# mozack/vdjer

Measured on AMD Instinct MI355X. Metric: M paired-reads/sec (k-mer build + contig score), IgH 50bp PE, higher is better.
Workload: dtype u8/u64 (2-bit packed bases, integer counts)

## Files before the change

profiles/summarize_pmc.py:

```python
#!/usr/bin/env python3
import collections
import csv
import glob
import json
import os
import sys


def short(name):
    return name.replace("void ", "").replace("(anonymous namespace)::", "").split("(")[0].split("<")[0]


def med(v):
    v = sorted(v)
    return v[len(v) // 2] if v else None


def stream_in(bench_line):
    if not bench_line:
        return {}
    b = bench_line
    pairs = b["config"]["pairs_per_gpu"]
    st = b.get("scorer_stats", {})
    sym, symw = st.get("kmer_build_sym", 0), st.get("kmer_build_sym_walk", 0)
    tuples = st.get("gated_instances", 0) / (2 if sym else 1)
    items = st.get("recount_items", 0)
    recs = 4 * pairs
    gate = 24 * recs
    return {"k_pool_pack": 101 * recs,
            "k_gated_hist": gate, "k_part_records_g": gate + 16 * tuples, "k_part_tuples_g": 16 * tuples, "k_seg_hist_g": 16 * tuples,
            "k_gated_reduce": 16 * tuples, "k_gated_local": 16 * tuples, "k_walk_items": 24 * recs,
            "k_part_items": 8 * items, "k_recount": 8 * items, "k_compact_partials": 0, "k_bucket_merge": 0}


COMPOSITES = {
    "k_surv_table": ("k_surv_table2", "k_succ_links2"),
    "k_chain_order": ("k_chain_init", "k_chain_jump", "k_chain_len", "k_scan_sums", "k_scan_apply", "k_chain_place", "k_chain_permute", "k_table_remap",
                      "k_partner", "k_chain_words", "k_partner_check"),
    "k_node_order": ("k_rank_keys", "k_rank_scatter", "k_node_emit2"),
    "k_shard_resolve": ("k_resolve_first", "k_resolve_add", "k_resolve_keep"),
}


def step_span(rows, steps):
    packs = [i for i, r in enumerate(rows) if short(r["Kernel_Name"]).startswith("k_pool_pack") or short(r["Kernel_Name"]).startswith("k_pool_unpack")]
    walks = [i for i, r in enumerate(rows) if short(r["Kernel_Name"]) == "k_walk_items"]
    if not packs or len(walks) < steps:
        return []
    chains = int(os.environ.get("PROF_CHAINS", "1"))
    per = max(1, round(len(packs) / max(1, len(walks)))) * chains
    first = packs[-per * steps] if len(packs) >= per * steps else packs[0]
    return rows[first:]


def main():
    out = sys.argv[1]
    steps_timed = int(os.environ.get("PROF_STEPS", "2"))
    bench_line = None
    try:
        bench_line = json.loads(open(os.path.join(out, "bench.json")).read().strip().splitlines()[-1])
    except Exception:
        pass
    STREAM_IN = stream_in(bench_line)
    res = collections.defaultdict(dict)
    step_tot = {}
    for grp in ("fetch", "write", "sq", "tcc", "inst", "ea"):
        per = collections.defaultdict(lambda: collections.defaultdict(list))
        for f in glob.glob(os.path.join(out, grp, "**", "*counter_collection.csv"), recursive=True):
            rows = list(csv.DictReader(open(f)))
            for r in rows:
                per[short(r["Kernel_Name"])][r["Counter_Name"]].append(float(r["Counter_Value"]))
            if grp in ("fetch", "write") and rows:
                key = "Dispatch_Id" if "Dispatch_Id" in rows[0] else None
                if key:
                    rows.sort(key=lambda r: int(r[key]))
                span = step_span(rows, steps_timed)
                agg = collections.defaultdict(lambda: [0.0, 0])
                for r in span:
                    a = agg[short(r["Kernel_Name"])]
                    a[0] += float(r["Counter_Value"]) * 1024
                    a[1] += 1
                step_tot[grp] = {k_: (v_[0] / steps_timed, v_[1] / steps_timed) for k_, v_ in agg.items()}
        for k, cs in per.items():
            for c, v in cs.items():
                res[k][c] = med(v)
                res[k].setdefault("launches_seen", len(v))
    stats = {}
    for f in glob.glob(os.path.join(out, "stats", "**", "*kernel_stats.csv"), recursive=True):
        for r in csv.DictReader(open(f)):
            stats[short(r["Name"])] = {"calls": int(r["Calls"]), "avg_ns": float(r["AverageNs"]), "total_ns": float(r["TotalDurationNs"])}
    for k, d in res.items():
        if "FETCH_SIZE" in d:
            fetch, write = d["FETCH_SIZE"] * 1024, d.get("WRITE_SIZE", 0.0) * 1024
            stream = STREAM_IN.get(k)
            d["fabric_bytes_max"] = int(2 * fetch + write)
            d["stream_in_bytes"] = None if stream is None else int(stream)
            d["hbm_bytes"] = int(fetch + min(fetch, stream / 2) + write) if stream is not None else int(2 * fetch + write)
            d["traffic_rule"] = "FETCH + min(FETCH, stream_in/2) + WRITE" if stream is not None else "2*FETCH + WRITE (no stated stream: bound)"
        if d.get("TCC_HIT_sum") is not None and d.get("TCC_MISS_sum") is not None and d["TCC_HIT_sum"] + d["TCC_MISS_sum"] > 0:
            d["l2_hit"] = round(d["TCC_HIT_sum"] / (d["TCC_HIT_sum"] + d["TCC_MISS_sum"]), 4)
        if d.get("SQ_WAVE_CYCLES"):
            for c in ("SQ_WAIT_ANY", "SQ_WAIT_INST_ANY", "SQ_ACTIVE_INST_ANY", "SQ_WAIT_INST_LDS"):
                if d.get(c) is not None:
                    d[c + "_frac"] = round(d[c] / d["SQ_WAVE_CYCLES"], 4)
        if d.get("SQ_LDS_IDX_ACTIVE"):
            d["lds_conflict_frac"] = round(d.get("SQ_LDS_BANK_CONFLICT", 0.0) / d["SQ_LDS_IDX_ACTIVE"], 4)
        d.update(stats.get(k, {}))
        if d.get("SQ_INSTS_VALU") and d.get("avg_ns"):
            d["valu_issue_frac_at_2.4GHz"] = round(d["SQ_INSTS_VALU"] * 4 / (1024 * 2.4 * d["avg_ns"]), 3)
    step = None
    if "fetch" in step_tot:
        fk, wk = step_tot["fetch"], step_tot.get("write", {})
        tot_f = tot_w = tot_cal = 0.0
        per_kernel = {}
        for k_ in set(fk) | set(wk):
            f_, n_ = fk.get(k_, (0.0, 0))
            w_ = wk.get(k_, (0.0, 0))[0]
            stream = STREAM_IN.get(k_)
            cal = f_ + (min(f_, stream * n_ / 2) if stream is not None else f_) + w_
            per_kernel[k_] = {"fetch_bytes_per_step": int(f_), "write_bytes_per_step": int(w_), "launches_per_step": n_, "fabric_bytes_per_step": int(cal)}
            tot_f += f_; tot_w += w_; tot_cal += cal
        step = {"bytes_per_step": int(tot_cal), "bytes_per_step_max": int(2 * tot_f + tot_w), "fetch_counted": int(tot_f), "write_counted": int(tot_w),
                "kernels_counted": len(per_kernel), "steps": steps_timed,
                "rule": "every dispatch of the last `steps` steps of the process (all kernels: the library's, rocPRIM's, fills), FETCH_SIZE / WRITE_SIZE passes; "
                        "per kernel FETCH + min(FETCH, stated coalesced input / 2) + WRITE, kernels without a stated stream at the bound 2*FETCH + WRITE",
                "per_kernel": per_kernel}
        for comp, members in COMPOSITES.items():
            got = [per_kernel[m] for m in members if m in per_kernel]
            if got:
                res[comp]["composite_of"] = [m for m in members if m in per_kernel]
                res[comp]["hbm_bytes_per_step"] = int(sum(g["fabric_bytes_per_step"] for g in got))
                res[comp]["launches_per_step"] = sum(g["launches_per_step"] for g in got)
                ns_ = sum(res[m].get("avg_ns", 0.0) * per_kernel[m]["launches_per_step"] for m in members if m in per_kernel and m in res)
                res[comp]["ns_per_step"] = ns_
                for c in ("l2_hit", "SQ_WAIT_ANY_frac", "lds_conflict_frac"):
                    ws = [(res[m].get(c), res[m].get("avg_ns", 0.0) * per_kernel[m]["launches_per_step"]) for m in members if m in res and m in per_kernel and res[m].get(c) is not None]
                    if ws and sum(w for _, w in ws) > 0:
                        res[comp][c] = round(sum(v * w for v, w in ws) / sum(w for _, w in ws), 4)
    json.dump({"kernels": res, "step": step}, sys.stdout, indent=1, sort_keys=True)


if __name__ == "__main__":
    main()
```

vdjer_amd/csrc/vdjx_kmer.hip:

```cpp
#include "vdjx_common.h"

#include <algorithm>
#include <numeric>
#include <type_traits>
#include <string.h>
#include <stdlib.h>

#define HIST_THREADS 512
#define HIST_BLOCKS 512u
#define LOCAL_SLOTS 2048u
#define K3_SUB_TUPLES g_sub_tuples
__device__ u32 g_sub_tuples = 262144u;
#define NONE32 0xFFFFFFFFu
#define INST_MASK 0x7FFFFFFFu

struct RecView {
	u64 bhi, blo, nm, lq;
};

__device__ inline RecView load_rec(const u64* __restrict__ bases, const u64* __restrict__ nmask,
                                   const u64* __restrict__ lowq, size_t r) {
	RecView v;
	const ulonglong2 b = ((const ulonglong2*) bases)[r];
	v.bhi = b.x; v.blo = b.y;
// ... 1132 lines not shown
#define REPLY_RQ0 248
template <bool SYM>
__global__ __launch_bounds__(64) void k_shard_reply(const uint2* __restrict__ queries, u32 nq, const u32* __restrict__ owner_off, u32 G,
                                                    const Partial* __restrict__ dense, const u32* __restrict__ dense_ref,
                                                    const u32* __restrict__ dstart, u32 NBo, const u64* __restrict__ low_inst,
                                                    const u64* __restrict__ bases, const u64* __restrict__ nmask,
                                                    vdjx_qrows quals, u64 rec_base, const u32* __restrict__ scan, u32 n_local, int k, int rl, int ob,
                                                    uint8_t* __restrict__ replies) {
	const u32 qi = blockIdx.x;
	if (qi >= nq) return;
	const u32 lane = threadIdx.x;
	u32 o = 0;
	while (o + 1 < G && owner_off[o + 1] <= qi) o++;
	const uint2 q = queries[qi];
	const u32 di = dstart[(size_t) o * NBo] + q.x;
	u64 finst, finst_r = 0;
	u32 p_cg;
	if (SYM) { const PartialS p = ((const PartialS*) dense)[di]; finst = ps_fg(p); finst_r = p.fgr; p_cg = ps_cg(p); }
	else { const Partial p = dense[di]; finst = p.fg; p_cg = p.cg; }
	const u32 need = q.y >> 30;
	const u32 om = (1u << ob) - 1u;
	auto local_rec = [&](u64 inst) -> u64 {
		if (!scan) return (inst >> ob) - rec_base;
		const u32 g = (u32) (inst >> ob);
		u32 lo = 0, hi = n_local;
		while (lo + 1 < hi) { const u32 mid = lo + ((hi - lo) >> 1); if (scan[mid] <= g) lo = mid; else hi = mid; }
		return lo;
	};
	const u64 frec = local_rec(finst);
	const u32 foff = (u32) finst & om;
	const u64 finst_local = (frec << ob) | foff;
	const u64 frec_r = SYM ? local_rec(finst_r) : 0;
	const u32 foff_r = (u32) finst_r & om;
	const u64 finst_r_local = (frec_r << ob) | foff_r;
	uint8_t* out = replies + (size_t) qi * REPLY_BYTES;
	if (lane == 0) {
		((u32*) out)[0] = q.y;
		((u32*) out)[1] = 0;
		((u64*) out)[1] = finst;
		if (SYM) ((u64*) out)[REPLY_R0 / 8] = finst_r;
	}
	if (!SYM && lane < (REPLY_BYTES - REPLY_R0) / 4) ((u32*) (out + REPLY_R0))[lane] = 0;
	if (lane < 8) {
		const int W = rl <= VDJX_SHORT_READ_LEN ? 2 : VDJX_LONG_W, M = rl <= VDJX_SHORT_READ_LEN ? 1 : VDJX_LONG_M;
		((u64*) out)[2 + lane] = (int) lane < W ? bases[frec * W + lane] : ((int) lane < W + M ? nmask[frec * M + (lane - W)] : 0ull);
	}
	if ((int) lane >= k) return;
	u32 acc = 0, acc_r = 0;
	const u32 ref = dense_ref[di];
	if ((need & NEED_Q) && ref != NONE32) {
		const u32 cg = p_cg & ~PART_FLAG;
		for (u32 i = 0; i < cg; i++) {
			const u64 inst = low_inst[ref + i];
			if (inst != (scan ? finst_local : finst)) acc += (u32) (uint8_t) (quals.row((inst >> ob) - rec_base)[((u32) inst & om) + lane] - 33);
			if (SYM) {
				const u64 m = vdjx_inst_mirror(inst, ob, rl, k);
				if (m != (scan ? finst_r_local : finst_r)) acc_r += (u32) (uint8_t) (quals.row((m >> ob) - rec_base)[((u32) m & om) + lane] - 33);
			}
		}
	}
	const uint8_t* fr = quals.row(frec);
	out[REPLY_Q0 + lane] = (uint8_t) (acc > 255u ? 255u : acc);
	out[REPLY_Q0 + REPLY_KQ + lane] = (uint8_t) (fr[foff + lane] - 33);
	out[REPLY_Q0 + 2 * REPLY_KQ + lane] = (uint8_t) (fr[lane] - 33);
	if (SYM) {
		const uint8_t* frr = quals.row(frec_r);
		out[REPLY_RQ0 + lane] = (uint8_t) (acc_r > 255u ? 255u : acc_r);
		out[REPLY_RQ0 + REPLY_KQ + lane] = (uint8_t) (frr[foff_r + lane] - 33);
		out[REPLY_RQ0 + 2 * REPLY_KQ + lane] = (uint8_t) (frr[lane] - 33);
	}
}

__global__ void k_resolve_first(const uint8_t* __restrict__ replies, u32 nr, const u64* __restrict__ p_mg, u32* __restrict__ p_r0,
                                const u64* __restrict__ p_mgr, u32 np) {
	const u32 r = blockIdx.x * blockDim.x + threadIdx.x;
	if (r >= nr) return;
	const uint8_t* me = replies + (size_t) r * REPLY_BYTES;
	const u32 pid = ((const u32*) me)[0] & PID_MASK;
	if (((const u64*) me)[1] == p_mg[pid]) p_r0[pid] = r;
	if (p_mgr && ((const u64*) me)[REPLY_R0 / 8] == p_mgr[pid]) p_r0[np + pid] = r;
}

__global__ __launch_bounds__(256) void k_resolve_add(const uint8_t* __restrict__ replies, u32 nr, const u32* __restrict__ p_r0, int k, u32* __restrict__ p_fl,
                                                     u32* __restrict__ p_S, u32 np) {
	const u32 r = blockIdx.x * 4u + (threadIdx.x >> 6);
	const u32 lane = threadIdx.x & 63u;
	if (r >= nr) return;
	const uint8_t* me = replies + (size_t) r * REPLY_BYTES;
	const u32 w0 = ((const u32*) me)[0];
	const u32 pid = w0 & PID_MASK, need = w0 >> 30;
	const u32 r0 = p_r0[pid];
	if (r0 == NONE32) return;
	if ((need & NEED_SEQ) && r != r0 && lane == 0) {
		const u64* a = (const u64*) me;
		const u64* b = (const u64*) (replies + (size_t) r0 * REPLY_BYTES);
		u64 d = 0;
#pragma unroll
		for (int w = 2; w < 10; w++) d |= a[w] ^ b[w];
		if (d) p_fl[pid] = 1;
	}
	if ((need & NEED_Q) && (int) lane < k) {
		const uint8_t* first = me + REPLY_Q0 + (r == r0 ? 2 * REPLY_KQ : REPLY_KQ);
		atomicAdd(&p_S[(size_t) pid * 64 + lane], (u32) me[REPLY_Q0 + lane] + (u32) first[lane]);
		if (np) {
			const uint8_t* first_r = me + REPLY_RQ0 + (r == p_r0[np + pid] ? 2 * REPLY_KQ : REPLY_KQ);
			atomicAdd(&p_S[((size_t) np + pid) * 64 + lane], (u32) me[REPLY_RQ0 + lane] + (u32) first_r[lane]);
		}
	}
}

template <bool SYM>
__global__ void k_resolve_keep(PendOut po, u32 np, const u32* __restrict__ p_fl, const u32* __restrict__ p_S, int k, u32 mf, u32 mqq, u32 tlow,
                               SurvOutG so) {
	const u32 p = blockIdx.x * blockDim.x + threadIdx.x;
	const bool in = p < np;
	const u32 need = in ? po.need[p] : 0u;
	bool keep = in && ((need & NEED_SEQ) ? p_fl[p] != 0 : true);
	const u32 cg = in ? po.cg[p] : 0u;
	const u32 cgc = cg > CNT_CAP ? CNT_CAP : cg;
	keep = keep && cgc >= mf;
	bool keep_r = keep;
	if (keep && cg < tlow) {
		for (int j = 0; j < k; j++) if (p_S[(size_t) p * 64 + j] < mqq) { keep = false; break; }
		if (SYM) for (int j = 0; j < k; j++) if (p_S[((size_t) np + p) * 64 + j] < mqq) { keep_r = false; break; }
	}
	if (!SYM) {
		const u32 pos = vdjx_wave_inc(so.n, keep);
		if (keep && pos < so.cap) {
			so.lo[pos] = po.lo[p]; so.hi[pos] = po.hi[p];
			so.gcnt[pos] = cgc; so.gfirst[pos] = po.mg[p];
		}
		return;
	}
	const bool any = keep || keep_r;
	const u32 pos = vdjx_wave_inc(so.n, any, 2u);
	if (any && pos + 1 < so.cap) {
		so.lo[pos] = po.lo[p]; so.hi[pos] = po.hi[p];
		so.gcnt[pos] = cgc | (keep ? 0u : GC_SHADOW); so.gfirst[pos] = po.mg[p];
		u64 rh, rlo;
		vdjx_kmer_rc(po.hi[p], po.lo[p], k, rh, rlo);
		so.lo[pos + 1] = rlo; so.hi[pos + 1] = rh;
		so.gcnt[pos + 1] = cgc | (keep_r ? 0u : GC_SHADOW); so.gfirst[pos + 1] = po.mgr[p];
	}
}

__global__ void k_first_to_scan(u64* __restrict__ a, size_t na, u64* __restrict__ b, size_t nb, const u32* __restrict__ scan, int ob) {
	const size_t i = (size_t) blockIdx.x * blockDim.x + threadIdx.x;
	if (i >= na + nb) return;
	u64* p = i < na ? a + i : b + (i - na);
	const u64 v = *p;
	if (v != NONE64) *p = ((u64) scan[v >> ob] << ob) | (v & ((1ull << ob) - 1ull));
}

__global__ void k_node_flags(const u64* __restrict__ s_lo, const u64* __restrict__ s_hi, u32 n, int k,
                             const u32* __restrict__ vbits, const u32* __restrict__ jbits,
                             uint8_t* __restrict__ has_v, uint8_t* __restrict__ has_j) {
	u32 i = blockIdx.x * blockDim.x + threadIdx.x;
	if (i >= n) return;
	if (k <= 16) { has_v[i] = 1; has_j[i] = 1; return; }
	u128 key = ((u128) s_hi[i] << 64) | s_lo[i];
	u32 code = (u32) (key >> (2 * (k - 16)));
	has_v[i] = code ? (vbits[code >> 5] >> (code & 31)) & 1u : 0;
	has_j[i] = code ? (jbits[code >> 5] >> (code & 31)) & 1u : 0;
}


#define IT_INST_BITS 35
#define IT_INST_MASK ((1ull << IT_INST_BITS) - 1ull)
#define IT_SURV_SHIFT 38
int vdjx_sort_pairs_raw(void* tmp, size_t* tmp_bytes, hipStream_t st, u64* k_in, u64* k_out, u32* v_in, u32* v_out, u32 n, unsigned end_bit);
#define IT_HOLE 0xFFFFFFFFFFFFFFFFull
#define WALK_THREADS 256

#define SLOT_HI_BITS 36
#define SLOT_HI_MASK ((1ull << SLOT_HI_BITS) - 1ull)
struct SurvTable { const ulonglong2* slots; u32 mask; const ulonglong2* skey; const u32* bloom; u32 bloom_mask; };

struct ItemFmt {
	u32 pmask;
	u32 len_shift;
	u32 maxlen;
	u32 mul, inv;
	u32 bmask;
	u32 ns;
};
__device__ inline u32 it_surv(const ItemFmt& f, u64 x) { return (u32) (x >> IT_SURV_SHIFT) & f.pmask; }
__device__ inline u32 it_len(const ItemFmt& f, u64 x) { return f.maxlen > 1 ? (u32) (x >> f.len_shift) + 1u : 1u; }
__device__ inline u32 it_scat(const ItemFmt& f, u32 p) { return ((((p >> 4) * f.mul) & f.bmask) << 4) | (p & 15u); }

__global__ void k_surv_table2(const u64* __restrict__ s_lo, const u64* __restrict__ s_hi, u32 n, ulonglong2* __restrict__ slots, u32 mask,
                              ulonglong2* __restrict__ skey, u32* __restrict__ bloom, u32 bloom_mask) {
	const u32 i = blockIdx.x * blockDim.x + threadIdx.x;
	if (i >= n) return;
	const u64 lo = s_lo[i], hi = s_hi[i];
	skey[i] = make_ulonglong2(lo, hi);
	const u64 h = vdjx_mix(lo, hi);
	{
		const u32 bit = (u32) (h >> 40) & bloom_mask;
		atomicOr(&bloom[bit >> 5], 1u << (bit & 31));
	}
	u32 slot = (u32) (h >> 20) & mask;
	const unsigned long long entry = hi | ((unsigned long long) (i + 1) << SLOT_HI_BITS);
	while (atomicCAS((unsigned long long*) &slots[slot].y, 0ull, entry) != 0ull) slot = (slot + 1) & mask;
	slots[slot].x = lo;
}

__device__ inline int surv_lookup2f(const SurvTable& t, u64 lo, u64 hi);

__device__ inline int surv_lookup2(const SurvTable& t, u64 lo, u64 hi) {
	u32 slot = (u32) (vdjx_mix(lo, hi) >> 20) & t.mask;
	for (;;) {
		const ulonglong2 v = t.slots[slot];
		if (!v.y) return -1;
		if (v.x == lo && (v.y & SLOT_HI_MASK) == hi) return (int) (v.y >> SLOT_HI_BITS) - 1;
		slot = (slot + 1) & t.mask;
	}
}

__device__ inline int surv_lookup2f(const SurvTable& t, u64 lo, u64 hi) {
	const u64 h = vdjx_mix(lo, hi);
	const u32 bit = (u32) (h >> 40) & t.bloom_mask;
	if (!((t.bloom[bit >> 5] >> (bit & 31)) & 1u)) return -1;
	return surv_lookup2(t, lo, hi);
}

__global__ void k_succ_links2(SurvTable t, u32 n, int k, const u32* __restrict__ gcnt, u32* __restrict__ succ, unsigned long long* __restrict__ pred,
                              u32* __restrict__ bestsucc) {
	const u32 u = blockIdx.x * blockDim.x + threadIdx.x;
	if (u >= n) return;
	const ulonglong2 kk = t.skey[u];
	const u128 base = (((u128) kk.y << 64) | kk.x) << 2;
	const u128 km = k < 64 ? (((u128) 1) << (2 * k)) - 1 : ~(u128) 0;
	const int sh = 2 * (k - 1);
	const u32 fb = (u32) (sh < 64 ? kk.x >> sh : kk.y >> (sh - 64)) & 3u;
	const unsigned long long mine = ((unsigned long long) (gcnt[u] & GC_MASK) << 32) | ((unsigned long long) (fb ^ 1u) << 30) | (unsigned long long) u;
	u32 best = NONE32, best_g = 0;
	for (u32 b = 0; b < 4; b++) {
		const u128 key = (base | (u128) b) & km;
		const int s = surv_lookup2(t, (u64) key, (u64) (key >> 64));
		succ[u * 4 + b] = s >= 0 ? (u32) s : NONE32;
		if (s >= 0 && (u32) s != u) {
			const u32 g = gcnt[s] & GC_MASK;
			if (best == NONE32 || g >= best_g) { best = (u32) s; best_g = g; }
			atomicMax(&pred[s], mine);
		}
	}
	bestsucc[u] = best;
}

#define CHAIN_JUMPS 31
__global__ void k_chain_init(const unsigned long long* __restrict__ pred, const u32* __restrict__ bestsucc, u32 n, u64* __restrict__ pd) {
	const u32 v = blockIdx.x * blockDim.x + threadIdx.x;
	if (v >= n) return;
	const unsigned long long x = pred[v];
	const u32 u = (u32) x & 0x3FFFFFFFu;
	pd[v] = x != 0ull && bestsucc[u] == v ? ((u64) u << 32) | 1ull : ((u64) NONE32 << 32);
}

__global__ void k_partner(SurvTable t, u32 n, int k, u32* __restrict__ partner) {
	const u32 p = blockIdx.x * blockDim.x + threadIdx.x;
	if (p >= n) return;
	const ulonglong2 kk = t.skey[p];
	u64 rh, rlo;
	vdjx_kmer_rc(kk.y, kk.x, k, rh, rlo);
	const int q = surv_lookup2(t, rlo, rh);
	partner[p] = q >= 0 ? (u32) q : NONE32;
}
__global__ void k_partner_check(const u32* __restrict__ partner, const u64* __restrict__ linw, u32 n, u32* __restrict__ bad) {
	const u32 p = blockIdx.x * blockDim.x + threadIdx.x;
	if (p >= n) return;
	bool wrong = partner[p] == NONE32;
	const bool linked = (linw[p >> 4] >> (15u - (p & 15u))) & 1ull;
	if (!wrong && linked && (p + 1 >= n || partner[p + 1] != partner[p] - 1u)) wrong = true;
	const u64 m = __ballot(wrong);
	if (m && __lane_id() == 0) atomicAdd(bad, (u32) __popcll(m));
}

__global__ void k_chain_jump(u64* __restrict__ pd, u32 n, const u32* __restrict__ open_prev, u32* __restrict__ open_now) {
	if (open_prev && *open_prev == 0) return;
	const u32 v = blockIdx.x * blockDim.x + threadIdx.x;
	bool open = false;
	if (v < n) {
		u64 x = __atomic_load_n(&pd[v], __ATOMIC_RELAXED);
		for (int it = 0; it < CHAIN_JUMPS; it++) {
			const u32 p = (u32) (x >> 32);
			if (p == NONE32) break;
			const u64 y = __atomic_load_n(&pd[p], __ATOMIC_RELAXED);
			const u32 pp = (u32) (y >> 32);
			if (pp == NONE32) break;
			x = ((u64) pp << 32) | (u64) ((u32) x + (u32) y);
			__atomic_store_n(&pd[v], x, __ATOMIC_RELAXED);
			open = true;
		}
	}
	if (__ballot(open) && __lane_id() == 0) atomicAdd(open_now, 1u);
}

__device__ inline void chain_of(const u64* pd, u32 v, u32& head, u32& dist) {
	const u64 x = pd[v];
	const u32 p = (u32) (x >> 32);
	head = v; dist = 0;
	if (p == NONE32) return;
	if ((u32) (pd[p] >> 32) != NONE32) return;
	head = p; dist = (u32) x;
}
__global__ void k_chain_len(const u64* __restrict__ pd, u32 n, u32* __restrict__ len) {
	const u32 v = blockIdx.x * blockDim.x + threadIdx.x;
	if (v >= n) return;
	u32 h, d;
	chain_of(pd, v, h, d);
	atomicAdd(&len[h], 1u);
}

#define SCAN_BLOCK 4096u
__global__ __launch_bounds__(256) void k_scan_sums(const u32* __restrict__ a, u32 n, u32* __restrict__ sums) {
	__shared__ u32 part[4];
	const u32 b0 = blockIdx.x * SCAN_BLOCK;
	u32 s = 0;
	for (u32 i = threadIdx.x; i < SCAN_BLOCK; i += 256) s += b0 + i < n ? a[b0 + i] : 0u;
	s = (u32) vdjx_wave_scan_add((int) s);
	if ((threadIdx.x & 63) == 63) part[threadIdx.x >> 6] = s;
	__syncthreads();
	if (threadIdx.x == 0) sums[blockIdx.x] = part[0] + part[1] + part[2] + part[3];
}
__global__ __launch_bounds__(256) void k_scan_apply(const u32* __restrict__ a, u32 n, const u32* __restrict__ sum_start, u32* __restrict__ out) {
	__shared__ u32 part[5];
	const u32 b0 = blockIdx.x * SCAN_BLOCK + threadIdx.x * 16;
	u32 loc[16];
	u32 s = 0;
	for (int i = 0; i < 16; i++) { loc[i] = s; s += b0 + i < n ? a[b0 + i] : 0u; }
	const u32 incl = (u32) vdjx_wave_scan_add((int) s);
	if ((threadIdx.x & 63) == 63) part[threadIdx.x >> 6] = incl;
	__syncthreads();
	u32 base = sum_start[blockIdx.x] + incl - s;
	for (u32 w = 0; w < (threadIdx.x >> 6); w++) base += part[w];
	for (int i = 0; i < 16; i++) if (b0 + i < n) out[b0 + i] = base + loc[i];
}

__global__ void k_chain_place(const u64* __restrict__ pd, const u32* __restrict__ off, u32 n, u32* __restrict__ newidx) {
	const u32 v = blockIdx.x * blockDim.x + threadIdx.x;
	if (v >= n) return;
	u32 h, d;
	chain_of(pd, v, h, d);
	newidx[v] = off[h] + d;
}
__global__ void k_chain_permute(const u32* __restrict__ newidx, u32 n, const u64* __restrict__ lo, const u64* __restrict__ hi, const u32* __restrict__ gcnt,
                                const u64* __restrict__ gfirst, const u32* __restrict__ succ, u64* __restrict__ lo2, u64* __restrict__ hi2,
                                u32* __restrict__ gcnt2, u64* __restrict__ gfirst2, ulonglong2* __restrict__ skey2, u32* __restrict__ succ2) {
	const u32 v = blockIdx.x * blockDim.x + threadIdx.x;
	if (v >= n) return;
	const u32 q = newidx[v];
	const u64 l = lo[v], h = hi[v];
	lo2[q] = l; hi2[q] = h; gcnt2[q] = gcnt[v]; gfirst2[q] = gfirst[v];
	skey2[q] = make_ulonglong2(l, h);
	const uint4 s = *(const uint4*) &succ[(size_t) v * 4];
	uint4 r;
	r.x = s.x == NONE32 ? NONE32 : newidx[s.x];
	r.y = s.y == NONE32 ? NONE32 : newidx[s.y];
	r.z = s.z == NONE32 ? NONE32 : newidx[s.z];
	r.w = s.w == NONE32 ? NONE32 : newidx[s.w];
	*(uint4*) &succ2[(size_t) q * 4] = r;
}
__global__ void k_table_remap(ulonglong2* __restrict__ slots, u32 n_slots, const u32* __restrict__ newidx) {
	const u32 i = blockIdx.x * blockDim.x + threadIdx.x;
	if (i >= n_slots) return;
	const u64 y = slots[i].y;
	if (!y) return;
	slots[i].y = (y & SLOT_HI_MASK) | ((u64) (newidx[(u32) (y >> SLOT_HI_BITS) - 1] + 1u) << SLOT_HI_BITS);
}

__global__ void k_chain_words(const u32* __restrict__ succ, const ulonglong2* __restrict__ skey, u32 n, int k, u64* __restrict__ linw, u32* __restrict__ fbw,
                              const u32* __restrict__ partner) {
	const u32 p = blockIdx.x * blockDim.x + threadIdx.x;
	const u32 j = p & 15u;
	u64 w = 0;
	u32 fb = 0;
	if (p < n) {
		const uint4 s = *(const uint4*) &succ[(size_t) p * 4];
		const u32 sv[4] = {s.x, s.y, s.z, s.w};
		const bool mirrored = !partner || (p + 1 < n && partner[p] != NONE32 && partner[p + 1] == partner[p] - 1u);
		for (u32 b = 0; b < 4; b++) if (sv[b] != NONE32) {
			if (sv[b] == p + 1 && mirrored) w |= (1ull << (15u - j)) | ((u64) b << (32u + 2u * (15u - j)));
			else w |= 1ull << (31u - j);
		}
		const ulonglong2 kk = skey[p];
		const int sh = 2 * (k - 1);
		fb = (u32) (sh < 64 ? kk.x >> sh : kk.y >> (sh - 64)) & 3u;
	}
	u32 fw = fb << (2 * j);
	for (int d = 1; d < 16; d <<= 1) {
		w |= ((u64) (u32) __shfl_xor((int) (w >> 32), d) << 32) | (u32) __shfl_xor((int) (u32) w, d);
		fw |= (u32) __shfl_xor((int) fw, d);
	}
	if (j == 0 && p < n) { linw[p >> 4] = w; fbw[p >> 4] = fw; }
}

struct WalkRecS {
	u64 bhi, blo; int rl;
	__device__ inline void kmer_u(int k, int o, u64& hi, u64& lo) const { vdjx_kmer_at(bhi, blo, rl, k, o, hi, lo); }
	__device__ inline void kmer_l(int k, int o, u64& hi, u64& lo) const { vdjx_kmer_at_lane(bhi, blo, rl, k, o, hi, lo); }
	__device__ inline u32 bases16(int bi) const {
		const int sh = 2 * (rl - 16 - bi);
		const u32 rw_dn = vdjx_bits_at_lane(bhi, blo, (u32) (sh > 0 ? sh : 0));
		const u32 up = (u32) (sh < 0 ? -sh : 0);
		return (rw_dn << (up & 31u)) & (0u - (u32) (up < 32u));
	}
	__device__ inline u32 base(int i) const { return vdjx_base_at_lane(bhi, blo, rl, i); }
};
struct WalkRecL {
	const u64* row;
	__device__ inline void kmer_u(int k, int o, u64& hi, u64& lo) const { vdjx_kmer_at_words(row, k, o, hi, lo); }
	__device__ inline void kmer_l(int k, int o, u64& hi, u64& lo) const { vdjx_kmer_at_words(row, k, o, hi, lo); }
	__device__ inline u32 bases16(int bi) const { return vdjx_bases16_words(row, bi); }
	__device__ inline u32 base(int i) const { return vdjx_base_words(row, i); }
};
__device__ inline bool wm_test(u64 m, int i) { return (m >> i) & 1ull; }
__device__ inline bool wm_test(const vdjx_mask3& m, int i) { return m.test(i); }
__device__ inline void wm_set(u64& m, int i) { m |= 1ull << i; }
__device__ inline void wm_set(vdjx_mask3& m, int i) { m.set(i); }
__device__ inline int wm_next(u64 m, int from, int none) { const u64 x = from < 64 ? m & (~0ull << from) : 0ull; return x ? __builtin_ctzll(x) : none; }
__device__ inline int wm_next(const vdjx_mask3& m, int from, int none) { return m.next(from, none); }
__device__ inline u32 wm_slice32(u64 m, int from) { return from < 64 ? (u32) (m >> from) : 0u; }
__device__ inline u32 wm_slice32(const vdjx_mask3& m, int from) { return (u32) m.slice(from); }

template <bool LONG, bool SYM = false>
__global__ __launch_bounds__(WALK_THREADS) void k_walk_items(const u64* __restrict__ bases, const u64* __restrict__ nmask, size_t R, int rl, int ob_bits, int k,
                                                             SurvTable t, const u32* __restrict__ succ, const u64* __restrict__ linw, ItemFmt f,
                                                             u32 range_shift, u32 n_ranges,
                                                             u64* __restrict__ raw, u64 raw_cap, u32 blk_items,
                                                             unsigned long long* __restrict__ g_cursor,
                                                             u32* __restrict__ range_cnt, u32* __restrict__ g_err, u32 dbg_in,
                                                             const u32* __restrict__ partner) {
	static_assert(!(LONG && SYM), "SYM is the short-read form");
#ifdef VDJX_ABLATE
	const u32 dbg = dbg_in;
#else
	(void) dbg_in;
	constexpr u32 dbg = 0u;
#endif
	extern __shared__ u32 hist[];
	typedef typename std::conditional<LONG, vdjx_mask3, u64>::type MaskT;
	typedef typename std::conditional<LONG, WalkRecL, WalkRecS>::type RecT;
	for (u32 i = threadIdx.x; i < n_ranges; i += WALK_THREADS) hist[i] = 0;
	__syncthreads();
	u64* myrow = (u64*) (hist + ((n_ranges + 1u) & ~1u)) + threadIdx.x * GL_ROW_LONG;
	const int P = rl - k + 1;
	const size_t per = ((R + gridDim.x - 1) / gridDim.x + WALK_THREADS - 1) / WALK_THREADS * WALK_THREADS;
	const size_t r0 = (size_t) blockIdx.x * per;
	const size_t r1 = r0 + per < R ? r0 + per : R;
	const int lane = __lane_id();
	u64 blk = 0;
	u32 fill = blk_items;
#ifdef WALK_STATS
	u32 st_rows = 0, st_rounds = 0, st_filter = 0, st_lookup = 0, st_items = 0, st_chain = 0;
#define WST(x) x
#else
#define WST(x)
#endif
	bool have_blk = false, dead = false;
	__shared__ u64 dq[WALK_THREADS / 64][128];
	__shared__ ulonglong2 dq_b[LONG ? 1 : WALK_THREADS / 64][LONG ? 1 : 128];
	__shared__ u64 dq_v[LONG ? 1 : WALK_THREADS / 64][LONG ? 1 : 128];
	const u32 wq = threadIdx.x >> 6;
	u32 qn = 0;
	auto walk_row = [&](auto fresh_tag, const size_t r, const bool live, const int o_from, const ulonglong2 qb, const u64 qv) {
		constexpr bool FRESH = decltype(fresh_tag)::value;
		RecT v;
		MaskT V{};
		if constexpr (LONG) {
			v.row = myrow;
			if (live) {
				stage_row_long(myrow, bases, r);
				const vdjx_mask3 nm = load_bad3(nmask, nullptr, r);
				for (int o16 = 0; o16 < P; o16 += 16) {
					const u64 g = (u64) vdjx_clean16(nm, o16, k, P) << (o16 & 63);
					if ((o16 >> 6) == 0) V.w0 |= g; else if ((o16 >> 6) == 1) V.w1 |= g; else V.w2 |= g;
				}
			} else
				for (int w = 0; w < GL_ROW_LONG; w++) myrow[w] = 0;
		} else {
			v.bhi = v.blo = 0; v.rl = rl;
			if (!FRESH) { if (live) { v.bhi = qb.x; v.blo = qb.y; V = qv; } }
			else if (live) {
				const RecView rv = load_rec(bases, nmask, nullptr, r);
				v.bhi = rv.bhi; v.blo = rv.blo;
				u64 inv = rv.nm;
				int cur = 1;
				while (cur * 2 <= k) { inv |= inv >> cur; cur *= 2; }
				inv |= inv >> (k - cur);
				V = ~inv & (P >= 64 ? ~0ull : (1ull << P) - 1ull);
			}
		}
		int o = wm_next(V, o_from, P);
		int s = -1;
		u32 in = 0;
		bool first = FRESH, have_c = false;
		MaskT C{};
		WST(st_rows++;)
		while (__ballot(o < P)) {
			WST(st_rounds++;)
			bool need = o < P && s < 0;
			if (FRESH) {
				const bool later = need && !first;
				const u64 lm = __ballot(later);
				if (lm) {
					if (later) {
						const u32 qi = qn + (u32) __popcll(lm & ((1ull << lane) - 1ull));
						dq[wq][qi] = ((u64) r << 8) | (u64) (u32) o;
						if constexpr (!LONG) { dq_b[wq][qi] = make_ulonglong2(v.bhi, v.blo); dq_v[wq][qi] = V; }
						o = P; need = false;
					}
					qn += (u32) __popcll(lm);
				}
			}
			WST(if (__ballot(need)) st_lookup++;)
			if (!FRESH && __ballot(need && !first && !have_c)) {
				WST(st_filter++;)
				const bool mine = need && !first && !have_c;
				for (int ob = 0; ob < P; ob += 4) {
					u32 wv[4], bt[4];
#pragma unroll
					for (int j = 0; j < 4; j++) {
						const int oo = ob + j;
						wv[j] = 0; bt[j] = 0;
						if (mine && oo >= o && oo < P && wm_test(V, oo)) {
							u64 khi, klo;
							v.kmer_u(k, oo, khi, klo);
							const u32 bit = (u32) (vdjx_mix(klo, khi) >> 40) & t.bloom_mask;
							bt[j] = bit & 31u;
							wv[j] = (dbg & 8u) ? 0xFFFFFFFFu : t.bloom[bit >> 5];
						}
					}
#pragma unroll
					for (int j = 0; j < 4; j++) if ((wv[j] >> bt[j]) & 1u) wm_set(C, ob + j);
				}
				if (mine) have_c = true;
			}
			if (need) {
				bool filtered = false;
				if (!first) {
					o = wm_next(C, o, P);
					filtered = true;
				}
				first = false;
				if (o < P) {
					u64 khi, klo;
					v.kmer_l(k, o, khi, klo);
// ... 188 lines not shown
#pragma unroll
		for (u32 j = 0; j < PER; j++) {
			const size_t t = ts + (size_t) j * PART_THREADS + threadIdx.x;
			r_b[j] = NONE32;
			if (t < te) { r_it[j] = in[t]; r_b[j] = (it_scat(f, it_surv(f, r_it[j])) >> range_shift) & mask; }
		}
#pragma unroll
		for (u32 j = 0; j < PER; j++) if (r_b[j] != NONE32) atomicAdd(&cnt[r_b[j]], 1u);
		__syncthreads();
		part_scan(cnt, base, tmp, nbk);
		for (u32 i = threadIdx.x; i < nbk; i += PART_THREADS) {
			cur[i] = base[i];
			gbase[i] = cnt[i] ? atomicAdd(&gc[i], cnt[i]) : 0u;
		}
		__syncthreads();
#pragma unroll
		for (u32 j = 0; j < PER; j++) if (r_b[j] != NONE32) stage[atomicAdd(&cur[r_b[j]], 1u)] = r_it[j];
		__syncthreads();
		const u32 n = base[nbk];
		for (u32 i = threadIdx.x; i < n; i += PART_THREADS) {
			const u64 x = stage[i];
			const u32 b = (it_scat(f, it_surv(f, x)) >> range_shift) & mask;
			out[gbase[b] + (i - base[b])] = x;
		}
		__syncthreads();
	}
}

#define RC_THREADS 1024
#define RC_UNR 4
template <typename IT> struct RcNone;
template <> struct RcNone<u32> { static constexpr u32 v = 0xFFFFFFFFu; };
template <> struct RcNone<u64> { static constexpr u64 v = 0xFFFFFFFFFFFFFFFFull; };
__device__ inline void rc_min(u32* p, u32 v) { atomicMin(p, v); }
__device__ inline void rc_min(u64* p, u64 v) { atomicMin((unsigned long long*) p, (unsigned long long) v); }

#define RC_CS 17u
#define RC_MS 77u
__device__ inline u32 rc_win(u32 k, u32 s) { return 31u + ((0x261B0E00u >> (8u * k)) & 0xFFu) + s - 1u; }
template <u32 SB, typename IT>
__global__ __launch_bounds__(RC_THREADS) void k_recount(const u64* __restrict__ items, const u32* __restrict__ range_start, ItemFmt f, u32 ns, u64 rec_base, int ob,
                                                        const u32* __restrict__ fbw, u32* __restrict__ ucnt, u64* __restrict__ ufirst, u64* __restrict__ in_first,
                                                        unsigned long long* __restrict__ n_inst) {
	__shared__ u32 c[SB / 16 * RC_CS];
	__shared__ IT mv[SB / 16 * RC_MS];
	__shared__ IT ef[SB * 4];
	__shared__ u32 fbl[SB / 16];
	__shared__ unsigned long long tot;
	constexpr IT NONE = RcNone<IT>::v;
	const u32 b = blockIdx.x;
	const u32 s0 = b * SB;
	const u32 nb = (ns + 15u) >> 4;
	for (u32 i = threadIdx.x; i < SB / 16 * RC_CS; i += RC_THREADS) c[i] = 0;
	for (u32 i = threadIdx.x; i < SB / 16 * RC_MS; i += RC_THREADS) mv[i] = NONE;
	for (u32 i = threadIdx.x; i < SB * 4; i += RC_THREADS) ef[i] = NONE;
	for (u32 i = threadIdx.x; i < SB / 16; i += RC_THREADS) {
		const u32 sb = (s0 >> 4) + i;
		const u32 blk = (sb * f.inv) & f.bmask;
		fbl[i] = sb <= f.bmask && blk < nb ? fbw[blk] : 0u;
	}
	if (threadIdx.x == 0) tot = 0;
	__syncthreads();
	const u32 i0 = range_start[b], i1 = range_start[b + 1];
	const u32 iend = i0 + (i1 - i0 + RC_THREADS * RC_UNR - 1) / (RC_THREADS * RC_UNR) * (RC_THREADS * RC_UNR);
	for (u32 ib = i0 + threadIdx.x; ib < iend; ib += RC_THREADS * RC_UNR) {
		u64 xs[RC_UNR];
#pragma unroll
		for (int u = 0; u < RC_UNR; u++) { const u32 i = ib + (u32) u * RC_THREADS; xs[u] = i < i1 ? items[i] : IT_HOLE; }
#pragma unroll
		for (int u = 0; u < RC_UNR; u++) {
			const u64 x = xs[u];
			const bool live = x != IT_HOLE;
			const u32 p = it_surv(f, x);
			const u32 len = live ? it_len(f, x) : 1u;
			const u32 sl = live ? it_scat(f, p) - s0 : 0u;
			const u32 a = sl & 15u, e = a + len - 1u;
			const u64 inst = x & IT_INST_MASK;
			const bool shaped = live && (a == 0u || e == 15u);
			const u32 cb = (sl >> 4) * RC_CS, mb = (sl >> 4) * RC_MS;
			const u32 slot = mb + (a == 0u ? e : 15u + a);
			const IT val = (IT) (inst + 15u - a);
			bool mine = shaped;
			const u64 act = __ballot(shaped);
			if (act) {
				const int leader = __ffsll((long long) act) - 1;
				const u32 lslot = (u32) __builtin_amdgcn_readlane((int) slot, leader);
				const bool same = shaped && slot == lslot;
				const u64 m = __ballot(same);
				if (__popcll(m) >= 8) {
					const u64 v64 = inst + 15u - a;
					const u32 hi_min = vdjx_wave_min(same ? (u32) (v64 >> 32) : 0xFFFFFFFFu);
					const u32 lo_min = vdjx_wave_min(same && (u32) (v64 >> 32) == hi_min ? (u32) v64 : 0xFFFFFFFFu);
					if (__lane_id() == leader) {
						const u32 n = (u32) __popcll(m);
						atomicAdd(&c[cb + e], n);
						if (a) atomicAdd(&c[cb + a - 1u], 0u - n);
						rc_min(&mv[lslot], (IT) (((u64) hi_min << 32) | lo_min));
					}
					mine = shaped && !same;
				}
			}
			if (live && (mine || !shaped)) {
				atomicAdd(&c[cb + e], 1u);
				if (a) atomicAdd(&c[cb + a - 1u], 0xFFFFFFFFu);
			}
			if (mine) rc_min(&mv[slot], val);
			if (live && !shaped) {
				const u32 k = 31u - (u32) __builtin_clz(len), w = 1u << k;
				rc_min(&mv[mb + rc_win(k, a)], val);
				if (len != w) rc_min(&mv[mb + rc_win(k, e + 1u - w)], val);
			}
			if (live && ((x >> 37) & 1ull)) {
				IT* ep = &ef[sl * 4 + (u32) ((x >> 35) & 3ull)];
				if (vdjx_peek(ep) > (IT) inst) rc_min(ep, (IT) inst);
			}
		}
	}
	__syncthreads();
	const u64 add = rec_base << ob;
	u32 my_cnt = 0;
	for (u32 i = threadIdx.x; i < SB; i += RC_THREADS) {
		const u32 sb = (s0 + i) >> 4;
		const u32 blk = (sb * f.inv) & f.bmask;
		const u32 x = i & 15u, p = (blk << 4) | x;
		if (sb > f.bmask || blk >= nb || p >= ns) continue;
		const u32 cbase = (i >> 4) * RC_CS, mbase = (i >> 4) * RC_MS;
		u32 cc = 0;
		IT mm = NONE;
		IT me = NONE;
		for (u32 e = x; e < 16; e++) { cc += c[cbase + e]; const IT t = mv[mbase + e]; mm = t < mm ? t : mm; if (x) me = t < me ? t : me; }
		for (u32 a = 1; a <= x; a++) { const IT t = mv[mbase + 15 + a]; mm = t < mm ? t : mm; if (a < x) me = t < me ? t : me; }
#pragma unroll
		for (u32 k = 0; k < 4; k++) {
			const u32 w = 1u << k;
			const u32 lo = x >= w ? x - w + 1u : 1u, hi = x < 15u - w ? x : 15u - w;
			for (u32 s = lo ? lo : 1u; s <= hi; s++) { const IT t = mv[mbase + rc_win(k, s)]; mm = t < mm ? t : mm; if (s < x) me = t < me ? t : me; }
		}
		my_cnt += cc;
		ucnt[p] = cc;
		ufirst[p] = mm == NONE ? NONE64 : (u64) mm - 15u + x + add;
		IT e4[4] = {ef[i * 4], ef[i * 4 + 1], ef[i * 4 + 2], ef[i * 4 + 3]};
		if (x && me != NONE) {
			const u32 pa = (fbl[i >> 4] >> (2 * (x - 1))) & 3u;
			const IT t = (IT) (me - 15u + x);
			if (t < e4[pa]) e4[pa] = t;
		}
		for (u32 q = 0; q < 4; q++) in_first[(size_t) p * 4 + q] = e4[q] == NONE ? NONE64 : (u64) e4[q] + add;
	}
	if (my_cnt) atomicAdd(&tot, (unsigned long long) my_cnt);
	__syncthreads();
	if (threadIdx.x == 0 && tot) atomicAdd(n_inst, tot);
}

__global__ void k_count_unseen(const u64* __restrict__ ufirst, u32 n, u32* __restrict__ out) {
	const u32 i = blockIdx.x * blockDim.x + threadIdx.x;
	const bool un = i < n && ufirst[i] == NONE64;
	const u64 m = __ballot(un);
	if (m && __lane_id() == 0) atomicAdd(out, (u32) __popcll(m));
}

__global__ void k_edges_from_in(SurvTable t, u32 n, int k, const u64* __restrict__ in_first, u32* __restrict__ in_from,
                                u64* __restrict__ edge_first, u32* __restrict__ edge_to) {
	const u32 e = blockIdx.x * blockDim.x + threadIdx.x;
	if (e >= n * 4u) return;
	const u64 fs = in_first[e];
	if (fs == NONE64) { in_from[e] = NONE32; return; }
	const u32 v = e >> 2, a = e & 3u;
	const ulonglong2 kk = t.skey[v];
	const u128 kv = ((u128) kk.y << 64) | kk.x;
	const u128 ku = (kv >> 2) | ((u128) a << (2 * (k - 1)));
	const int u = surv_lookup2(t, (u64) ku, (u64) (ku >> 64));
	in_from[e] = u >= 0 ? (u32) u : NONE32;
	if (u >= 0) {
		const u32 oe = (u32) u * 4u + ((u32) kk.x & 3u);
		edge_first[oe] = fs;
		edge_to[oe] = v;
	}
}

struct SurvRec { u64 lo, hi; u32 gcnt, pad; u64 gfirst; };

__global__ void k_surv_pack(const u64* __restrict__ lo, const u64* __restrict__ hi, const u32* __restrict__ gcnt,
                            const u64* __restrict__ gfirst, u32 n, SurvRec* __restrict__ out) {
	u32 i = blockIdx.x * blockDim.x + threadIdx.x;
	if (i >= n) return;
	SurvRec r{lo[i], hi[i], gcnt[i], 0u, gfirst[i]};
	out[i] = r;
}

__global__ void k_surv_unpack(const SurvRec* __restrict__ in, u32 n, u64* __restrict__ lo, u64* __restrict__ hi, u32* __restrict__ gcnt,
                              u64* __restrict__ gfirst, u32* __restrict__ n_real) {
	u32 i = blockIdx.x * blockDim.x + threadIdx.x;
	const bool in_range = i < n;
	SurvRec r{0, 0, GC_SHADOW, 0, 0};
	if (in_range) {
		r = in[i];
		lo[i] = r.lo; hi[i] = r.hi; gcnt[i] = r.gcnt; gfirst[i] = r.gfirst;
	}
	(void) vdjx_wave_inc(n_real, in_range && !(r.gcnt & GC_SHADOW));
}

struct NodeOut {
	u64* first_inst; u32* gcnt; u32* freq; uint8_t* hv; uint8_t* hj; u64* klo; u64* khi; char* kmers;
	uint8_t* to_deg; u32* to_ids; uint8_t* from_deg; u32* from_ids;
};

__global__ void k_rank_keys(const u64* __restrict__ ufirst, const u32* __restrict__ gcnt, u32 n, u64* __restrict__ key, u32* __restrict__ idx) {
	const u32 i = blockIdx.x * blockDim.x + threadIdx.x;
	if (i < n) { key[i] = (gcnt[i] & GC_SHADOW) ? NONE64 : ufirst[i]; idx[i] = i; }
}
__global__ void k_rank_scatter(const u64* __restrict__ key, const u32* __restrict__ idx, u32 n, u32* __restrict__ rank) {
	const u32 j = blockIdx.x * blockDim.x + threadIdx.x;
	if (j >= n) return;
	const u32 i = idx[j];
	rank[i] = key[j] == NONE64 ? i : j;
}

__global__ __launch_bounds__(256) void k_root_count(const uint8_t* __restrict__ from_deg, u32 n, u32* __restrict__ block_cnt) {
	__shared__ u32 cnt;
	if (threadIdx.x == 0) cnt = 0;
	__syncthreads();
	const u32 i = blockIdx.x * 256 + threadIdx.x;
	const bool r = i < n && from_deg[i] == 0;
	const u64 b = __ballot(r);
	if ((threadIdx.x & 63) == 0 && b) atomicAdd(&cnt, (u32) __popcll(b));
	__syncthreads();
	if (threadIdx.x == 0) block_cnt[blockIdx.x] = cnt;
}

__global__ __launch_bounds__(256) void k_root_list(const uint8_t* __restrict__ from_deg, u32 n, const u32* __restrict__ block_start,
                                                   u32* __restrict__ roots) {
	__shared__ u32 wave_cnt[4];
	const u32 i = blockIdx.x * 256 + threadIdx.x;
	const bool r = i < n && from_deg[i] == 0;
	const u64 b = __ballot(r);
	const u32 w = threadIdx.x >> 6, lane = threadIdx.x & 63;
	if (lane == 0) wave_cnt[w] = (u32) __popcll(b);
	__syncthreads();
	u32 base = block_start[blockIdx.x];
	for (u32 j = 0; j < w; j++) base += wave_cnt[j];
	if (r) roots[base + (u32) __popcll(b & ((1ull << lane) - 1))] = i;
}

__device__ inline void sort4_desc64(u64 (&f)[4], u32 (&id)[4]) {
#define CSW(a, b) { const bool sw = kk[a] < kk[b]; if (sw) { u64 t = kk[a]; kk[a] = kk[b]; kk[b] = t; u32 u = id[a]; id[a] = id[b]; id[b] = u; } }
	u64 kk[4];
	for (int i = 0; i < 4; i++) kk[i] = f[i] == NONE64 ? 0ull : f[i] + 1;
	CSW(0, 1) CSW(2, 3) CSW(0, 2) CSW(1, 3) CSW(1, 2)
	for (int i = 0; i < 4; i++) f[i] = kk[i] ? kk[i] - 1 : NONE64;
#undef CSW
}

__global__ void k_node_emit2(const u64* __restrict__ s_lo, const u64* __restrict__ s_hi, const u32* __restrict__ s_gcnt,
                             const u32* __restrict__ s_ucnt, const u64* __restrict__ s_ufirst, const uint8_t* __restrict__ hv,
                             const uint8_t* __restrict__ hj, const u32* __restrict__ rank, const u64* __restrict__ edge_first,
                             const u32* __restrict__ edge_to, const u64* __restrict__ in_first, const u32* __restrict__ in_from,
                             u32 n, int k, NodeOut o) {
	const u32 s = blockIdx.x * blockDim.x + threadIdx.x;
	if (s >= n) return;
	if (s_gcnt[s] & GC_SHADOW) return;
	const u32 r = rank[s];
	o.first_inst[r] = s_ufirst[s];
	o.gcnt[r] = s_gcnt[s];
	o.freq[r] = s_ucnt[s] > 32765u ? 32765u : s_ucnt[s];
	o.hv[r] = hv[s];
	o.hj[r] = hj[s];
	const u128 key = ((u128) s_hi[s] << 64) | s_lo[s];
	for (int j = 0; j < k; j++) {
		const u32 b = (u32) (key >> (2 * (k - 1 - j))) & 3u;
		o.kmers[(size_t) r * k + j] = b == 0 ? 'A' : (b == 1 ? 'T' : (b == 2 ? 'C' : 'G'));
	}
	u64 f[4];
	u32 id[4];
	for (int e = 0; e < 4; e++) {
		f[e] = edge_first[(size_t) s * 4 + e];
		if (f[e] != NONE64 && (s_gcnt[edge_to[(size_t) s * 4 + e]] & GC_SHADOW)) f[e] = NONE64;
		id[e] = f[e] != NONE64 ? rank[edge_to[(size_t) s * 4 + e]] + 1 : 0;
	}
	sort4_desc64(f, id);
	u32 deg = 0;
	for (int e = 0; e < 4; e++) { o.to_ids[(size_t) r * 4 + e] = f[e] != NONE64 ? id[e] : 0; deg += f[e] != NONE64; }
	o.to_deg[r] = (uint8_t) deg;
	for (int e = 0; e < 4; e++) {
		f[e] = in_first[(size_t) s * 4 + e];
		if (f[e] != NONE64 && (in_from[(size_t) s * 4 + e] == NONE32 || (s_gcnt[in_from[(size_t) s * 4 + e]] & GC_SHADOW))) f[e] = NONE64;
		id[e] = f[e] != NONE64 ? rank[in_from[(size_t) s * 4 + e]] + 1 : 0;
	}
	sort4_desc64(f, id);
	deg = 0;
	for (int e = 0; e < 4; e++) { o.from_ids[(size_t) r * 4 + e] = f[e] != NONE64 ? id[e] : 0; deg += f[e] != NONE64; }
	o.from_deg[r] = (uint8_t) deg;
}

namespace {

struct PersistAlloc {
	vdjx_ctx* c;
	explicit PersistAlloc(vdjx_ctx* ctx) : c(ctx) {}
	template <typename T> hipError_t alloc(T** out, size_t n) {
		*out = (T*) c->shard_arena.alloc((n ? n : 1) * sizeof(T));
		return *out ? hipSuccess : hipErrorOutOfMemory;
	}
	vdjx_arena::mark_t mark() const { return c->shard_arena.mark(); }
	void release_to(vdjx_arena::mark_t m) { c->shard_arena.release_to(m); }
};

struct PoolView { const u64* bases; const u64* nmask; vdjx_qrows quals; int rl; int ob; };

template <typename TUP> struct GTuples {
	TUP* t = nullptr;
	u32* bucket_start = nullptr;
	u32 NB = 0, N = 0;
};

struct SurvivorsG {
	u64 *lo = nullptr, *hi = nullptr, *gfirst = nullptr, *ufirst = nullptr;
	u32 *gcnt = nullptr, *ucnt = nullptr;
	u32 n = 0, n_real = 0;
	u64 ndist = 0;
};

inline u32 ceil_log2_u64(u64 x) { u32 b = 0; while ((1ull << b) < x) b++; return b; }

static bool sync_debug() { static const bool on = vdjx_env_set("VDJX_SYNC_DEBUG"); return on; }
static void dbg_sync(vdjx_ctx* c, const char* what) {
	if (!sync_debug()) return;
	const hipError_t e = hipStreamSynchronize(c->stream);
	fprintf(stderr, "[vdjx] %s: %s\n", what, hipGetErrorString(e));
}

struct GatedHist { u32 HB = 0, NBH = 0, N = 0; u32* hstart = nullptr; bool sym = false; };
static bool build_sym(const vdjx_pool* pool, int k) {
	return pool->sym && pool->W == 2 && (k & 1) && pool->n_records % 2 == 0;
}
static bool sym_walk_wanted() { static const bool on = !vdjx_env_set("VDJX_NO_SYM_WALK"); return on; }
static size_t gated_bucket_default() { static const size_t v = (size_t) vdjx_env_num("VDJX_GATED_BUCKET", 3072, 1, 1ll << 32); return v; }
template <typename A>
int stage_gated_hist(vdjx_ctx* c, A& db, const vdjx_pool* pool, int k, size_t per_bucket, u64 geometry_instances, GatedHist* gh, bool sym = false) {
	hipStream_t st = c->stream;
	const size_t R = sym ? pool->n_records / 2 : pool->n_records;
	const int P = pool->rl - k + 1;
	const u64 NI = geometry_instances ? geometry_instances : (u64) R * (u64) P;
	const size_t per = per_bucket ? per_bucket : gated_bucket_default();
	const u32 hb_max = pool->W > 2 ? 14u : 15u;
	u32 HB = ceil_log2_u64((NI + per - 1) / per);
	HB = std::max(8u, std::min(hb_max, HB));
	const u32 NBH = 1u << HB;
#ifdef VDJX_ABLATE
	static const u32 hist_dbg = (u32) vdjx_env_num("VDJX_HIST_DBG", 0, 0, 4);
#else
	constexpr u32 hist_dbg = 0;
#endif
	u32 nblk = (u32) std::min<size_t>(HIST_BLOCKS, (R + 4095) / 4096);
	if (nblk == 0) nblk = 1;
	size_t rpb = (R + nblk - 1) / nblk;
	u32 *hcnt, *hstart;
	HIP_TRY(db.alloc(&hcnt, NBH));
	HIP_TRY(db.alloc(&hstart, NBH + 1));
	HIP_TRY(hipMemsetAsync(hcnt, 0, (size_t) NBH * 4, st));
	const bool lng = pool->W > 2;
	const size_t lds_hist = (size_t) NBH * 4 + (HIST_THREADS / 64) * (lng ? GL_WAVE_BYTES_LONG : GL_WAVE_BYTES);
	HIP_TRY(hipFuncSetAttribute((const void*) k_gated_hist<false>, hipFuncAttributeMaxDynamicSharedMemorySize, (int) lds_hist));
	HIP_TRY(hipFuncSetAttribute((const void*) k_gated_hist<true>, hipFuncAttributeMaxDynamicSharedMemorySize, (int) lds_hist));
	HIP_TRY(hipFuncSetAttribute((const void*) k_gated_hist<false, true>, hipFuncAttributeMaxDynamicSharedMemorySize, (int) lds_hist));
	{
		vdjx_prof_scope ps(c, "k_gated_hist");
		if (lng) hipLaunchKernelGGL(k_gated_hist<true>, dim3(nblk), dim3(HIST_THREADS), lds_hist, st, pool->d_bases, pool->d_nmask, pool->d_lowq, R, pool->rl, k, HB, rpb, hcnt, hist_dbg);
		else if (sym) hipLaunchKernelGGL((k_gated_hist<false, true>), dim3(nblk), dim3(HIST_THREADS), lds_hist, st, pool->d_bases, pool->d_nmask, pool->d_lowq, R, pool->rl, k, HB, rpb, hcnt, hist_dbg);
		else hipLaunchKernelGGL(k_gated_hist<false>, dim3(nblk), dim3(HIST_THREADS), lds_hist, st, pool->d_bases, pool->d_nmask, pool->d_lowq, R, pool->rl, k, HB, rpb, hcnt, hist_dbg);
	}
	dbg_sync(c, "k_gated_hist");
	hipLaunchKernelGGL(k_bucket_scan, dim3(1), dim3(1024), 0, st, hcnt, NBH, hstart);
	HIP_TRY(hipMemcpyAsync(c->h_pin, hstart + NBH, 4, hipMemcpyDeviceToHost, st));
	HIP_TRY(hipStreamSynchronize(st));
	HIP_TRY(hipGetLastError());
#ifdef VDJX_ABLATE
	if (hist_dbg) return VDJX_ESTATE;
#endif
	const u32 N = *(const u32*) c->h_pin;
	c->stats["gated_instances"] = sym ? 2ull * N : N;
	gh->HB = HB; gh->NBH = NBH; gh->N = N; gh->hstart = hstart; gh->sym = sym;
	return VDJX_OK;
}

template <typename TUP, typename A>
int stage_gated_cut(vdjx_ctx* c, A& db, const vdjx_pool* pool, u64 rec_base, int k, size_t per_bucket, u64 geometry_instances, const GatedHist& gh, GTuples<TUP>* out) {
	hipStream_t st = c->stream;
	const bool sym = gh.sym;
	const size_t R = sym ? pool->n_records / 2 : pool->n_records;
	const int P = pool->rl - k + 1;
	const size_t per = per_bucket ? per_bucket : gated_bucket_default();
	const u32 hb_max = pool->W > 2 ? 14u : 15u;
	const bool lng = pool->W > 2;
	const u32 HB = gh.HB, NBH = gh.NBH, N = gh.N;
	u32* hstart = gh.hstart;
	size_t rpb;
	out->N = N;
	const u64 Ng = geometry_instances ? geometry_instances : (u64) N;
	static const size_t refine = (size_t) vdjx_env_num("VDJX_REFINE_TUPLES", 4096, 1, 1ll << 32);
	u32 T = 8;
	while (T < HB && ((u64) per << T) < Ng) T++;
	u32 extra = 0;
	const size_t refine_at = per_bucket ? std::max<size_t>(per_bucket, refine / 2) : refine;
	if (T == HB && HB == hb_max && Ng / NBH > refine_at) {
		extra = 1;
		while (extra < 5 && (Ng >> extra) / NBH > refine_at) extra++;
	}
	const u32 Tt = T + extra;
	const u32 NBt = 1u << Tt;
	HIP_TRY(db.alloc(&out->t, (size_t) N + 1));
	constexpr u32 stage_tuples = PARTR_STAGE_BYTES / (u32) sizeof(TUP);
	constexpr u32 lds_partr = PARTR_STAGE_BYTES + stage_tuples * 4;
	HIP_TRY(hipFuncSetAttribute((const void*) k_part_records_g<TUP, false>, hipFuncAttributeMaxDynamicSharedMemorySize, (int) lds_partr));
	HIP_TRY(hipFuncSetAttribute((const void*) k_part_records_g<TUP, true>, hipFuncAttributeMaxDynamicSharedMemorySize, (int) lds_partr));
	HIP_TRY(hipFuncSetAttribute((const void*) k_part_records_g<TUP, false, true>, hipFuncAttributeMaxDynamicSharedMemorySize, (int) lds_partr));
	HIP_TRY(hipFuncSetAttribute((const void*) k_part_tuples_g<TUP>, hipFuncAttributeMaxDynamicSharedMemorySize, PART_LDS_BYTES));
	u32 cbits = Tt, fbits = 0;
	if (Tt > 10) { cbits = extra ? Tt - 10 : 8; fbits = Tt - cbits; }
	const u32 NBc = 1u << cbits;
	u32 nblk2 = (u32) std::min<size_t>(1024, (R + 2047) / 2048);
	if (nblk2 == 0) nblk2 = 1;
	rpb = (R + nblk2 - 1) / nblk2;
	u32* gcur;
	HIP_TRY(db.alloc(&gcur, NBc));
	TUP* l1 = out->t;
	if (fbits) HIP_TRY(db.alloc(&l1, (size_t) N + 1));
	{
		vdjx_prof_scope ps(c, "k_part_records");
		hipLaunchKernelGGL(k_init_cursors, dim3((NBc + 255) / 256), dim3(256), 0, st, hstart, NBc, HB - cbits, gcur);
		const u64 NIl = (u64) R * (u64) P;
		u64 rr = N ? (u64) stage_tuples * 3 / 4 * NIl / ((u64) N * (u64) P) : 1u << 16;
		rr = std::max<u64>(PART_THREADS, std::min<u64>(rr / PART_THREADS * PART_THREADS, lng ? 1u << 14 : 1u << 16));
		if (lng) hipLaunchKernelGGL((k_part_records_g<TUP, true>), dim3(nblk2), dim3(PART_THREADS), lds_partr, st, pool->d_bases, pool->d_nmask, pool->d_lowq, R, rec_base,
		                            pool->rl, k, 64 - cbits, NBc, rpb, (u32) rr, gcur, l1);
		else if (sym) hipLaunchKernelGGL((k_part_records_g<TUP, false, true>), dim3(nblk2), dim3(PART_THREADS), lds_partr, st, pool->d_bases, pool->d_nmask, pool->d_lowq, R, rec_base,
		                                 pool->rl, k, 64 - cbits, NBc, rpb, (u32) rr, gcur, l1);
		else hipLaunchKernelGGL((k_part_records_g<TUP, false>), dim3(nblk2), dim3(PART_THREADS), lds_partr, st, pool->d_bases, pool->d_nmask, pool->d_lowq, R, rec_base,
		                        pool->rl, k, 64 - cbits, NBc, rpb, (u32) rr, gcur, l1);
	}
	dbg_sync(c, "k_part_records");
	u32* tstart;
	HIP_TRY(db.alloc(&tstart, NBt + 1));
	out->NB = NBt;
	out->bucket_start = tstart;
	constexpr u32 slices = PART_SLICES;
	if (extra) {
		u32* fine_cnt;
		HIP_TRY(db.alloc(&fine_cnt, NBt));
		HIP_TRY(hipMemsetAsync(fine_cnt, 0, (size_t) NBt * 4, st));
		vdjx_prof_scope ps(c, "k_seg_hist");
		hipLaunchKernelGGL(k_seg_hist_g<TUP>, dim3(NBc * slices), dim3(512), 0, st, l1, hstart, HB - cbits, slices, 64 - Tt, fbits, fine_cnt);
		hipLaunchKernelGGL(k_bucket_scan, dim3(1), dim3(1024), 0, st, fine_cnt, NBt, tstart);
	} else {
		hipLaunchKernelGGL(k_pick_u32, dim3((NBt + 1 + 255) / 256), dim3(256), 0, st, hstart, 1u << (HB - Tt), NBt + 1, tstart);
	}
	if (fbits) {
		u32* gcur2;
		HIP_TRY(db.alloc(&gcur2, NBt));
		vdjx_prof_scope ps(c, "k_part_tuples");
		hipLaunchKernelGGL(k_init_cursors, dim3((NBt + 255) / 256), dim3(256), 0, st, tstart, NBt, 0u, gcur2);
		hipLaunchKernelGGL(k_part_tuples_g<TUP>, dim3(NBc * slices), dim3(PART_THREADS), PART_LDS_BYTES, st, l1, hstart, HB - cbits, slices, 64 - Tt, fbits,
		                   gcur2, out->t);
	}
	return VDJX_OK;
}

template <typename TUP, typename A>
int stage_gated_partition(vdjx_ctx* c, A& db, const vdjx_pool* pool, u64 rec_base, int k, size_t per_bucket, u64 geometry_instances, GTuples<TUP>* out, bool sym = false) {
	GatedHist gh;
	int rc = stage_gated_hist(c, db, pool, k, per_bucket, geometry_instances, &gh, sym);
	if (rc) return rc;
	return stage_gated_cut<TUP>(c, db, pool, rec_base, k, per_bucket, geometry_instances, gh, out);
}

static int set_sub_tuples(vdjx_ctx* c) {
	static const u32 sub = (u32) vdjx_env_num("VDJX_SUB_TUPLES", 262144, 1, 0xFFFFFFFFll);
	if (c->sub_tuples_set != sub) {
		HIP_TRY(hipMemcpyToSymbolAsync(HIP_SYMBOL(g_sub_tuples), &sub, 4, 0, hipMemcpyHostToDevice, c->stream));
		c->sub_tuples_set = sub;
	}
	return VDJX_OK;
}
template <typename TUP, typename A>
int bucket_order(vdjx_ctx* c, A& db, const GTuples<TUP>& t, u32** order) {
	*order = nullptr;
	if (t.NB < 1024) return VDJX_OK;
	HIP_TRY(db.alloc(order, t.NB));
	hipLaunchKernelGGL(k_bucket_order, dim3(1), dim3(1024), 0, c->stream, t.bucket_start, t.NB, *order);
	return VDJX_OK;
}

template <typename TUP, typename A>
int stage_gated_reduce(vdjx_ctx* c, A& db, const GTuples<TUP>& t, const PoolView& pv, u64 rec_base, int k, int mf, int mq, SurvivorsG* sv, bool sym = false) {
	hipStream_t st = c->stream;
	int rc = set_sub_tuples(c);
	if (rc) return rc;
	if (mq >= 255) mq = 254;
	const u32 mqq = (u32) (mq < 0 ? 0 : (mq > 214 ? 214 : mq));
	const u32 tlow = 1 + (mqq + 19) / 20;
	const u32 cmin = (u32) std::max(mf, 2);
	const u32 mfu = (u32) std::max(mf, 0);
	const u32 cap = (sym ? t.N : t.N / 2) + 16;
	u32 *g_err, *n_surv;
	u64* g_distinct;
	HIP_TRY(db.alloc(&sv->lo, cap)); HIP_TRY(db.alloc(&sv->hi, cap)); HIP_TRY(db.alloc(&sv->gcnt, cap)); HIP_TRY(db.alloc(&sv->gfirst, cap));
	HIP_TRY(db.alloc(&g_distinct, 64 * 16 + 2));
	g_err = (u32*) (g_distinct + 64 * 16);
	n_surv = g_err + 1;
	u32* n_real = g_err + 2;
	HIP_TRY(hipMemsetAsync(g_distinct, 0, (64 * 16 + 2) * 8, st));
	SurvOutG so{sv->lo, sv->hi, sv->gcnt, sv->gfirst, n_surv, cap, n_real};
	static const u32 rd_dbg = (u32) vdjx_env_num("VDJX_RD_DBG", 0, 0, 9);
	if (t.N) {
		vdjx_prof_scope ps(c, "k_gated_reduce");
		u32* order;
		if ((rc = bucket_order(c, db, t, &order))) return rc;
		if (sym) hipLaunchKernelGGL((k_gated_reduce<TUP, true>), dim3(t.NB), dim3(RD_THREADS), 0, st, t.t, t.bucket_start, pv.bases, pv.nmask, pv.quals, pv.rl, pv.ob, k, rec_base,
		                            mfu, cmin, mqq, tlow, so, g_distinct, g_err, rd_dbg, (const u32*) order);
		else hipLaunchKernelGGL(k_gated_reduce<TUP>, dim3(t.NB), dim3(RD_THREADS), 0, st, t.t, t.bucket_start, pv.bases, pv.nmask, pv.quals, pv.rl, pv.ob, k, rec_base,
		                        mfu, cmin, mqq, tlow, so, g_distinct, g_err, rd_dbg, (const u32*) order);
	}
	u64* spread = (u64*) c->h_pin;
	u32* tail = (u32*) (spread + 64 * 16);
	static_assert((64 * 16 + 2) * 8 == VDJX_HPIN_SYNC_BYTES, "h_pin layout (vdjx_common.h)");
	HIP_TRY(hipMemcpyAsync(spread, g_distinct, VDJX_HPIN_SYNC_BYTES, hipMemcpyDeviceToHost, st));
	HIP_TRY(hipStreamSynchronize(st));
	HIP_TRY(hipGetLastError());
	const u32 ns = tail[1], err = tail[0];
	if (err) { vdjx_set_error("k_gated_reduce: %u buckets could not be split to fit LDS", err); return VDJX_EHIP; }
	if (ns > cap) { vdjx_set_error("survivor capacity logic failed (%u > %u)", ns, cap); return VDJX_EHIP; }
	sv->ndist = 0;
	for (int i = 0; i < 64; i++) sv->ndist += spread[i * 16];
	sv->n = ns;
	sv->n_real = sym ? tail[2] : ns;
	c->stats["kmer_build_shadows"] = ns - sv->n_real;
	return VDJX_OK;
}

struct RecountOut { u32* ucnt; u64* ufirst; u64* in_first; u32* in_from; u64* edge_first; u32* edge_to; };
struct RecountStatus { const u32* g_err = nullptr; const u32* n_items = nullptr; const unsigned long long* n_inst = nullptr; u32 ns = 0; };
#define VDJX_ESYMWALK (-1000)
static int recount_status_check(vdjx_ctx* c, const u32* hp, u32 ns) {
	if (hp[6] || hp[7]) { vdjx_set_error("the mirrored walk found %u + %u places where the chains are not mirror images", hp[6], hp[7]); return VDJX_ESYMWALK; }
	if (hp[0]) { vdjx_set_error("k_walk_items: item buffer too small (%u waves stopped)", hp[0]); return VDJX_EHIP; }
	if (hp[1]) { vdjx_set_error("internal error: %u of %u surviving k-mers were not met again in the records (VDJX_SYNC_DEBUG=1 names them)", hp[1], ns); return VDJX_EHIP; }
	c->stats["recount_items"] = hp[2];
	c->stats["recount_instances"] = *(const unsigned long long*) (hp + 4);
	return VDJX_OK;
}

template <typename A>
int stage_recount(vdjx_ctx* c, A& db, const vdjx_pool* pool, u64 rec_base, int k, SurvivorsG& sv, const RecountOut& ro,
                  bool derive_edges, SurvTable* table_out = nullptr, RecountStatus* defer = nullptr, bool sym_walk = false) {
	hipStream_t st = c->stream;
	const size_t R = pool->n_records;
	const int P = pool->rl - k + 1;
	const u32 ns = sv.n;
	if (ns >= (1u << 26)) { vdjx_set_error("more than 2^26 surviving k-mers: not supported by the recount items"); return VDJX_ELIMIT; }
	if (R >= (1ull << 29)) { vdjx_set_error("more than 2^29 records on one GPU: not supported by the recount items"); return VDJX_ELIMIT; }
	if ((u64) R * (u64) P >= (1ull << 32)) { vdjx_set_error("records*offsets = %llu >= 2^32 on one GPU: shard the pool over more GPUs", (unsigned long long) ((u64) R * (u64) P)); return VDJX_ELIMIT; }
	u32 tmask = 1023;
	while ((size_t) tmask + 1 < (size_t) ns * 2) tmask = tmask * 2 + 1;
	unsigned long long* pred;
	ulonglong2* table;
	u32 *succ0, *succ, *bloom, *clen, *coff, *csum, *csum_start, *newidx, *jump_open, *fbw, *gcnt2, *bestsucc, *partner = nullptr;
	u64 *pd, *lo2, *hi2, *gfirst2, *linw;
	ulonglong2 *skey0, *skey;
	u32 bloom_bits = 1u << 16;
	while (bloom_bits < (1u << 30) && (size_t) bloom_bits < (size_t) ns * 16) bloom_bits <<= 1;
	const u32 nb16 = (ns + 15u) >> 4;
	const u32 n_scan = (ns + SCAN_BLOCK - 1) / SCAN_BLOCK;
	const u32 n_jump = (ceil_log2_u64((u64) ns + 1) + 4) / 5 + 1;
	{
		auto up = [](size_t b) { return (b + 255) & ~(size_t) 255; };
		const size_t b_bloom = up(bloom_bits / 8), b_table = up(((size_t) tmask + 1) * 16), b_pred = up((size_t) ns * 8), b_clen = up((size_t) ns * 4),
		             b_jump = up((size_t) (n_jump + 1) * 4), b_linw = up(((size_t) nb16 + 1) * 8);
		uint8_t* z;
		const size_t zb = b_bloom + b_table + b_pred + b_clen + b_jump + b_linw;
		HIP_TRY(db.alloc(&z, zb));
		HIP_TRY(hipMemsetAsync(z, 0, zb, st));
		table = (ulonglong2*) z; z += b_table;
		bloom = (u32*) z; z += b_bloom;
		pred = (unsigned long long*) z; z += b_pred;
		clen = (u32*) z; z += b_clen;
		jump_open = (u32*) z; z += b_jump;
		linw = (u64*) z;
	}
	HIP_TRY(db.alloc(&skey0, ns)); HIP_TRY(db.alloc(&skey, ns));
	HIP_TRY(db.alloc(&succ0, (size_t) ns * 4)); HIP_TRY(db.alloc(&succ, (size_t) ns * 4));
	HIP_TRY(db.alloc(&pd, ns)); HIP_TRY(db.alloc(&coff, ns));
	HIP_TRY(db.alloc(&csum, n_scan)); HIP_TRY(db.alloc(&csum_start, n_scan + 1)); HIP_TRY(db.alloc(&newidx, ns));
	HIP_TRY(db.alloc(&lo2, ns)); HIP_TRY(db.alloc(&hi2, ns)); HIP_TRY(db.alloc(&gcnt2, ns)); HIP_TRY(db.alloc(&gfirst2, ns));
	HIP_TRY(db.alloc(&fbw, nb16));
	HIP_TRY(db.alloc(&bestsucc, ns));
	if (sym_walk) HIP_TRY(db.alloc(&partner, ns));
	const SurvTable tb0{table, tmask, skey0, bloom, bloom_bits - 1};
	const SurvTable tb{table, tmask, skey, bloom, bloom_bits - 1};
	if (table_out) *table_out = tb;
	const dim3 gs((ns + 255) / 256), bs(256);
	{
		vdjx_prof_scope ps(c, "k_surv_table");
		hipLaunchKernelGGL(k_surv_table2, gs, bs, 0, st, sv.lo, sv.hi, ns, table, tmask, skey0, bloom, bloom_bits - 1);
		hipLaunchKernelGGL(k_succ_links2, gs, bs, 0, st, tb0, ns, k, sv.gcnt, succ0, pred, bestsucc);
	}
	{
		vdjx_prof_scope ps(c, "k_chain_order");
		hipLaunchKernelGGL(k_chain_init, gs, bs, 0, st, pred, bestsucc, ns, pd);
		for (u32 j = 0; j < n_jump; j++) hipLaunchKernelGGL(k_chain_jump, gs, bs, 0, st, pd, ns, j ? jump_open + j - 1 : (const u32*) nullptr, jump_open + j);
		hipLaunchKernelGGL(k_chain_len, gs, bs, 0, st, pd, ns, clen);
		hipLaunchKernelGGL(k_scan_sums, dim3(n_scan), dim3(256), 0, st, clen, ns, csum);
		hipLaunchKernelGGL(k_bucket_scan, dim3(1), dim3(1024), 0, st, csum, n_scan, csum_start);
		hipLaunchKernelGGL(k_scan_apply, dim3(n_scan), dim3(256), 0, st, clen, ns, csum_start, coff);
		hipLaunchKernelGGL(k_chain_place, gs, bs, 0, st, pd, coff, ns, newidx);
		hipLaunchKernelGGL(k_chain_permute, gs, bs, 0, st, newidx, ns, sv.lo, sv.hi, sv.gcnt, sv.gfirst, succ0, lo2, hi2, gcnt2, gfirst2, skey, succ);
		hipLaunchKernelGGL(k_table_remap, dim3(tmask / 256 + 1), bs, 0, st, table, tmask + 1, newidx);
		if (sym_walk) hipLaunchKernelGGL(k_partner, gs, bs, 0, st, tb, ns, k, partner);
		hipLaunchKernelGGL(k_chain_words, gs, bs, 0, st, succ, skey, ns, k, linw, fbw, (const u32*) partner);
	}
	dbg_sync(c, "k_chain_order");
	if (sync_debug()) {
		std::vector<u32> ni(ns), seen(ns, 0);
		(void) hipMemcpy(ni.data(), newidx, (size_t) ns * 4, hipMemcpyDeviceToHost);
		u32 dup = 0, oob = 0;
		for (u32 i = 0; i < ns; i++) { if (ni[i] >= ns) oob++; else if (seen[ni[i]]++) dup++; }
		std::vector<u64> pdh(ns);
		std::vector<unsigned long long> prh(ns);
		(void) hipMemcpy(pdh.data(), pd, (size_t) ns * 8, hipMemcpyDeviceToHost);
		(void) hipMemcpy(prh.data(), pred, (size_t) ns * 8, hipMemcpyDeviceToHost);
		u32 unresolved = 0;
		for (u32 i = 0; i < ns; i++) { const u32 p0 = (u32) (pdh[i] >> 32); if (p0 != NONE32 && (u32) (pdh[p0] >> 32) != NONE32) unresolved++; }
		fprintf(stderr, "[vdjx] chain order: %u survivors, %u duplicate new indices, %u out of range, %u unresolved (cycles), %u jump launches\n", ns, dup, oob, unresolved, n_jump);
		for (u32 i = 0, shown = 0; i < ns && shown < 6; i++) if (ni[i] < ns && seen[ni[i]] > 1) {
			fprintf(stderr, "[vdjx]   old %u -> new %u: pd = (%u, %u), pred word %llx\n", i, ni[i], (u32) (pdh[i] >> 32), (u32) pdh[i], prh[i]);
			shown++;
		}
	}
	sv.lo = lo2; sv.hi = hi2; sv.gcnt = gcnt2; sv.gfirst = gfirst2;
	ItemFmt f;
	{
		const u32 sb = ceil_log2_u64(ns);
		static const u32 force_lb = (u32) vdjx_env_num("VDJX_RC_LEN_BITS", 4, 0, 4);
		const u32 lb = std::min(std::min(4u, 26u - sb), force_lb);
		const u32 pb = 26u - lb;
		f.pmask = (1u << pb) - 1u;
		f.len_shift = IT_SURV_SHIFT + pb;
		f.maxlen = 1u << lb;
		const u32 t = ceil_log2_u64(nb16);
		f.bmask = (1u << t) - 1u;
		f.mul = t ? ((0x9E3779B9u >> (32 - t)) | 1u) : 1u;
		u32 x = f.mul;
		for (int i = 0; i < 5; i++) x *= 2u - f.mul * x;
		f.inv = x & f.bmask;
		f.ns = ns;
	}
	const u32 nsp = (f.bmask + 1u) << 4;
	static const bool force_wide = vdjx_env_num("VDJX_RC_WIDE", 0, 0, 1) != 0;
	static const u32 cap_shift = (u32) vdjx_env_num("VDJX_RC_MAX_SHIFT", 12, 8, 12);
	const bool narrow = R < (1ull << (32 - pool->ob)) && !force_wide;
	static const u32 max_ranges = (u32) vdjx_env_num("VDJX_RC_MAX_RANGES", PART_MAXB, 2, PART_MAXB);
	const u32 max_shift = std::max(8u, std::min(narrow ? 11u : 10u, cap_shift));
	u32 range_shift = 8;
	while (range_shift < max_shift && (nsp >> range_shift) > max_ranges) range_shift++;
	const u32 n_ranges = std::max(1u, nsp >> range_shift);
	u32 l2bits = 0;
	while (((n_ranges + (1u << l2bits) - 1) >> l2bits) > max_ranges) l2bits++;
	if (l2bits) l2bits = std::min(10u, std::max(l2bits, (ceil_log2_u64(n_ranges) + 1u) / 2u));
	const u32 n_coarse = (n_ranges + (1u << l2bits) - 1) >> l2bits;
	const u32 n_ranges_p = n_coarse << l2bits;
	constexpr size_t walk_blocks = 7168;
	const size_t Rw = sym_walk ? R / 2 : R;
	u32 nblk = (u32) std::min<size_t>(walk_blocks, (Rw + WALK_THREADS * 8 - 1) / (WALK_THREADS * 8));
	constexpr u32 walk_resident = 1536;
	if (nblk > walk_resident && nblk < walk_blocks) nblk = nblk / walk_resident * walk_resident;
	if (nblk < walk_resident) nblk = (u32) std::min<size_t>(walk_resident, (Rw + WALK_THREADS - 1) / WALK_THREADS);
	if (nblk == 0) nblk = 1;
	const size_t nwaves = (size_t) nblk * (WALK_THREADS / 64);
	const size_t NI = R * (size_t) P;
	u32 blk_items = 4096;
	while (blk_items > 256 && nwaves * blk_items > NI / 2 + 65536) blk_items >>= 1;
	const u64 raw_cap = (u64) NI + (u64) NI / (blk_items / 64) + nwaves * (u64) blk_items + blk_items;
	u64 *raw, *items;
	unsigned long long *g_cursor, *n_inst;
	u32 *range_cnt, *range_start, *g_err, *gcur;
	const vdjx_arena::mark_t tmp_mark = db.mark();
	HIP_TRY(db.alloc(&raw, (size_t) raw_cap));
	HIP_TRY(db.alloc(&g_cursor, 4 + ((size_t) n_ranges_p + 1) / 2));
	n_inst = g_cursor + 1;
	g_err = (u32*) (g_cursor + 2);
	range_cnt = (u32*) (g_cursor + 4);
	HIP_TRY(db.alloc(&range_start, n_ranges_p + 1));
	HIP_TRY(hipMemsetAsync(g_cursor, 0, 32 + (size_t) n_ranges_p * 4, st));
	if (sym_walk) {
		vdjx_prof_scope ps(c, "k_chain_order");
		hipLaunchKernelGGL(k_partner_check, gs, bs, 0, st, partner, linw, ns, g_err + 3);
	}
	const bool lng = pool->W > 2;
	if (lng && R >= (1ull << 27)) { vdjx_set_error("more than 2^27 records of long reads on one GPU: not supported by the recount items"); return VDJX_ELIMIT; }
	const size_t lds_walk = (((size_t) n_ranges_p + 1) & ~(size_t) 1) * 4 + (lng ? (size_t) WALK_THREADS * GL_ROW_LONG * 8 : 0);
	if ((size_t) n_ranges_p * 4 > 64 * 1024) { vdjx_set_error("too many survivor ranges for the walk histogram"); return VDJX_ELIMIT; }
	HIP_TRY(hipFuncSetAttribute((const void*) k_walk_items<false>, hipFuncAttributeMaxDynamicSharedMemorySize, (int) lds_walk));
	HIP_TRY(hipFuncSetAttribute((const void*) k_walk_items<true>, hipFuncAttributeMaxDynamicSharedMemorySize, (int) lds_walk));
	HIP_TRY(hipFuncSetAttribute((const void*) k_walk_items<false, true>, hipFuncAttributeMaxDynamicSharedMemorySize, (int) lds_walk));
#ifdef VDJX_ABLATE
	static const u32 walk_dbg = (u32) vdjx_env_num("VDJX_WALK_DBG", 0, 0, 63);
#else
	constexpr u32 walk_dbg = 0;
#endif
	if (R && walk_dbg != 0u) {
		u64* raw2;
		unsigned long long* cur2;
		u32* cnt2;
		HIP_TRY(db.alloc(&raw2, (size_t) raw_cap));
		HIP_TRY(db.alloc(&cur2, 8));
		HIP_TRY(db.alloc(&cnt2, n_ranges_p));
		HIP_TRY(hipMemsetAsync(cur2, 0, 64, st));
		HIP_TRY(hipMemsetAsync(cnt2, 0, (size_t) n_ranges_p * 4, st));
		vdjx_prof_scope ps(c, "k_walk_dbg");
		if (lng) hipLaunchKernelGGL(k_walk_items<true>, dim3(nblk), dim3(WALK_THREADS), lds_walk, st, pool->d_bases, pool->d_nmask, R, pool->rl, pool->ob, k, tb, succ, linw, f, range_shift,
		                            n_ranges_p, raw2, raw_cap, blk_items, cur2, cnt2, g_err, walk_dbg, (const u32*) nullptr);
		else hipLaunchKernelGGL(k_walk_items<false>, dim3(nblk), dim3(WALK_THREADS), lds_walk, st, pool->d_bases, pool->d_nmask, R, pool->rl, pool->ob, k, tb, succ, linw, f, range_shift,
		                        n_ranges_p, raw2, raw_cap, blk_items, cur2, cnt2, g_err, walk_dbg, (const u32*) nullptr);
		HIP_TRY(hipMemsetAsync(g_err, 0, 4, st));
		if (walk_dbg & 32u) {
			unsigned long long hs[8];
			HIP_TRY(hipMemcpyAsync(hs, cur2, 64, hipMemcpyDeviceToHost, st));
			HIP_TRY(hipStreamSynchronize(st));
			const char* nm[] = {"", "rows", "rounds", "filter", "lookup", "chain", "item_trips"};
			for (int i = 1; i < 7; i++) c->stats[std::string("walk_dbg_") + nm[i]] = hs[i];
		}
	}
	if (R) {
		vdjx_prof_scope ps(c, "k_walk_items");
		if (lng) hipLaunchKernelGGL(k_walk_items<true>, dim3(nblk), dim3(WALK_THREADS), lds_walk, st, pool->d_bases, pool->d_nmask, R, pool->rl, pool->ob, k, tb, succ, linw, f, range_shift,
		                            n_ranges_p, raw, raw_cap, blk_items, g_cursor, range_cnt, g_err, 0u, (const u32*) nullptr);
		else if (sym_walk) hipLaunchKernelGGL((k_walk_items<false, true>), dim3(nblk), dim3(WALK_THREADS), lds_walk, st, pool->d_bases, pool->d_nmask, R / 2, pool->rl, pool->ob, k, tb, succ, linw, f, range_shift,
		                                      n_ranges_p, raw, raw_cap, blk_items, g_cursor, range_cnt, g_err, 0u, (const u32*) partner);
		else hipLaunchKernelGGL(k_walk_items<false>, dim3(nblk), dim3(WALK_THREADS), lds_walk, st, pool->d_bases, pool->d_nmask, R, pool->rl, pool->ob, k, tb, succ, linw, f, range_shift,
		                        n_ranges_p, raw, raw_cap, blk_items, g_cursor, range_cnt, g_err, 0u, (const u32*) nullptr);
	}
	dbg_sync(c, "k_walk_items");
	hipLaunchKernelGGL(k_bucket_scan, dim3(1), dim3(1024), 0, st, range_cnt, n_ranges_p, range_start);
	size_t items_cap = NI + 1;
	if (!defer) {
		u32* hp = (u32*) c->h_pin;
		HIP_TRY(hipMemcpyAsync(hp, range_start + n_ranges_p, 4, hipMemcpyDeviceToHost, st));
		HIP_TRY(hipStreamSynchronize(st));
		HIP_TRY(hipGetLastError());
		items_cap = (size_t) hp[0] + 1;
	}
	HIP_TRY(db.alloc(&items, items_cap));
	HIP_TRY(hipFuncSetAttribute((const void*) k_part_items, hipFuncAttributeMaxDynamicSharedMemorySize, PART_LDS_BYTES));
	HIP_TRY(db.alloc(&gcur, n_ranges_p));
	{
		vdjx_prof_scope ps(c, "k_part_items");
		u32 npb = (u32) std::min<size_t>(1024, (NI / 4 + 65535) / 65536);
		if (npb == 0) npb = 1;
		if (!l2bits) {
			hipLaunchKernelGGL(k_init_cursors, dim3((n_ranges_p + 255) / 256), dim3(256), 0, st, range_start, n_ranges_p, 0u, gcur);
			hipLaunchKernelGGL(k_part_items, dim3(npb), dim3(PART_THREADS), PART_LDS_BYTES, st, raw, g_cursor, f, range_shift, n_ranges_p, gcur, items);
		} else {
			u64* l1;
			u32* gcur1;
			HIP_TRY(db.alloc(&l1, items_cap));
			HIP_TRY(db.alloc(&gcur1, n_coarse));
			HIP_TRY(hipFuncSetAttribute((const void*) k_part_items2, hipFuncAttributeMaxDynamicSharedMemorySize, PART_LDS_BYTES));
			hipLaunchKernelGGL(k_init_cursors, dim3((n_coarse + 255) / 256), dim3(256), 0, st, range_start, n_coarse, l2bits, gcur1);
			hipLaunchKernelGGL(k_part_items, dim3(npb), dim3(PART_THREADS), PART_LDS_BYTES, st, raw, g_cursor, f, range_shift + l2bits, n_coarse, gcur1, l1);
			hipLaunchKernelGGL(k_init_cursors, dim3((n_ranges_p + 255) / 256), dim3(256), 0, st, range_start, n_ranges_p, 0u, gcur);
			const u32 sl2 = std::max(8u, std::min(64u, 2048u / n_coarse));
			hipLaunchKernelGGL(k_part_items2, dim3(n_coarse * sl2), dim3(PART_THREADS), PART_LDS_BYTES, st, l1, range_start, l2bits, sl2, f, range_shift, l2bits, gcur, items);
		}
	}
	dbg_sync(c, "k_part_items");
	{
		vdjx_prof_scope ps(c, "k_recount");
#define RC_LAUNCH(SB, IT) hipLaunchKernelGGL((k_recount<SB, IT>), dim3(n_ranges), dim3(RC_THREADS), 0, st, items, range_start, f, ns, rec_base, pool->ob, fbw, ro.ucnt, ro.ufirst, ro.in_first, n_inst)
		if (narrow) {
			switch (range_shift) {
				case 8: RC_LAUNCH(256, u32); break;
				case 9: RC_LAUNCH(512, u32); break;
				case 10: RC_LAUNCH(1024, u32); break;
				default: RC_LAUNCH(2048, u32); break;
			}
		} else {
			switch (range_shift) {
				case 8: RC_LAUNCH(256, u64); break;
				case 9: RC_LAUNCH(512, u64); break;
				default: RC_LAUNCH(1024, u64); break;
			}
		}
#undef RC_LAUNCH
	}
	dbg_sync(c, "k_recount");
	if (derive_edges) {
		hipLaunchKernelGGL(k_count_unseen, dim3((ns + 255) / 256), dim3(256), 0, st, ro.ufirst, ns, g_err + 1);
		HIP_TRY(hipMemsetAsync(ro.edge_first, 0xFF, (size_t) ns * 32, st));
		hipLaunchKernelGGL(k_edges_from_in, dim3((ns * 4 + 255) / 256), dim3(256), 0, st, tb, ns, k, ro.in_first, ro.in_from, ro.edge_first, ro.edge_to);
	}
	if (defer && !sync_debug()) {
		defer->g_err = g_err; defer->n_items = range_start + n_ranges_p; defer->n_inst = n_inst; defer->ns = ns;
		return VDJX_OK;
	}
	if (defer) defer->g_err = nullptr;
	u32* hp = (u32*) c->h_pin;
	HIP_TRY(hipMemcpyAsync(hp, g_err, 8, hipMemcpyDeviceToHost, st));
	HIP_TRY(hipMemcpyAsync(hp + 2, range_start + n_ranges_p, 4, hipMemcpyDeviceToHost, st));
	HIP_TRY(hipMemcpyAsync(hp + 4, n_inst, 8, hipMemcpyDeviceToHost, st));
	HIP_TRY(hipMemcpyAsync(hp + 6, g_err + 2, 8, hipMemcpyDeviceToHost, st));
	HIP_TRY(hipStreamSynchronize(st));
	HIP_TRY(hipGetLastError());
	if (hp[6] || hp[7]) { vdjx_set_error("the mirrored walk found %u + %u places where the chains are not mirror images", hp[6], hp[7]); return VDJX_ESYMWALK; }
	const u32 err[2] = {hp[0], hp[1]}, n_items = hp[2];
	const unsigned long long inst = *(const unsigned long long*) (hp + 4);
	if (err[0]) { vdjx_set_error("k_walk_items: item buffer too small (%u waves stopped)", err[0]); return VDJX_EHIP; }
	if (err[1]) {
		if (sync_debug()) {
			std::vector<u64> uf(ns), lo(ns), hi(ns), gf(ns);
			std::vector<u32> gc(ns);
			(void) hipMemcpy(uf.data(), ro.ufirst, (size_t) ns * 8, hipMemcpyDeviceToHost);
			(void) hipMemcpy(lo.data(), sv.lo, (size_t) ns * 8, hipMemcpyDeviceToHost);
			(void) hipMemcpy(hi.data(), sv.hi, (size_t) ns * 8, hipMemcpyDeviceToHost);
			(void) hipMemcpy(gf.data(), sv.gfirst, (size_t) ns * 8, hipMemcpyDeviceToHost);
			(void) hipMemcpy(gc.data(), sv.gcnt, (size_t) ns * 4, hipMemcpyDeviceToHost);
			for (u32 i = 0, shown = 0; i < ns && shown < 8; i++) if (uf[i] == NONE64) {
				char txt[65];
				for (int j = 0; j < k; j++) { const int sh = 2 * (k - 1 - j); const u32 c2 = (u32) (sh < 64 ? lo[i] >> sh : hi[i] >> (sh - 64)) & 3u; txt[j] = "ATCG"[c2]; }
				txt[k] = 0;
				fprintf(stderr, "[vdjx] unseen survivor %u: %s gated count %u first gated instance record %llu offset %llu\n", i, txt, gc[i],
				        (unsigned long long) (gf[i] >> 6), (unsigned long long) (gf[i] & 63));
				shown++;
			}
		}
		vdjx_set_error("internal error: %u of %u surviving k-mers were not met again in the records", err[1], ns);
		return VDJX_EHIP;
	}
	c->stats["recount_items"] = n_items;
	c->stats["recount_instances"] = inst;
	db.release_to(tmp_mark);
	return VDJX_OK;
}

template <typename A>
int stage_finish2(vdjx_ctx* c, A& db, const SurvivorsG& sv, const RecountOut& ro, u64 n_records_total, int k, int P, int ob, vdjx_graph* g) {
	hipStream_t st = c->stream;
	const u32 ns = sv.n;
	const u32 nr = sv.n_real <= ns ? sv.n_real : ns;
	g->n = nr;
	g->k = k;
	g->ctx = c;
	g->device = c->device;
	if (ns == 0) return VDJX_OK;
	uint8_t *d_hv, *d_hj;
	HIP_TRY(db.alloc(&d_hv, ns));
	HIP_TRY(db.alloc(&d_hj, ns));
	{
		vdjx_prof_scope ps(c, "k_node_flags");
		hipLaunchKernelGGL(k_node_flags, dim3((ns + 255) / 256), dim3(256), 0, st, sv.lo, sv.hi, ns, k, c->d_vbits, c->d_jbits, d_hv, d_hj);
	}
	u64 *rk_key, *rk_key2;
	u32 *rk_idx, *rk_idx2, *rank;
	HIP_TRY(db.alloc(&rk_key, ns));
	HIP_TRY(db.alloc(&rk_key2, ns));
	HIP_TRY(db.alloc(&rk_idx, ns));
	HIP_TRY(db.alloc(&rk_idx2, ns));
	HIP_TRY(db.alloc(&rank, ns));
	unsigned rk_bits = 1;
	while (rk_bits < 64 && (1ull << rk_bits) <= ((n_records_total << ob) | 1ull)) rk_bits++;
	auto up = [](size_t b) { return (b + 255) & ~(size_t) 255; };
	const size_t need = up((size_t) ns * 8) + 5 * up((size_t) ns * 4) + 4 * up(ns) + 2 * up((size_t) ns * 16) + up((size_t) ns * k);
	{
		hipError_t e = c->blocks.acquire(need, &g->d_block, &g->block_cap);
		if (e != hipSuccess) { vdjx_set_error("graph alloc (%zu bytes): %s", need, hipGetErrorString(e)); return VDJX_EHIP; }
	}
	char* bp = g->d_block;
	auto carve = [&](size_t b) { char* r = bp; bp += up(b); return r; };
	NodeOut no;
	no.klo = no.khi = nullptr;
	no.first_inst = g->d_first_inst = (u64*) carve((size_t) ns * 8);
	no.gcnt = g->d_gcnt = (u32*) carve((size_t) ns * 4);
	no.freq = g->d_freq = (u32*) carve((size_t) ns * 4);
	no.to_ids = g->d_to_ids = (u32*) carve((size_t) ns * 16);
	no.from_ids = g->d_from_ids = (u32*) carve((size_t) ns * 16);
	no.hv = g->d_hv = (uint8_t*) carve(ns);
	no.hj = g->d_hj = (uint8_t*) carve(ns);
	no.to_deg = g->d_to_deg = (uint8_t*) carve(ns);
	no.from_deg = g->d_from_deg = (uint8_t*) carve(ns);
	no.kmers = g->d_kmers = carve((size_t) ns * k);
	g->export_bytes = (size_t) (bp - g->d_block);
	g->d_roots = (u32*) carve((size_t) ns * 4);
	{
		vdjx_prof_scope ps(c, "k_node_order");
		hipLaunchKernelGGL(k_rank_keys, dim3((ns + 255) / 256), dim3(256), 0, st, sv.ufirst, sv.gcnt, ns, rk_key, rk_idx);
		{
			size_t tb = 0;
			int rc_ = vdjx_sort_pairs_raw(nullptr, &tb, st, rk_key, rk_key2, rk_idx, rk_idx2, ns, rk_bits);
			if (rc_) return rc_;
			char* tmp;
			HIP_TRY(db.alloc(&tmp, tb + 256));
			if ((rc_ = vdjx_sort_pairs_raw(tmp, &tb, st, rk_key, rk_key2, rk_idx, rk_idx2, ns, rk_bits))) return rc_;
		}
		hipLaunchKernelGGL(k_rank_scatter, dim3((ns + 255) / 256), dim3(256), 0, st, rk_key2, rk_idx2, ns, rank);
		hipLaunchKernelGGL(k_node_emit2, dim3((ns + 255) / 256), dim3(256), 0, st, sv.lo, sv.hi, sv.gcnt, sv.ucnt, sv.ufirst, d_hv, d_hj, rank,
		                   ro.edge_first, ro.edge_to, ro.in_first, ro.in_from, ns, k, no);
	}
	u32 n_roots = 0;
	{
		const u32 nrb = (nr + 255) / 256;
		u32 *rb_cnt, *rb_start;
		HIP_TRY(db.alloc(&rb_cnt, nrb + 1));
		HIP_TRY(db.alloc(&rb_start, nrb + 1));
		vdjx_prof_scope ps(c, "k_root_list");
		if (nrb) hipLaunchKernelGGL(k_root_count, dim3(nrb), dim3(256), 0, st, no.from_deg, nr, rb_cnt);
		hipLaunchKernelGGL(k_bucket_scan, dim3(1), dim3(1024), 0, st, rb_cnt, nrb, rb_start);
		if (nrb) hipLaunchKernelGGL(k_root_list, dim3(nrb), dim3(256), 0, st, no.from_deg, nr, rb_start, g->d_roots);
		HIP_TRY(hipMemcpyAsync(c->h_pin, rb_start + nrb, 4, hipMemcpyDeviceToHost, st));
	}
	HIP_TRY(hipStreamSynchronize(st));
	HIP_TRY(hipGetLastError());
	n_roots = *(const u32*) c->h_pin;
	g->n_roots = n_roots;
	vdjx_prof_collect(c, false);
	return VDJX_OK;
}

template <typename TUP>
int kmer_build_impl2(vdjx_ctx* c, const vdjx_pool* pool, int k, int mf, int mq, vdjx_graph* g) {
	const int P = pool->rl - k + 1;
	vdjx_work db(c);
	GTuples<TUP> t;
	const bool sym = build_sym(pool, k);
	c->stats["kmer_build_sym"] = sym ? 1 : 0;
	int rc = stage_gated_partition<TUP>(c, db, pool, 0, k, 0, 0, &t, sym);
	if (rc) return rc;
	PoolView pv{pool->d_bases, pool->d_nmask, vdjx_qrows{pool->d_quals, pool->d_quals2, pool->q_split, pool->qstride}, pool->rl, pool->ob};
	SurvivorsG sv;
	rc = stage_gated_reduce<TUP>(c, db, t, pv, 0, k, mf, mq, &sv, sym);
	if (rc) return rc;
	vdjx_ri_open_gate(c);
	dbg_sync(c, "gated_reduce");
	g->pre_nodes = (size_t) sv.ndist;
	RecountOut ro{};
	if (sv.n) {
		HIP_TRY(db.alloc(&sv.ucnt, sv.n)); HIP_TRY(db.alloc(&sv.ufirst, sv.n));
		HIP_TRY(db.alloc(&ro.in_first, (size_t) sv.n * 4)); HIP_TRY(db.alloc(&ro.in_from, (size_t) sv.n * 4));
		HIP_TRY(db.alloc(&ro.edge_first, (size_t) sv.n * 4)); HIP_TRY(db.alloc(&ro.edge_to, (size_t) sv.n * 4));
		ro.ucnt = sv.ucnt; ro.ufirst = sv.ufirst;
		for (int attempt = 0; attempt < 2; attempt++) {
			const bool sym_walk = sym && sym_walk_wanted() && attempt == 0;
			c->stats["kmer_build_sym_walk"] = sym_walk ? 1 : 0;
			RecountStatus rs;
			rc = stage_recount(c, db, pool, 0, k, sv, ro, true, nullptr, &rs, sym_walk);
			if (rc == VDJX_ESYMWALK && sym_walk) { c->stats["kmer_build_sym_walk_retries"] += 1; continue; }
			if (rc) return rc;
			u32* hp = (u32*) c->h_pin + 1024;
			hp[6] = hp[7] = 0;
			if (rs.g_err) {
				HIP_TRY(hipMemcpyAsync(hp + 8, rs.n_inst, 24, hipMemcpyDeviceToHost, c->stream));
				HIP_TRY(hipMemcpyAsync(hp + 2, rs.n_items, 4, hipMemcpyDeviceToHost, c->stream));
			}
			rc = stage_finish2(c, db, sv, ro, pool->n_records, k, P, pool->ob, g);
			if (rc) return rc;
			if (rs.g_err) { hp[4] = hp[8]; hp[5] = hp[9]; hp[0] = hp[10]; hp[1] = hp[11]; hp[6] = hp[12]; hp[7] = hp[13]; }
			rc = rs.g_err ? recount_status_check(c, hp, rs.ns) : VDJX_OK;
			if (rc != VDJX_ESYMWALK || !sym_walk) return rc == VDJX_ESYMWALK ? VDJX_EHIP : rc;
			c->stats["kmer_build_sym_walk_retries"] += 1;
			if (g->d_block) { c->blocks.release(g->d_block, g->block_cap); g->d_block = nullptr; g->block_cap = 0; }
		}
		return VDJX_EHIP;
	}
	return stage_finish2(c, db, sv, ro, pool->n_records, k, P, pool->ob, g);
}

}

extern "C" int vdjx_kmer_build(vdjx_ctx* c, const vdjx_pool* pool, int k, int mf, int mq, vdjx_graph** out) {
	if (!c || !pool || !out) { vdjx_set_error("vdjx_kmer_build: NULL argument"); return VDJX_EINVAL; }
	*out = nullptr;
	if (pool->ctx != c) { vdjx_set_error("vdjx_kmer_build: pool belongs to another context"); return VDJX_EINVAL; }
	if (k < 1 || k > VDJX_MAX_KMER || k > pool->rl) { vdjx_set_error("k=%d outside [1,min(%d,rl=%d)]", k, VDJX_MAX_KMER, pool->rl); return VDJX_ELIMIT; }
	if (k > 16 && !c->anchors_loaded) { vdjx_set_error("vdjx_kmer_build: call vdjx_anchor_sets_load first (k > 16)"); return VDJX_ESTATE; }
	HIP_TRY(hipSetDevice(c->device));
	vdjx_clear_errors();
	vdjx_graph* g = new vdjx_graph();
	const int rc = k <= 45 ? kmer_build_impl2<Tup16>(c, pool, k, mf, mq, g) : kmer_build_impl2<Tup24>(c, pool, k, mf, mq, g);
	if (rc != VDJX_OK) { vdjx_graph_free(g); return rc; }
	*out = g;
	return VDJX_OK;
}

struct vdjx_shard {
	vdjx_ctx* c = nullptr;
	const vdjx_pool* pool = nullptr;
	int k = 0, mf = 0, mq = 0, rank = 0, nranks = 1;
	u64 rec_stride = 0;
	const u32* scan = nullptr;
	u64 total_records = 0;
	u64 rec_base() const { return scan ? 0 : rec_stride * (u64) rank; }
	u64 records_in_all() const { return scan ? total_records : rec_stride * (u64) nranks; }
	bool sym_capable = false, sym = false;
	bool wide = false;
	u32 NBf = 0, NBo = 0;
	u32 *nd = nullptr, *dstart = nullptr;
	Partial* dense = nullptr;
	u32* dense_ref = nullptr;
	u64* low_inst = nullptr;
	u32 n_dense = 0;
	SurvivorsG local_sv, all_sv;
	u32 sv_cap = 0;
	u32* n_surv = nullptr;
	PendOut po{};
	u32 n_pend = 0;
	uint2* queries = nullptr;
	std::vector<u32> src_base, nq;
	u32 *p_fl = nullptr, *p_S = nullptr, *p_r0 = nullptr;
	u32 mqq = 0, tlow = 0;
	SurvTable tb{};
	int phase = 0;
	bool have_hist = false;
	GatedHist gh;
	u64 agreed = 0;
	Partial* sparse = nullptr;
	u32* sparse_ref = nullptr;
	vdjx_arena::mark_t fill_mark{0, 0};
	const u32* tuple_bucket_start = nullptr;
	u32 NBt = 0;
};

static int shard_begin_impl(vdjx_ctx* c, const vdjx_pool* pool, int k, int mf, int mq, int rank, int nranks,
                            uint64_t rec_stride, const uint32_t* d_scan, uint64_t total_records, vdjx_shard** out) {
	if (!c || !pool || !out) { vdjx_set_error("vdjx_shard_begin: NULL argument"); return VDJX_EINVAL; }
	*out = nullptr;
	if (c->live_shard) { vdjx_set_error("vdjx_shard_begin: a sharded build is already in flight on this context"); return VDJX_ESTATE; }
	if (nranks < 1 || nranks > 256 || rank < 0 || rank >= nranks) { vdjx_set_error("1 <= nranks <= 256, 0 <= rank < nranks"); return VDJX_EINVAL; }
	if (k < 1 || k > VDJX_MAX_KMER || k > pool->rl) { vdjx_set_error("k=%d outside [1,min(%d,rl=%d)]", k, VDJX_MAX_KMER, pool->rl); return VDJX_ELIMIT; }
	if (d_scan) {
		if (total_records < pool->n_records) { vdjx_set_error("total_records %llu < local records %zu", (unsigned long long) total_records, pool->n_records); return VDJX_EINVAL; }
		if (total_records >= (1ull << 32) || total_records >= (1ull << (INST_BITS - pool->ob))) { vdjx_set_error("global record count %llu: scan positions are 32 bits and instance ids record << %d | offset in %d bits", (unsigned long long) total_records, pool->ob, INST_BITS); return VDJX_ELIMIT; }
		rec_stride = (total_records + (uint64_t) nranks - 1) / (uint64_t) nranks;
	} else {
		if (rec_stride < pool->n_records) { vdjx_set_error("rec_stride %llu < local records %zu", (unsigned long long) rec_stride, pool->n_records); return VDJX_EINVAL; }
		if (rec_stride * (uint64_t) nranks >= (1ull << (INST_BITS - pool->ob))) { vdjx_set_error("global record count %llu >= 2^%d (instance ids are record << %d | offset in %d bits)", (unsigned long long) (rec_stride * nranks), INST_BITS - pool->ob, pool->ob, INST_BITS); return VDJX_ELIMIT; }
	}
	if (k > 16 && !c->anchors_loaded) { vdjx_set_error("vdjx_shard_begin: call vdjx_anchor_sets_load first (k > 16)"); return VDJX_ESTATE; }
	if (pool->W > 2 && pool->n_records >= (1ull << 27)) { vdjx_set_error("more than 2^27 records of long reads on one GPU: not supported by the recount items"); return VDJX_ELIMIT; }
	vdjx_shard* s = new vdjx_shard();
	s->c = c; s->pool = pool; s->k = k; s->mf = mf; s->mq = mq; s->rank = rank; s->nranks = nranks;
	s->rec_stride = rec_stride;
	s->scan = d_scan; s->total_records = total_records;
	s->sym_capable = build_sym(pool, k) && s->rec_base() % 2 == 0;
	s->wide = k > 45;
	if (mq >= 255) mq = 254;
	s->mqq = (u32) (mq < 0 ? 0 : (mq > 214 ? 214 : mq));
	s->tlow = 1 + (s->mqq + 19) / 20;
	c->live_shard = s;
	*out = s;
	return VDJX_OK;
}

extern "C" int vdjx_shard_begin(vdjx_ctx* c, const vdjx_pool* pool, int k, int mf, int mq, int rank, int nranks,
                                uint64_t rec_stride, vdjx_shard** out) {
	return shard_begin_impl(c, pool, k, mf, mq, rank, nranks, rec_stride, nullptr, 0, out);
}

extern "C" int vdjx_shard_begin_share(vdjx_ctx* c, const vdjx_pool* pool, int k, int mf, int mq, int rank, int nranks,
                                      const uint32_t* d_scan_index, uint64_t total_records, vdjx_shard** out) {
	if (pool && pool->n_records && !d_scan_index) { vdjx_set_error("vdjx_shard_begin_share: NULL scan index"); return VDJX_EINVAL; }
	static const uint32_t none = 0;
	return shard_begin_impl(c, pool, k, mf, mq, rank, nranks, 0, d_scan_index ? d_scan_index : &none, total_records, out);
}

extern "C" void vdjx_shard_free(vdjx_shard* s) {
	if (!s) return;
	(void) hipSetDevice(s->c->device);
	(void) hipStreamSynchronize(s->c->stream);
	s->c->shard_arena.reset();
	s->c->live_shard = nullptr;
	delete s;
}

extern "C" size_t vdjx_shard_record_bytes(int kind) {
	return kind == 0 ? sizeof(Partial) : kind == 1 ? sizeof(uint2) : kind == 2 ? REPLY_BYTES : kind == 3 ? sizeof(SurvRec) : 0;
}

static u64 shard_geometry_bound(const vdjx_shard* s) {
	const int P = s->pool->rl - s->k + 1;
	return std::max<u64>(1, s->rec_stride * (u64) P / 4);
}

template <typename TUP>
static int shard_local_impl(vdjx_shard* s) {
	vdjx_ctx* c = s->c;
	hipStream_t st = c->stream;
	PersistAlloc db(c);
	const u64 rec_base = s->rec_base();
	GTuples<TUP> t;
	int rc = VDJX_OK;
	if (s->have_hist && s->gh.sym != s->sym) s->have_hist = false;
	const size_t per_b = 0;
	if (!s->have_hist) rc = stage_gated_hist(c, db, s->pool, s->k, per_b, shard_geometry_bound(s) / (s->sym ? 2 : 1), &s->gh, s->sym);
	if (rc) return rc;
	s->have_hist = true;
	const size_t cap = (size_t) s->gh.N + 1;
	const size_t nb_max = ((size_t) 1 << 20) + 16 * (size_t) s->nranks + 2;
	Partial* sparse;
	u32 *g_err, *sparse_ref;
	HIP_TRY(db.alloc(&s->low_inst, cap));
	HIP_TRY(db.alloc(&s->dense_ref, cap));
	HIP_TRY(db.alloc(&s->nd, nb_max));
	HIP_TRY(db.alloc(&s->dstart, nb_max + 1));
	HIP_TRY(db.alloc(&g_err, 1));
	u32* keep_starts;
	HIP_TRY(db.alloc(&keep_starts, nb_max + 1));
	s->fill_mark = db.mark();
	HIP_TRY(db.alloc(&sparse, cap));
	HIP_TRY(db.alloc(&sparse_ref, cap));
	const vdjx_arena::mark_t tuple_mark = db.mark();
	rc = stage_gated_cut<TUP>(c, db, s->pool, rec_base, s->k, per_b, (s->agreed ? s->agreed : shard_geometry_bound(s)) / (s->sym ? 2 : 1), s->gh, &t);
	if (rc) return rc;
	if (t.NB < (u32) s->nranks) { vdjx_set_error("vdjx_shard_local: fewer buckets (%u) than ranks", t.NB); return VDJX_ELIMIT; }
	s->NBo = t.NB / (u32) s->nranks;
	if (s->NBo * (u32) s->nranks != t.NB) s->NBo = (s->NBo + 1 + 15) & ~15u;
	s->NBf = s->NBo * (u32) s->nranks;
	if ((size_t) s->NBf + 1 > nb_max) { vdjx_set_error("vdjx_shard_local: %u buckets", s->NBf); return VDJX_ELIMIT; }
	HIP_TRY(hipMemsetAsync(g_err, 0, 4, st));
	if (s->NBf > t.NB) HIP_TRY(hipMemsetAsync(s->nd + t.NB, 0, (size_t) (s->NBf - t.NB) * 4, st));
	if ((rc = set_sub_tuples(c))) return rc;
	{
		vdjx_prof_scope ps(c, "k_gated_local");
		u32* order;
		if ((rc = bucket_order(c, db, t, &order))) return rc;
		if (s->sym) hipLaunchKernelGGL((k_gated_local<TUP, true>), dim3(t.NB), dim3(LG_THREADS), 0, st, t.t, t.bucket_start, s->pool->d_bases, s->pool->d_nmask, rec_base,
		                               s->k, s->pool->rl, s->pool->ob, s->tlow, sparse, sparse_ref, s->nd, s->low_inst, g_err, (const u32*) order);
		else hipLaunchKernelGGL(k_gated_local<TUP>, dim3(t.NB), dim3(LG_THREADS), 0, st, t.t, t.bucket_start, s->pool->d_bases, s->pool->d_nmask, rec_base,
		                        s->k, s->pool->rl, s->pool->ob, s->tlow, sparse, sparse_ref, s->nd, s->low_inst, g_err, (const u32*) order);
	}
	hipLaunchKernelGGL(k_bucket_scan, dim3(1), dim3(1024), 0, st, s->nd, s->NBf, s->dstart);
	u32* d_pick;
	const u32 G = (u32) s->nranks;
	HIP_TRY(db.alloc(&d_pick, G + 1));
	hipLaunchKernelGGL(k_pick_u32, dim3(1), dim3(512), 0, st, s->dstart, s->NBo, G + 1, d_pick);
	std::vector<u32> pick(G + 1);
	u32 err = 0;
	HIP_TRY(hipMemcpyAsync(pick.data(), d_pick, (G + 1) * 4, hipMemcpyDeviceToHost, st));
	HIP_TRY(hipMemcpyAsync(&err, g_err, 4, hipMemcpyDeviceToHost, st));
	HIP_TRY(hipMemcpyAsync(keep_starts, t.bucket_start, ((size_t) t.NB + 1) * 4, hipMemcpyDeviceToDevice, st));
	HIP_TRY(hipStreamSynchronize(st));
	HIP_TRY(hipGetLastError());
	if (err) { vdjx_set_error("k_gated_local: %u buckets could not be split to fit LDS", err); return VDJX_EHIP; }
	s->src_base.assign(pick.begin(), pick.end());
	s->n_dense = pick[G];
	s->sparse = sparse; s->sparse_ref = sparse_ref; s->NBt = t.NB;
	s->dense = nullptr;
	db.release_to(tuple_mark);
	s->tuple_bucket_start = keep_starts;
	return VDJX_OK;
}

extern "C" int vdjx_shard_local(vdjx_shard* s, uint64_t* send_counts, uint32_t* dir_len) {
	if (!s || !send_counts || !dir_len) { vdjx_set_error("vdjx_shard_local: NULL argument"); return VDJX_EINVAL; }
	if (s->phase != 0) { vdjx_set_error("vdjx_shard_local: already called"); return VDJX_ESTATE; }
	HIP_TRY(hipSetDevice(s->c->device));
	vdjx_clear_errors();
	int rc = s->wide ? shard_local_impl<Tup24>(s) : shard_local_impl<Tup16>(s);
	if (rc) return rc;
	vdjx_ri_open_gate(s->c);
	for (int g = 0; g < s->nranks; g++) send_counts[g] = s->src_base[g + 1] - s->src_base[g];
	*dir_len = s->NBo;
	s->phase = 1;
	return VDJX_OK;
// ... 120 lines not shown
	c->stats["shard_open_kmers"] = np;
	c->stats["shard_decided_at_merge"] = ns;
	{
		u64 nqs = 0;
		for (u32 q : s->nq) nqs += q;
		c->stats["shard_questions"] = nqs;
	}
	v.n = ns;
	v.ndist = ndist;
	for (u32 g = 0; g < G; g++) query_counts[g] = s->nq[g];
	const size_t sides = s->sym ? 2 : 1;
	HIP_TRY(db.alloc(&s->p_fl, (size_t) np + 1));
	HIP_TRY(db.alloc(&s->p_r0, sides * np + 1));
	HIP_TRY(db.alloc(&s->p_S, sides * np * 64 + 1));
	if (np) {
		HIP_TRY(hipMemsetAsync(s->p_fl, 0, (size_t) np * 4, st));
		HIP_TRY(hipMemsetAsync(s->p_r0, 0xFF, sides * np * 4, st));
		HIP_TRY(hipMemsetAsync(s->p_S, 0, sides * np * 256, st));
	}
	return VDJX_OK;
}

extern "C" int vdjx_shard_merge(vdjx_shard* s, const void* d_recv_dir, const void* d_recv_partials, const uint64_t* recv_counts,
                                uint64_t* query_counts) {
	if (!s || !recv_counts || !query_counts || !d_recv_dir) { vdjx_set_error("vdjx_shard_merge: NULL argument"); return VDJX_EINVAL; }
	if (s->phase != 1) { vdjx_set_error("vdjx_shard_merge: call vdjx_shard_local first (once)"); return VDJX_ESTATE; }
	uint64_t tot = 0;
	for (int g = 0; g < s->nranks; g++) tot += recv_counts[g];
	if (tot >= (1ull << 30)) { vdjx_set_error("vdjx_shard_merge: too many partial aggregates for one owner (%llu): use more ranks", (unsigned long long) tot); return VDJX_ELIMIT; }
	if (tot && !d_recv_partials) { vdjx_set_error("vdjx_shard_merge: NULL buffer"); return VDJX_EINVAL; }
	HIP_TRY(hipSetDevice(s->c->device));
	vdjx_clear_errors();
	int rc = s->wide ? shard_merge_impl<u64>(s, (const u32*) d_recv_dir, (const Partial*) d_recv_partials, recv_counts, query_counts)
	                 : shard_merge_impl<u32>(s, (const u32*) d_recv_dir, (const Partial*) d_recv_partials, recv_counts, query_counts);
	if (rc) return rc;
	s->phase = 2;
	return VDJX_OK;
}

extern "C" int vdjx_shard_queries(vdjx_shard* s, void* d_out) {
	if (!s || s->phase < 2) { vdjx_set_error("vdjx_shard_queries: call vdjx_shard_merge first"); return VDJX_ESTATE; }
	HIP_TRY(hipSetDevice(s->c->device));
	vdjx_clear_errors();
	hipStream_t st = s->c->stream;
	size_t at = 0;
	for (int g = 0; g < s->nranks; g++) {
		if (!s->nq[g]) continue;
		if (!d_out) { vdjx_set_error("vdjx_shard_queries: NULL buffer"); return VDJX_EINVAL; }
		HIP_TRY(hipMemcpyAsync((uint2*) d_out + at, s->queries + s->src_base[g], (size_t) s->nq[g] * sizeof(uint2), hipMemcpyDeviceToDevice, st));
		at += s->nq[g];
	}
	HIP_TRY(hipStreamSynchronize(st));
	return VDJX_OK;
}

extern "C" int vdjx_shard_reply(vdjx_shard* s, const void* d_queries, const uint64_t* counts, void* d_replies) {
	if (!s || !counts) { vdjx_set_error("vdjx_shard_reply: NULL argument"); return VDJX_EINVAL; }
	if (s->phase < 1 || (s->n_dense && !s->dense)) { vdjx_set_error("vdjx_shard_reply: call vdjx_shard_local and vdjx_shard_local_fill first"); return VDJX_ESTATE; }
	vdjx_ctx* c = s->c;
	HIP_TRY(hipSetDevice(c->device));
	vdjx_clear_errors();
	const u32 G = (u32) s->nranks;
	std::vector<u32> off(G + 1, 0);
	for (u32 g = 0; g < G; g++) off[g + 1] = off[g] + (u32) counts[g];
	const u32 nq = off[G];
	if (!nq) return VDJX_OK;
	if (!d_queries || !d_replies) { vdjx_set_error("vdjx_shard_reply: NULL buffer"); return VDJX_EINVAL; }
	PersistAlloc db(c);
	u32* d_off;
	HIP_TRY(db.alloc(&d_off, G + 1));
	hipStream_t st = c->stream;
	HIP_TRY(hipMemcpyAsync(d_off, off.data(), (G + 1) * 4, hipMemcpyHostToDevice, st));
	const vdjx_pool* p = s->pool;
	{
		vdjx_prof_scope ps(c, "k_shard_reply");
		if (s->sym) hipLaunchKernelGGL(k_shard_reply<true>, dim3(nq), dim3(64), 0, st, (const uint2*) d_queries, nq, d_off, G, s->dense, s->dense_ref, s->dstart, s->NBo,
		                               s->low_inst, p->d_bases, p->d_nmask, vdjx_qrows{p->d_quals, p->d_quals2, p->q_split, p->qstride}, s->rec_base(), s->scan, (u32) p->n_records, s->k, p->rl, p->ob, (uint8_t*) d_replies);
		else hipLaunchKernelGGL(k_shard_reply<false>, dim3(nq), dim3(64), 0, st, (const uint2*) d_queries, nq, d_off, G, s->dense, s->dense_ref, s->dstart, s->NBo,
		                        s->low_inst, p->d_bases, p->d_nmask, vdjx_qrows{p->d_quals, p->d_quals2, p->q_split, p->qstride}, s->rec_base(), s->scan, (u32) p->n_records, s->k, p->rl, p->ob, (uint8_t*) d_replies);
	}
	HIP_TRY(hipStreamSynchronize(st));
	HIP_TRY(hipGetLastError());
	return VDJX_OK;
}

extern "C" int vdjx_shard_resolve(vdjx_shard* s, const void* d_replies, uint64_t n_replies, uint64_t* n_survivors, uint64_t* n_distinct) {
	if (!s || !n_survivors || !n_distinct) { vdjx_set_error("vdjx_shard_resolve: NULL argument"); return VDJX_EINVAL; }
	if (s->phase != 2) { vdjx_set_error("vdjx_shard_resolve: call vdjx_shard_merge first (once)"); return VDJX_ESTATE; }
	uint64_t expect = 0;
	for (u32 q : s->nq) expect += q;
	if (n_replies != expect) { vdjx_set_error("vdjx_shard_resolve: %llu answers for %llu questions", (unsigned long long) n_replies, (unsigned long long) expect); return VDJX_EINVAL; }
	vdjx_ctx* c = s->c;
	HIP_TRY(hipSetDevice(c->device));
	vdjx_clear_errors();
	hipStream_t st = c->stream;
	SurvivorsG& v = s->local_sv;
	if (s->n_pend) {
		if (!d_replies) { vdjx_set_error("vdjx_shard_resolve: NULL buffer"); return VDJX_EINVAL; }
		const u32 nr = (u32) n_replies;
		SurvOutG so{v.lo, v.hi, v.gcnt, v.gfirst, s->n_surv, s->sv_cap, nullptr};
		vdjx_prof_scope ps(c, "k_shard_resolve");
		hipLaunchKernelGGL(k_resolve_first, dim3((nr + 255) / 256), dim3(256), 0, st, (const uint8_t*) d_replies, nr, s->po.mg, s->p_r0, (const u64*) s->po.mgr, s->n_pend);
		hipLaunchKernelGGL(k_resolve_add, dim3((nr + 3) / 4), dim3(256), 0, st, (const uint8_t*) d_replies, nr, s->p_r0, s->k, s->p_fl, s->p_S, s->sym ? s->n_pend : 0u);
		if (s->sym) hipLaunchKernelGGL(k_resolve_keep<true>, dim3((s->n_pend + 255) / 256), dim3(256), 0, st, s->po, s->n_pend, s->p_fl, s->p_S, s->k,
		                               (u32) std::max(s->mf, 0), s->mqq, s->tlow, so);
		else hipLaunchKernelGGL(k_resolve_keep<false>, dim3((s->n_pend + 255) / 256), dim3(256), 0, st, s->po, s->n_pend, s->p_fl, s->p_S, s->k,
		                        (u32) std::max(s->mf, 0), s->mqq, s->tlow, so);
	}
	u32 ns = 0;
	HIP_TRY(hipMemcpyAsync(&ns, s->n_surv, 4, hipMemcpyDeviceToHost, st));
	HIP_TRY(hipStreamSynchronize(st));
	HIP_TRY(hipGetLastError());
	c->stats["shard_kept_after_answers"] = ns - v.n;
	v.n = ns;
	*n_survivors = ns;
	*n_distinct = v.ndist;
	s->phase = 3;
	return VDJX_OK;
}

extern "C" int vdjx_shard_survivors(vdjx_shard* s, void* d_out) {
	if (!s || s->phase < 3) { vdjx_set_error("vdjx_shard_survivors: call vdjx_shard_resolve first"); return VDJX_ESTATE; }
	const SurvivorsG& v = s->local_sv;
	if (!v.n) return VDJX_OK;
	if (!d_out) { vdjx_set_error("vdjx_shard_survivors: NULL buffer"); return VDJX_EINVAL; }
	HIP_TRY(hipSetDevice(s->c->device));
	vdjx_clear_errors();
	hipLaunchKernelGGL(k_surv_pack, dim3((v.n + 255) / 256), dim3(256), 0, s->c->stream, v.lo, v.hi, v.gcnt, v.gfirst, v.n, (SurvRec*) d_out);
	HIP_TRY(hipStreamSynchronize(s->c->stream));
	HIP_TRY(hipGetLastError());
	return VDJX_OK;
}

extern "C" int vdjx_shard_edges(vdjx_shard* s, const void* d_surv_all, uint64_t ns_total, void* d_in_first, void* d_ucnt, void* d_ufirst) {
	if (!s || s->phase < 3) { vdjx_set_error("vdjx_shard_edges: call vdjx_shard_resolve first"); return VDJX_ESTATE; }
	if (ns_total >= (1ull << 26)) { vdjx_set_error("vdjx_shard_edges: too many survivors"); return VDJX_ELIMIT; }
	vdjx_ctx* c = s->c;
	HIP_TRY(hipSetDevice(c->device));
	vdjx_clear_errors();
	PersistAlloc db(c);
	SurvivorsG& a = s->all_sv;
	a.n = (u32) ns_total;
	a.n_real = a.n;
	s->phase = 4;
	if (!ns_total) return VDJX_OK;
	if (!d_surv_all || !d_in_first || !d_ucnt || !d_ufirst) { vdjx_set_error("vdjx_shard_edges: NULL buffer"); return VDJX_EINVAL; }
	HIP_TRY(db.alloc(&a.lo, a.n)); HIP_TRY(db.alloc(&a.hi, a.n)); HIP_TRY(db.alloc(&a.gcnt, a.n)); HIP_TRY(db.alloc(&a.gfirst, a.n));
	u32* d_nreal;
	HIP_TRY(db.alloc(&d_nreal, 1));
	HIP_TRY(hipMemsetAsync(d_nreal, 0, 4, c->stream));
	hipLaunchKernelGGL(k_surv_unpack, dim3((a.n + 255) / 256), dim3(256), 0, c->stream, (const SurvRec*) d_surv_all, a.n, a.lo, a.hi, a.gcnt, a.gfirst, d_nreal);
	u32* h_nreal = (u32*) c->h_pin + 1536;
	HIP_TRY(hipMemcpyAsync(h_nreal, d_nreal, 4, hipMemcpyDeviceToHost, c->stream));
	RecountOut ro{(u32*) d_ucnt, (u64*) d_ufirst, (u64*) d_in_first, nullptr, nullptr, nullptr};
	const bool sym_walk = s->sym && sym_walk_wanted();
	c->stats["kmer_build_sym_walk"] = sym_walk ? 1 : 0;
	const SurvivorsG a_in = a;
	int rc = stage_recount(c, db, s->pool, s->rec_base(), s->k, a, ro, false, &s->tb, nullptr, sym_walk);
	if (rc == VDJX_ESYMWALK && sym_walk) {
		c->stats["kmer_build_sym_walk_retries"] += 1;
		a = a_in;
		rc = stage_recount(c, db, s->pool, s->rec_base(), s->k, a, ro, false, &s->tb, nullptr, false);
	}
	if (rc == VDJX_OK) a.n_real = *h_nreal;
	if (rc || !s->scan) return rc == VDJX_ESYMWALK ? VDJX_EHIP : rc;
	hipLaunchKernelGGL(k_first_to_scan, dim3((a.n * 5 + 255) / 256), dim3(256), 0, c->stream, (u64*) d_in_first, (size_t) a.n * 4, (u64*) d_ufirst, (size_t) a.n, s->scan, s->pool->ob);
	HIP_TRY(hipStreamSynchronize(c->stream));
	HIP_TRY(hipGetLastError());
	return VDJX_OK;
}

extern "C" int vdjx_shard_finish(vdjx_shard* s, const void* d_in_first, const void* d_ucnt, const void* d_ufirst,
                                 uint64_t pre_nodes_total, vdjx_graph** out) {
	if (!s || !out || s->phase < 4) { vdjx_set_error("vdjx_shard_finish: call vdjx_shard_edges first"); return VDJX_ESTATE; }
	*out = nullptr;
	vdjx_ctx* c = s->c;
	HIP_TRY(hipSetDevice(c->device));
	vdjx_clear_errors();
	PersistAlloc db(c);
	const int P = s->pool->rl - s->k + 1;
	SurvivorsG& a = s->all_sv;
	RecountOut ro{};
	if (a.n) {
		if (!d_ucnt || !d_ufirst || !d_in_first) { vdjx_set_error("vdjx_shard_finish: NULL buffer"); return VDJX_EINVAL; }
		a.ucnt = (u32*) d_ucnt;
		a.ufirst = (u64*) d_ufirst;
		ro.ucnt = a.ucnt; ro.ufirst = a.ufirst; ro.in_first = (u64*) d_in_first;
		HIP_TRY(db.alloc(&ro.in_from, (size_t) a.n * 4));
		HIP_TRY(db.alloc(&ro.edge_first, (size_t) a.n * 4));
		HIP_TRY(db.alloc(&ro.edge_to, (size_t) a.n * 4));
		HIP_TRY(hipMemsetAsync(ro.edge_first, 0xFF, (size_t) a.n * 32, c->stream));
		hipLaunchKernelGGL(k_edges_from_in, dim3((a.n * 4 + 255) / 256), dim3(256), 0, c->stream, s->tb, a.n, s->k, ro.in_first, ro.in_from, ro.edge_first, ro.edge_to);
	}
	vdjx_graph* g = new vdjx_graph();
	g->pre_nodes = (size_t) pre_nodes_total;
	int rc = stage_finish2(c, db, a, ro, s->records_in_all(), s->k, P, s->pool->ob, g);
	if (rc) { vdjx_graph_free(g); return rc; }
	*out = g;
	return VDJX_OK;
}

extern "C" size_t vdjx_graph_nodes(const vdjx_graph* g) { return g ? g->n : 0; }
extern "C" size_t vdjx_graph_pre_nodes(const vdjx_graph* g) { return g ? g->pre_nodes : 0; }
extern "C" size_t vdjx_graph_roots(const vdjx_graph* g) { return g ? g->n_roots : 0; }

static int graph_export_on(const vdjx_graph* g, hipStream_t st, uint64_t* first_inst, uint32_t* gated_count, uint32_t* freq, uint8_t* has_v,
                           uint8_t* has_j, uint8_t* to_deg, uint32_t* to_ids, uint8_t* from_deg, uint32_t* from_ids, char* kmers) {
	const size_t n = g->n;
	if (first_inst) HIP_TRY(hipMemcpyAsync(first_inst, g->d_first_inst, n * 8, hipMemcpyDeviceToHost, st));
	if (gated_count) HIP_TRY(hipMemcpyAsync(gated_count, g->d_gcnt, n * 4, hipMemcpyDeviceToHost, st));
	if (freq) HIP_TRY(hipMemcpyAsync(freq, g->d_freq, n * 4, hipMemcpyDeviceToHost, st));
	if (has_v) HIP_TRY(hipMemcpyAsync(has_v, g->d_hv, n, hipMemcpyDeviceToHost, st));
	if (has_j) HIP_TRY(hipMemcpyAsync(has_j, g->d_hj, n, hipMemcpyDeviceToHost, st));
	if (to_deg) HIP_TRY(hipMemcpyAsync(to_deg, g->d_to_deg, n, hipMemcpyDeviceToHost, st));
	if (from_deg) HIP_TRY(hipMemcpyAsync(from_deg, g->d_from_deg, n, hipMemcpyDeviceToHost, st));
	if (to_ids) HIP_TRY(hipMemcpyAsync(to_ids, g->d_to_ids, n * 16, hipMemcpyDeviceToHost, st));
	if (from_ids) HIP_TRY(hipMemcpyAsync(from_ids, g->d_from_ids, n * 16, hipMemcpyDeviceToHost, st));
	if (kmers) HIP_TRY(hipMemcpyAsync(kmers, g->d_kmers, n * (size_t) g->k, hipMemcpyDeviceToHost, st));
	return VDJX_OK;
}

extern "C" int vdjx_graph_export(const vdjx_graph* g, uint64_t* first_inst, uint32_t* gated_count, uint32_t* freq,
                                 uint8_t* has_v, uint8_t* has_j, uint8_t* to_deg, uint32_t* to_ids,
                                 uint8_t* from_deg, uint32_t* from_ids, char* kmers) {
	if (!g) { vdjx_set_error("vdjx_graph_export: NULL graph"); return VDJX_EINVAL; }
	if (g->n == 0) return VDJX_OK;
	if (!g->d_block || !vdjx_ctx_alive(g->ctx)) { vdjx_set_error("vdjx_graph_export: the graph's context is gone"); return VDJX_ESTATE; }
	HIP_TRY(hipSetDevice(g->device));
	int rc = graph_export_on(g, g->ctx->stream, first_inst, gated_count, freq, has_v, has_j, to_deg, to_ids, from_deg, from_ids, kmers);
	if (rc) return rc;
	HIP_TRY(hipStreamSynchronize(g->ctx->stream));
	return VDJX_OK;
}

extern "C" int vdjx_graph_export_begin(const vdjx_graph* g, uint64_t* first_inst, uint32_t* gated_count, uint32_t* freq,
                                       uint8_t* has_v, uint8_t* has_j, uint8_t* to_deg, uint32_t* to_ids,
                                       uint8_t* from_deg, uint32_t* from_ids, char* kmers) {
	if (!g) { vdjx_set_error("vdjx_graph_export_begin: NULL graph"); return VDJX_EINVAL; }
	if (g->n == 0) return VDJX_OK;
	if (!g->d_block || !vdjx_ctx_alive(g->ctx)) { vdjx_set_error("vdjx_graph_export_begin: the graph's context is gone"); return VDJX_ESTATE; }
	HIP_TRY(hipSetDevice(g->device));
	return graph_export_on(g, g->ctx->copy_stream, first_inst, gated_count, freq, has_v, has_j, to_deg, to_ids, from_deg, from_ids, kmers);
}

extern "C" int vdjx_graph_block_layout(const vdjx_graph* g, uint64_t* offsets, uint64_t* bytes) {
	if (!g || !offsets || !bytes) { vdjx_set_error("vdjx_graph_block_layout: NULL argument"); return VDJX_EINVAL; }
	const char* b = g->d_block;
	const void* at[10] = {g->d_first_inst, g->d_gcnt, g->d_freq, g->d_hv, g->d_hj, g->d_to_deg, g->d_to_ids, g->d_from_deg, g->d_from_ids, g->d_kmers};
	for (int i = 0; i < 10; i++) offsets[i] = g->n ? (uint64_t) ((const char*) at[i] - b) : 0;
	*bytes = g->n ? g->export_bytes : 0;
	return VDJX_OK;
}
static int graph_block_on(const vdjx_graph* g, bool copy_stream, void* host_block, const char* who) {
	if (!g) { vdjx_set_error("%s: NULL graph", who); return VDJX_EINVAL; }
	if (g->n == 0) return VDJX_OK;
	if (!host_block) { vdjx_set_error("%s: NULL buffer", who); return VDJX_EINVAL; }
	if (!g->d_block || !vdjx_ctx_alive(g->ctx)) { vdjx_set_error("%s: the graph's context is gone", who); return VDJX_ESTATE; }
	HIP_TRY(hipSetDevice(g->device));
	HIP_TRY(hipMemcpyAsync(host_block, g->d_block, g->export_bytes, hipMemcpyDeviceToHost, copy_stream ? g->ctx->copy_stream : g->ctx->stream));
	return VDJX_OK;
}
extern "C" int vdjx_graph_export_block(const vdjx_graph* g, void* host_block) {
	const int rc = graph_block_on(g, false, host_block, "vdjx_graph_export_block");
	if (rc || !g || g->n == 0) return rc;
	HIP_TRY(hipStreamSynchronize(g->ctx->stream));
	return VDJX_OK;
}
extern "C" int vdjx_graph_export_block_begin(const vdjx_graph* g, void* host_block) {
	return graph_block_on(g, true, host_block, "vdjx_graph_export_block_begin");
}

extern "C" int vdjx_graph_export_end(const vdjx_graph* g) {
	if (!g) { vdjx_set_error("vdjx_graph_export_end: NULL graph"); return VDJX_EINVAL; }
	if (!vdjx_ctx_alive(g->ctx)) { vdjx_set_error("vdjx_graph_export_end: the graph's context is gone"); return VDJX_ESTATE; }
	HIP_TRY(hipSetDevice(g->device));
	HIP_TRY(hipStreamSynchronize(g->ctx->copy_stream));
	return VDJX_OK;
}

extern "C" void vdjx_graph_free(vdjx_graph* g) {
	if (!g) return;
	if (g->d_block) {
		(void) hipSetDevice(g->device);
		if (vdjx_ctx_alive(g->ctx)) {
			(void) hipStreamSynchronize(g->ctx->copy_stream);
			g->ctx->blocks.release(g->d_block, g->block_cap);
		}
		else (void) hipFree(g->d_block);
	}
	delete g;
}
```

Baseline: 922.7.

## Fold partner lookup, table remap and edge derivation into existing chain kernels

After: 931.9, median of 6. Within noise of the previous version (+1.0%).

```diff
diff --git a/profiles/summarize_pmc.py b/profiles/summarize_pmc.py
--- a/profiles/summarize_pmc.py
+++ b/profiles/summarize_pmc.py
@@ -35,8 +35,7 @@
 
 COMPOSITES = {
     "k_surv_table": ("k_surv_table2", "k_succ_links2"),
-    "k_chain_order": ("k_chain_init", "k_chain_jump", "k_chain_len", "k_scan_sums", "k_scan_apply", "k_chain_place", "k_chain_permute", "k_table_remap",
-                      "k_partner", "k_chain_words", "k_partner_check"),
+    "k_chain_order": ("k_chain_init", "k_chain_jump", "k_chain_len", "k_scan_sums", "k_scan_apply", "k_chain_place", "k_chain_permute", "k_chain_words"),
     "k_node_order": ("k_rank_keys", "k_rank_scatter", "k_node_emit2"),
     "k_shard_resolve": ("k_resolve_first", "k_resolve_add", "k_resolve_keep"),
 }
diff --git a/vdjer_amd/csrc/vdjx_kmer.hip b/vdjer_amd/csrc/vdjx_kmer.hip
--- a/vdjer_amd/csrc/vdjx_kmer.hip
+++ b/vdjer_amd/csrc/vdjx_kmer.hip
@@ -1308,13 +1308,14 @@
 	if (v != NONE64) *p = ((u64) scan[v >> ob] << ob) | (v & ((1ull << ob) - 1ull));
 }
 
-__global__ void k_node_flags(const u64* __restrict__ s_lo, const u64* __restrict__ s_hi, u32 n, int k,
+__global__ void k_node_flags(const ulonglong2* __restrict__ skey, u32 n, int k,
                              const u32* __restrict__ vbits, const u32* __restrict__ jbits,
                              uint8_t* __restrict__ has_v, uint8_t* __restrict__ has_j) {
 	u32 i = blockIdx.x * blockDim.x + threadIdx.x;
 	if (i >= n) return;
 	if (k <= 16) { has_v[i] = 1; has_j[i] = 1; return; }
-	u128 key = ((u128) s_hi[i] << 64) | s_lo[i];
+	const ulonglong2 kk = skey[i];
+	u128 key = ((u128) kk.y << 64) | kk.x;
 	u32 code = (u32) (key >> (2 * (k - 16)));
 	has_v[i] = code ? (vbits[code >> 5] >> (code & 31)) & 1u : 0;
 	has_j[i] = code ? (jbits[code >> 5] >> (code & 31)) & 1u : 0;
@@ -1345,7 +1346,7 @@
 __device__ inline u32 it_scat(const ItemFmt& f, u32 p) { return ((((p >> 4) * f.mul) & f.bmask) << 4) | (p & 15u); }
 
 __global__ void k_surv_table2(const u64* __restrict__ s_lo, const u64* __restrict__ s_hi, u32 n, ulonglong2* __restrict__ slots, u32 mask,
-                              ulonglong2* __restrict__ skey, u32* __restrict__ bloom, u32 bloom_mask) {
+                              ulonglong2* __restrict__ skey, u32* __restrict__ bloom, u32 bloom_mask, u32* __restrict__ slot_of) {
 	const u32 i = blockIdx.x * blockDim.x + threadIdx.x;
 	if (i >= n) return;
 	const u64 lo = s_lo[i], hi = s_hi[i];
@@ -1359,6 +1360,7 @@
 	const unsigned long long entry = hi | ((unsigned long long) (i + 1) << SLOT_HI_BITS);
 	while (atomicCAS((unsigned long long*) &slots[slot].y, 0ull, entry) != 0ull) slot = (slot + 1) & mask;
 	slots[slot].x = lo;
+	slot_of[i] = slot;
 }
 
 __device__ inline int surv_lookup2f(const SurvTable& t, u64 lo, u64 hi);
@@ -1373,6 +1375,16 @@
 	}
 }
 
+__device__ inline u32 surv_slot2(const SurvTable& t, u64 lo, u64 hi) { return (u32) (vdjx_mix(lo, hi) >> 20) & t.mask; }
+__device__ inline int surv_resolve2(const SurvTable& t, u32 slot, ulonglong2 v, u64 lo, u64 hi) {
+	for (;;) {
+		if (!v.y) return -1;
+		if (v.x == lo && (v.y & SLOT_HI_MASK) == hi) return (int) (v.y >> SLOT_HI_BITS) - 1;
+		slot = (slot + 1) & t.mask;
+		v = t.slots[slot];
+	}
+}
+
 __device__ inline int surv_lookup2f(const SurvTable& t, u64 lo, u64 hi) {
 	const u64 h = vdjx_mix(lo, hi);
 	const u32 bit = (u32) (h >> 40) & t.bloom_mask;
@@ -1381,7 +1393,7 @@
 }
 
 __global__ void k_succ_links2(SurvTable t, u32 n, int k, const u32* __restrict__ gcnt, u32* __restrict__ succ, unsigned long long* __restrict__ pred,
-                              u32* __restrict__ bestsucc) {
+                              u32* __restrict__ bestsucc, u32* __restrict__ partner0) {
 	const u32 u = blockIdx.x * blockDim.x + threadIdx.x;
 	if (u >= n) return;
 	const ulonglong2 kk = t.skey[u];
@@ -1391,9 +1403,23 @@
 	const u32 fb = (u32) (sh < 64 ? kk.x >> sh : kk.y >> (sh - 64)) & 3u;
 	const unsigned long long mine = ((unsigned long long) (gcnt[u] & GC_MASK) << 32) | ((unsigned long long) (fb ^ 1u) << 30) | (unsigned long long) u;
 	u32 best = NONE32, best_g = 0;
+	u64 qlo[5], qhi[5];
+	u32 qslot[5];
+	ulonglong2 qv[5];
 	for (u32 b = 0; b < 4; b++) {
 		const u128 key = (base | (u128) b) & km;
-		const int s = surv_lookup2(t, (u64) key, (u64) (key >> 64));
+		qlo[b] = (u64) key; qhi[b] = (u64) (key >> 64);
+	}
+	const u32 nq = partner0 ? 5u : 4u;
+	qlo[4] = qhi[4] = 0;
+	if (partner0) vdjx_kmer_rc(kk.y, kk.x, k, qhi[4], qlo[4]);
+	for (u32 b = 0; b < 5; b++) if (b < nq) { qslot[b] = surv_slot2(t, qlo[b], qhi[b]); qv[b] = t.slots[qslot[b]]; }
+	if (partner0) {
+		const int q = surv_resolve2(t, qslot[4], qv[4], qlo[4], qhi[4]);
+		partner0[u] = q >= 0 ? (u32) q : NONE32;
+	}
+	for (u32 b = 0; b < 4; b++) {
+		const int s = surv_resolve2(t, qslot[b], qv[b], qlo[b], qhi[b]);
 		succ[u * 4 + b] = s >= 0 ? (u32) s : NONE32;
 		if (s >= 0 && (u32) s != u) {
 			const u32 g = gcnt[s] & GC_MASK;
@@ -1411,25 +1437,6 @@
 	const unsigned long long x = pred[v];
 	const u32 u = (u32) x & 0x3FFFFFFFu;
 	pd[v] = x != 0ull && bestsucc[u] == v ? ((u64) u << 32) | 1ull : ((u64) NONE32 << 32);
-}
-
-__global__ void k_partner(SurvTable t, u32 n, int k, u32* __restrict__ partner) {
-	const u32 p = blockIdx.x * blockDim.x + threadIdx.x;
-	if (p >= n) return;
-	const ulonglong2 kk = t.skey[p];
-	u64 rh, rlo;
-	vdjx_kmer_rc(kk.y, kk.x, k, rh, rlo);
-	const int q = surv_lookup2(t, rlo, rh);
-	partner[p] = q >= 0 ? (u32) q : NONE32;
-}
-__global__ void k_partner_check(const u32* __restrict__ partner, const u64* __restrict__ linw, u32 n, u32* __restrict__ bad) {
-	const u32 p = blockIdx.x * blockDim.x + threadIdx.x;
-	if (p >= n) return;
-	bool wrong = partner[p] == NONE32;
-	const bool linked = (linw[p >> 4] >> (15u - (p & 15u))) & 1ull;
-	if (!wrong && linked && (p + 1 >= n || partner[p + 1] != partner[p] - 1u)) wrong = true;
-	const u64 m = __ballot(wrong);
-	if (m && __lane_id() == 0) atomicAdd(bad, (u32) __popcll(m));
 }
 
 __global__ void k_chain_jump(u64* __restrict__ pd, u32 n, const u32* __restrict__ open_prev, u32* __restrict__ open_now) {
@@ -1460,12 +1467,16 @@
 	if ((u32) (pd[p] >> 32) != NONE32) return;
 	head = p; dist = (u32) x;
 }
-__global__ void k_chain_len(const u64* __restrict__ pd, u32 n, u32* __restrict__ len) {
+__global__ void k_chain_len(const u64* __restrict__ pd, const unsigned long long* __restrict__ pred, const u32* __restrict__ bestsucc, u32 n,
+                            u32* __restrict__ len) {
 	const u32 v = blockIdx.x * blockDim.x + threadIdx.x;
 	if (v >= n) return;
 	u32 h, d;
 	chain_of(pd, v, h, d);
-	atomicAdd(&len[h], 1u);
+	const bool unresolved = h == v && (u32) (pd[v] >> 32) != NONE32;
+	const u32 w = bestsucc[v];
+	const bool tail = w == NONE32 || ((u32) pred[w] & 0x3FFFFFFFu) != v;
+	if (unresolved || tail) len[h] = d + 1u;
 }
 
 #define SCAN_BLOCK 4096u
@@ -1500,15 +1511,21 @@
 	chain_of(pd, v, h, d);
 	newidx[v] = off[h] + d;
 }
-__global__ void k_chain_permute(const u32* __restrict__ newidx, u32 n, const u64* __restrict__ lo, const u64* __restrict__ hi, const u32* __restrict__ gcnt,
-                                const u64* __restrict__ gfirst, const u32* __restrict__ succ, u64* __restrict__ lo2, u64* __restrict__ hi2,
-                                u32* __restrict__ gcnt2, u64* __restrict__ gfirst2, ulonglong2* __restrict__ skey2, u32* __restrict__ succ2) {
+__global__ void k_chain_permute(const u32* __restrict__ newidx, u32 n, int k, const u64* __restrict__ lo, const u64* __restrict__ hi, const u32* __restrict__ gcnt,
+                                const u64* __restrict__ gfirst, const u32* __restrict__ succ, const u32* __restrict__ slot_of, const u32* __restrict__ partner0,
+                                u32* __restrict__ gcnt2, u64* __restrict__ gfirst2, ulonglong2* __restrict__ skey2, u32* __restrict__ succ2,
+                                u32* __restrict__ in_from, ulonglong2* __restrict__ slots, u32* __restrict__ partner) {
 	const u32 v = blockIdx.x * blockDim.x + threadIdx.x;
 	if (v >= n) return;
 	const u32 q = newidx[v];
 	const u64 l = lo[v], h = hi[v];
-	lo2[q] = l; hi2[q] = h; gcnt2[q] = gcnt[v]; gfirst2[q] = gfirst[v];
+	gcnt2[q] = gcnt[v]; gfirst2[q] = gfirst[v];
 	skey2[q] = make_ulonglong2(l, h);
+	slots[slot_of[v]].y = h | ((u64) (q + 1u) << SLOT_HI_BITS);
+	if (partner) {
+		const u32 p0 = partner0[v];
+		partner[q] = p0 == NONE32 ? NONE32 : newidx[p0];
+	}
 	const uint4 s = *(const uint4*) &succ[(size_t) v * 4];
 	uint4 r;
 	r.x = s.x == NONE32 ? NONE32 : newidx[s.x];
@@ -1516,17 +1533,16 @@
 	r.z = s.z == NONE32 ? NONE32 : newidx[s.z];
 	r.w = s.w == NONE32 ? NONE32 : newidx[s.w];
 	*(uint4*) &succ2[(size_t) q * 4] = r;
-}
-__global__ void k_table_remap(ulonglong2* __restrict__ slots, u32 n_slots, const u32* __restrict__ newidx) {
-	const u32 i = blockIdx.x * blockDim.x + threadIdx.x;
-	if (i >= n_slots) return;
-	const u64 y = slots[i].y;
-	if (!y) return;
-	slots[i].y = (y & SLOT_HI_MASK) | ((u64) (newidx[(u32) (y >> SLOT_HI_BITS) - 1] + 1u) << SLOT_HI_BITS);
+	const int sh = 2 * (k - 1);
+	const u32 fb = (u32) (sh < 64 ? l >> sh : h >> (sh - 64)) & 3u;
+	if (r.x != NONE32) in_from[(size_t) r.x * 4 + fb] = q;
+	if (r.y != NONE32) in_from[(size_t) r.y * 4 + fb] = q;
+	if (r.z != NONE32) in_from[(size_t) r.z * 4 + fb] = q;
+	if (r.w != NONE32) in_from[(size_t) r.w * 4 + fb] = q;
 }
 
 __global__ void k_chain_words(const u32* __restrict__ succ, const ulonglong2* __restrict__ skey, u32 n, int k, u64* __restrict__ linw, u32* __restrict__ fbw,
-                              const u32* __restrict__ partner) {
+                              const u32* __restrict__ partner, u32* __restrict__ bad) {
 	const u32 p = blockIdx.x * blockDim.x + threadIdx.x;
 	const u32 j = p & 15u;
 	u64 w = 0;
@@ -1549,6 +1565,10 @@
 		fw |= (u32) __shfl_xor((int) fw, d);
 	}
 	if (j == 0 && p < n) { linw[p >> 4] = w; fbw[p >> 4] = fw; }
+	if (partner) {
+		const u64 m = __ballot(p < n && partner[p] == NONE32);
+		if (m && __lane_id() == 0) atomicAdd(bad, (u32) __popcll(m));
+	}
 }
 
 struct WalkRecS {
@@ -2043,32 +2063,6 @@
 	if (threadIdx.x == 0 && tot) atomicAdd(n_inst, tot);
 }
 
-__global__ void k_count_unseen(const u64* __restrict__ ufirst, u32 n, u32* __restrict__ out) {
-	const u32 i = blockIdx.x * blockDim.x + threadIdx.x;
-	const bool un = i < n && ufirst[i] == NONE64;
-	const u64 m = __ballot(un);
-	if (m && __lane_id() == 0) atomicAdd(out, (u32) __popcll(m));
-}
-
-__global__ void k_edges_from_in(SurvTable t, u32 n, int k, const u64* __restrict__ in_first, u32* __restrict__ in_from,
-                                u64* __restrict__ edge_first, u32* __restrict__ edge_to) {
-	const u32 e = blockIdx.x * blockDim.x + threadIdx.x;
-	if (e >= n * 4u) return;
-	const u64 fs = in_first[e];
-	if (fs == NONE64) { in_from[e] = NONE32; return; }
-	const u32 v = e >> 2, a = e & 3u;
-	const ulonglong2 kk = t.skey[v];
-	const u128 kv = ((u128) kk.y << 64) | kk.x;
-	const u128 ku = (kv >> 2) | ((u128) a << (2 * (k - 1)));
-	const int u = surv_lookup2(t, (u64) ku, (u64) (ku >> 64));
-	in_from[e] = u >= 0 ? (u32) u : NONE32;
-	if (u >= 0) {
-		const u32 oe = (u32) u * 4u + ((u32) kk.x & 3u);
-		edge_first[oe] = fs;
-		edge_to[oe] = v;
-	}
-}
-
 struct SurvRec { u64 lo, hi; u32 gcnt, pad; u64 gfirst; };
 
 __global__ void k_surv_pack(const u64* __restrict__ lo, const u64* __restrict__ hi, const u32* __restrict__ gcnt,
@@ -2096,9 +2090,15 @@
 	uint8_t* to_deg; u32* to_ids; uint8_t* from_deg; u32* from_ids;
 };
 
-__global__ void k_rank_keys(const u64* __restrict__ ufirst, const u32* __restrict__ gcnt, u32 n, u64* __restrict__ key, u32* __restrict__ idx) {
+__global__ void k_rank_keys(const u64* __restrict__ ufirst, const u32* __restrict__ gcnt, u32 n, u64* __restrict__ key, u32* __restrict__ idx,
+                            u32* __restrict__ unseen) {
 	const u32 i = blockIdx.x * blockDim.x + threadIdx.x;
-	if (i < n) { key[i] = (gcnt[i] & GC_SHADOW) ? NONE64 : ufirst[i]; idx[i] = i; }
+	const u64 uf = i < n ? ufirst[i] : 0ull;
+	if (i < n) { key[i] = (gcnt[i] & GC_SHADOW) ? NONE64 : uf; idx[i] = i; }
+	if (unseen) {
+		const u64 m = __ballot(uf == NONE64);
+		if (m && __lane_id() == 0) atomicAdd(unseen, (u32) __popcll(m));
+	}
 }
 __global__ void k_rank_scatter(const u64* __restrict__ key, const u32* __restrict__ idx, u32 n, u32* __restrict__ rank) {
 	const u32 j = blockIdx.x * blockDim.x + threadIdx.x;
@@ -2142,10 +2142,10 @@
 #undef CSW
 }
 
-__global__ void k_node_emit2(const u64* __restrict__ s_lo, const u64* __restrict__ s_hi, const u32* __restrict__ s_gcnt,
+__global__ void k_node_emit2(const ulonglong2* __restrict__ skey, const u32* __restrict__ s_gcnt,
                              const u32* __restrict__ s_ucnt, const u64* __restrict__ s_ufirst, const uint8_t* __restrict__ hv,
-                             const uint8_t* __restrict__ hj, const u32* __restrict__ rank, const u64* __restrict__ edge_first,
-                             const u32* __restrict__ edge_to, const u64* __restrict__ in_first, const u32* __restrict__ in_from,
+                             const uint8_t* __restrict__ hj, const u32* __restrict__ rank, const u32* __restrict__ succ,
+                             const u64* __restrict__ in_first, const u32* __restrict__ in_from,
                              u32 n, int k, NodeOut o) {
 	const u32 s = blockIdx.x * blockDim.x + threadIdx.x;
 	if (s >= n) return;
@@ -2156,17 +2156,21 @@
 	o.freq[r] = s_ucnt[s] > 32765u ? 32765u : s_ucnt[s];
 	o.hv[r] = hv[s];
 	o.hj[r] = hj[s];
-	const u128 key = ((u128) s_hi[s] << 64) | s_lo[s];
+	const ulonglong2 kk2 = skey[s];
+	const u128 key = ((u128) kk2.y << 64) | kk2.x;
 	for (int j = 0; j < k; j++) {
 		const u32 b = (u32) (key >> (2 * (k - 1 - j))) & 3u;
 		o.kmers[(size_t) r * k + j] = b == 0 ? 'A' : (b == 1 ? 'T' : (b == 2 ? 'C' : 'G'));
 	}
 	u64 f[4];
 	u32 id[4];
+	const u32 fb = (u32) (key >> (2 * (k - 1))) & 3u;
+	const uint4 sc = *(const uint4*) &succ[(size_t) s * 4];
+	const u32 to[4] = {sc.x, sc.y, sc.z, sc.w};
 	for (int e = 0; e < 4; e++) {
-		f[e] = edge_first[(size_t) s * 4 + e];
-		if (f[e] != NONE64 && (s_gcnt[edge_to[(size_t) s * 4 + e]] & GC_SHADOW)) f[e] = NONE64;
-		id[e] = f[e] != NONE64 ? rank[edge_to[(size_t) s * 4 + e]] + 1 : 0;
+		f[e] = to[e] != NONE32 ? in_first[(size_t) to[e] * 4 + fb] : NONE64;
+		if (f[e] != NONE64 && (s_gcnt[to[e]] & GC_SHADOW)) f[e] = NONE64;
+		id[e] = f[e] != NONE64 ? rank[to[e]] + 1 : 0;
 	}
 	sort4_desc64(f, id);
 	u32 deg = 0;
@@ -2174,8 +2178,9 @@
 	o.to_deg[r] = (uint8_t) deg;
 	for (int e = 0; e < 4; e++) {
 		f[e] = in_first[(size_t) s * 4 + e];
-		if (f[e] != NONE64 && (in_from[(size_t) s * 4 + e] == NONE32 || (s_gcnt[in_from[(size_t) s * 4 + e]] & GC_SHADOW))) f[e] = NONE64;
-		id[e] = f[e] != NONE64 ? rank[in_from[(size_t) s * 4 + e]] + 1 : 0;
+		const u32 u = f[e] != NONE64 ? in_from[(size_t) s * 4 + e] : NONE32;
+		if (f[e] != NONE64 && (u >= n || (s_gcnt[u] & GC_SHADOW))) f[e] = NONE64;
+		id[e] = f[e] != NONE64 ? rank[u] + 1 : 0;
 	}
 	sort4_desc64(f, id);
 	deg = 0;
@@ -2207,6 +2212,7 @@
 struct SurvivorsG {
 	u64 *lo = nullptr, *hi = nullptr, *gfirst = nullptr, *ufirst = nullptr;
 	u32 *gcnt = nullptr, *ucnt = nullptr;
+	const ulonglong2* skey = nullptr;
 	u32 n = 0, n_real = 0;
 	u64 ndist = 0;
 };
@@ -2225,6 +2231,37 @@
 	return pool->sym && pool->W == 2 && (k & 1) && pool->n_records % 2 == 0;
 }
 static bool sym_walk_wanted() { static const bool on = !vdjx_env_set("VDJX_NO_SYM_WALK"); return on; }
+template <typename TUP> static int part_attrs() {
+	constexpr u32 stage_tuples = PARTR_STAGE_BYTES / (u32) sizeof(TUP);
+	constexpr int lds_partr = (int) (PARTR_STAGE_BYTES + stage_tuples * 4);
+	HIP_TRY(hipFuncSetAttribute((const void*) k_part_records_g<TUP, false>, hipFuncAttributeMaxDynamicSharedMemorySize, lds_partr));
+	HIP_TRY(hipFuncSetAttribute((const void*) k_part_records_g<TUP, true>, hipFuncAttributeMaxDynamicSharedMemorySize, lds_partr));
+	HIP_TRY(hipFuncSetAttribute((const void*) k_part_records_g<TUP, false, true>, hipFuncAttributeMaxDynamicSharedMemorySize, lds_partr));
+	HIP_TRY(hipFuncSetAttribute((const void*) k_part_tuples_g<TUP>, hipFuncAttributeMaxDynamicSharedMemorySize, PART_LDS_BYTES));
+	return VDJX_OK;
+}
+static int kernel_attrs_once(vdjx_ctx* c) {
+	static std::mutex mu;
+	static u64 done = 0;
+	std::lock_guard<std::mutex> lk(mu);
+	const bool tracked = c->device >= 0 && c->device < 64;
+	if (tracked && ((done >> c->device) & 1ull)) return VDJX_OK;
+	constexpr size_t hist_waves = HIST_THREADS / 64;
+	constexpr int lds_hist = (int) std::max<size_t>((4u << 15) + hist_waves * GL_WAVE_BYTES, (4u << 14) + hist_waves * GL_WAVE_BYTES_LONG);
+	constexpr int lds_walk = 64 * 1024 + WALK_THREADS * GL_ROW_LONG * 8;
+	HIP_TRY(hipFuncSetAttribute((const void*) k_gated_hist<false>, hipFuncAttributeMaxDynamicSharedMemorySize, lds_hist));
+	HIP_TRY(hipFuncSetAttribute((const void*) k_gated_hist<true>, hipFuncAttributeMaxDynamicSharedMemorySize, lds_hist));
+	HIP_TRY(hipFuncSetAttribute((const void*) k_gated_hist<false, true>, hipFuncAttributeMaxDynamicSharedMemorySize, lds_hist));
+	HIP_TRY(hipFuncSetAttribute((const void*) k_walk_items<false>, hipFuncAttributeMaxDynamicSharedMemorySize, lds_walk));
+	HIP_TRY(hipFuncSetAttribute((const void*) k_walk_items<true>, hipFuncAttributeMaxDynamicSharedMemorySize, lds_walk));
+	HIP_TRY(hipFuncSetAttribute((const void*) k_walk_items<false, true>, hipFuncAttributeMaxDynamicSharedMemorySize, lds_walk));
+	HIP_TRY(hipFuncSetAttribute((const void*) k_part_items, hipFuncAttributeMaxDynamicSharedMemorySize, PART_LDS_BYTES));
+	HIP_TRY(hipFuncSetAttribute((const void*) k_part_items2, hipFuncAttributeMaxDynamicSharedMemorySize, PART_LDS_BYTES));
+	if (int rc = part_attrs<Tup16>()) return rc;
+	if (int rc = part_attrs<Tup24>()) return rc;
+	if (tracked) done |= 1ull << c->device;
+	return VDJX_OK;
+}
 static size_t gated_bucket_default() { static const size_t v = (size_t) vdjx_env_num("VDJX_GATED_BUCKET", 3072, 1, 1ll << 32); return v; }
 template <typename A>
 int stage_gated_hist(vdjx_ctx* c, A& db, const vdjx_pool* pool, int k, size_t per_bucket, u64 geometry_instances, GatedHist* gh, bool sym = false) {
@@ -2251,9 +2288,7 @@
 	HIP_TRY(hipMemsetAsync(hcnt, 0, (size_t) NBH * 4, st));
 	const bool lng = pool->W > 2;
 	const size_t lds_hist = (size_t) NBH * 4 + (HIST_THREADS / 64) * (lng ? GL_WAVE_BYTES_LONG : GL_WAVE_BYTES);
-	HIP_TRY(hipFuncSetAttribute((const void*) k_gated_hist<false>, hipFuncAttributeMaxDynamicSharedMemorySize, (int) lds_hist));
-	HIP_TRY(hipFuncSetAttribute((const void*) k_gated_hist<true>, hipFuncAttributeMaxDynamicSharedMemorySize, (int) lds_hist));
-	HIP_TRY(hipFuncSetAttribute((const void*) k_gated_hist<false, true>, hipFuncAttributeMaxDynamicSharedMemorySize, (int) lds_hist));
+	if (int rc = kernel_attrs_once(c)) return rc;
 	{
 		vdjx_prof_scope ps(c, "k_gated_hist");
 		if (lng) hipLaunchKernelGGL(k_gated_hist<true>, dim3(nblk), dim3(HIST_THREADS), lds_hist, st, pool->d_bases, pool->d_nmask, pool->d_lowq, R, pool->rl, k, HB, rpb, hcnt, hist_dbg);
@@ -2302,10 +2337,7 @@
 	HIP_TRY(db.alloc(&out->t, (size_t) N + 1));
 	constexpr u32 stage_tuples = PARTR_STAGE_BYTES / (u32) sizeof(TUP);
 	constexpr u32 lds_partr = PARTR_STAGE_BYTES + stage_tuples * 4;
-	HIP_TRY(hipFuncSetAttribute((const void*) k_part_records_g<TUP, false>, hipFuncAttributeMaxDynamicSharedMemorySize, (int) lds_partr));
-	HIP_TRY(hipFuncSetAttribute((const void*) k_part_records_g<TUP, true>, hipFuncAttributeMaxDynamicSharedMemorySize, (int) lds_partr));
-	HIP_TRY(hipFuncSetAttribute((const void*) k_part_records_g<TUP, false, true>, hipFuncAttributeMaxDynamicSharedMemorySize, (int) lds_partr));
-	HIP_TRY(hipFuncSetAttribute((const void*) k_part_tuples_g<TUP>, hipFuncAttributeMaxDynamicSharedMemorySize, PART_LDS_BYTES));
+	if (int rc = kernel_attrs_once(c)) return rc;
 	u32 cbits = Tt, fbits = 0;
 	if (Tt > 10) { cbits = extra ? Tt - 10 : 8; fbits = Tt - cbits; }
 	const u32 NBc = 1u << cbits;
@@ -2428,8 +2460,8 @@
 	return VDJX_OK;
 }
 
-struct RecountOut { u32* ucnt; u64* ufirst; u64* in_first; u32* in_from; u64* edge_first; u32* edge_to; };
-struct RecountStatus { const u32* g_err = nullptr; const u32* n_items = nullptr; const unsigned long long* n_inst = nullptr; u32 ns = 0; };
+struct RecountOut { u32* ucnt; u64* ufirst; u64* in_first; const u32* succ; const u32* in_from; };
+struct RecountStatus { u32* g_err = nullptr; const u32* n_items = nullptr; const unsigned long long* n_inst = nullptr; u32 ns = 0; };
 #define VDJX_ESYMWALK (-1000)
 static int recount_status_check(vdjx_ctx* c, const u32* hp, u32 ns) {
 	if (hp[6] || hp[7]) { vdjx_set_error("the mirrored walk found %u + %u places where the chains are not mirror images", hp[6], hp[7]); return VDJX_ESYMWALK; }
@@ -2440,9 +2472,20 @@
 	return VDJX_OK;
 }
 
+static int recount_status_fetch(vdjx_ctx* c, const RecountStatus& rs, u32* hp) {
+	HIP_TRY(hipMemcpyAsync(hp + 8, rs.n_inst, 24, hipMemcpyDeviceToHost, c->stream));
+	HIP_TRY(hipMemcpyAsync(hp + 2, rs.n_items, 4, hipMemcpyDeviceToHost, c->stream));
+	return VDJX_OK;
+}
+static void recount_status_order(u32* hp) {
+	hp[4] = hp[8]; hp[5] = hp[9];
+	hp[0] = hp[10]; hp[1] = hp[11];
+	hp[6] = hp[12]; hp[7] = hp[13];
+}
+
 template <typename A>
-int stage_recount(vdjx_ctx* c, A& db, const vdjx_pool* pool, u64 rec_base, int k, SurvivorsG& sv, const RecountOut& ro,
-                  bool derive_edges, SurvTable* table_out = nullptr, RecountStatus* defer = nullptr, bool sym_walk = false) {
+int stage_recount(vdjx_ctx* c, A& db, const vdjx_pool* pool, u64 rec_base, int k, SurvivorsG& sv, RecountOut& ro,
+                  bool whole_pool, SurvTable* table_out = nullptr, RecountStatus* defer = nullptr, bool sym_walk = false) {
 	hipStream_t st = c->stream;
 	const size_t R = pool->n_records;
 	const int P = pool->rl - k + 1;
@@ -2454,20 +2497,55 @@
 	while ((size_t) tmask + 1 < (size_t) ns * 2) tmask = tmask * 2 + 1;
 	unsigned long long* pred;
 	ulonglong2* table;
-	u32 *succ0, *succ, *bloom, *clen, *coff, *csum, *csum_start, *newidx, *jump_open, *fbw, *gcnt2, *bestsucc, *partner = nullptr;
-	u64 *pd, *lo2, *hi2, *gfirst2, *linw;
+	u32 *succ0, *succ, *bloom, *clen, *coff, *csum, *csum_start, *newidx, *jump_open, *fbw, *gcnt2, *bestsucc, *slot_of, *in_from, *partner0 = nullptr, *partner = nullptr;
+	u64 *pd, *gfirst2, *linw;
+	unsigned long long *g_cursor, *n_inst;
+	u32 *range_cnt, *g_err;
 	ulonglong2 *skey0, *skey;
 	u32 bloom_bits = 1u << 16;
 	while (bloom_bits < (1u << 30) && (size_t) bloom_bits < (size_t) ns * 16) bloom_bits <<= 1;
 	const u32 nb16 = (ns + 15u) >> 4;
 	const u32 n_scan = (ns + SCAN_BLOCK - 1) / SCAN_BLOCK;
 	const u32 n_jump = (ceil_log2_u64((u64) ns + 1) + 4) / 5 + 1;
+	ItemFmt f;
+	{
+		const u32 sb = ceil_log2_u64(ns);
+		static const u32 force_lb = (u32) vdjx_env_num("VDJX_RC_LEN_BITS", 4, 0, 4);
+		const u32 lb = std::min(std::min(4u, 26u - sb), force_lb);
+		const u32 pb = 26u - lb;
+		f.pmask = (1u << pb) - 1u;
+		f.len_shift = IT_SURV_SHIFT + pb;
+		f.maxlen = 1u << lb;
+		const u32 t = ceil_log2_u64(nb16);
+		f.bmask = (1u << t) - 1u;
+		f.mul = t ? ((0x9E3779B9u >> (32 - t)) | 1u) : 1u;
+		u32 x = f.mul;
+		for (int i = 0; i < 5; i++) x *= 2u - f.mul * x;
+		f.inv = x & f.bmask;
+		f.ns = ns;
+	}
+	const u32 nsp = (f.bmask + 1u) << 4;
+	static const bool force_wide = vdjx_env_num("VDJX_RC_WIDE", 0, 0, 1) != 0;
+	static const u32 cap_shift = (u32) vdjx_env_num("VDJX_RC_MAX_SHIFT", 12, 8, 12);
+	const bool narrow = R < (1ull << (32 - pool->ob)) && !force_wide;
+	static const u32 max_ranges = (u32) vdjx_env_num("VDJX_RC_MAX_RANGES", PART_MAXB, 2, PART_MAXB);
+	const u32 max_shift = std::max(8u, std::min(narrow ? 11u : 10u, cap_shift));
+	u32 range_shift = 8;
+	while (range_shift < max_shift && (nsp >> range_shift) > max_ranges) range_shift++;
+	const u32 n_ranges = std::max(1u, nsp >> range_shift);
+	u32 l2bits = 0;
+	while (((n_ranges + (1u << l2bits) - 1) >> l2bits) > max_ranges) l2bits++;
+	if (l2bits) l2bits = std::min(10u, std::max(l2bits, (ceil_log2_u64(n_ranges) + 1u) / 2u));
+	const u32 n_coarse = (n_ranges + (1u << l2bits) - 1) >> l2bits;
+	const u32 n_ranges_p = n_coarse << l2bits;
+	if ((size_t) n_ranges_p * 4 > 64 * 1024) { vdjx_set_error("too many survivor ranges for the walk histogram"); return VDJX_ELIMIT; }
 	{
 		auto up = [](size_t b) { return (b + 255) & ~(size_t) 255; };
 		const size_t b_bloom = up(bloom_bits / 8), b_table = up(((size_t) tmask + 1) * 16), b_pred = up((size_t) ns * 8), b_clen = up((size_t) ns * 4),
-		             b_jump = up((size_t) (n_jump + 1) * 4), b_linw = up(((size_t) nb16 + 1) * 8);
+		             b_jump = up((size_t) (n_jump + 1) * 4), b_linw = up(((size_t) nb16 + 1) * 8),
+		             b_status = up(32 + (size_t) n_ranges_p * 4);
 		uint8_t* z;
-		const size_t zb = b_bloom + b_table + b_pred + b_clen + b_jump + b_linw;
+		const size_t zb = b_bloom + b_table + b_pred + b_clen + b_jump + b_linw + b_status;
 		HIP_TRY(db.alloc(&z, zb));
 		HIP_TRY(hipMemsetAsync(z, 0, zb, st));
 		table = (ulonglong2*) z; z += b_table;
@@ -2475,38 +2553,43 @@
 		pred = (unsigned long long*) z; z += b_pred;
 		clen = (u32*) z; z += b_clen;
 		jump_open = (u32*) z; z += b_jump;
-		linw = (u64*) z;
-	}
+		linw = (u64*) z; z += b_linw;
+		g_cursor = (unsigned long long*) z;
+	}
+	n_inst = g_cursor + 1;
+	g_err = (u32*) (g_cursor + 2);
+	range_cnt = (u32*) (g_cursor + 4);
 	HIP_TRY(db.alloc(&skey0, ns)); HIP_TRY(db.alloc(&skey, ns));
 	HIP_TRY(db.alloc(&succ0, (size_t) ns * 4)); HIP_TRY(db.alloc(&succ, (size_t) ns * 4));
 	HIP_TRY(db.alloc(&pd, ns)); HIP_TRY(db.alloc(&coff, ns));
 	HIP_TRY(db.alloc(&csum, n_scan)); HIP_TRY(db.alloc(&csum_start, n_scan + 1)); HIP_TRY(db.alloc(&newidx, ns));
-	HIP_TRY(db.alloc(&lo2, ns)); HIP_TRY(db.alloc(&hi2, ns)); HIP_TRY(db.alloc(&gcnt2, ns)); HIP_TRY(db.alloc(&gfirst2, ns));
+	HIP_TRY(db.alloc(&gcnt2, ns)); HIP_TRY(db.alloc(&gfirst2, ns));
+	HIP_TRY(db.alloc(&slot_of, ns)); HIP_TRY(db.alloc(&in_from, (size_t) ns * 4));
+	if (sync_debug()) HIP_TRY(hipMemsetAsync(in_from, 0xFF, (size_t) ns * 16, st));
 	HIP_TRY(db.alloc(&fbw, nb16));
 	HIP_TRY(db.alloc(&bestsucc, ns));
-	if (sym_walk) HIP_TRY(db.alloc(&partner, ns));
+	if (sym_walk) { HIP_TRY(db.alloc(&partner0, ns)); HIP_TRY(db.alloc(&partner, ns)); }
 	const SurvTable tb0{table, tmask, skey0, bloom, bloom_bits - 1};
 	const SurvTable tb{table, tmask, skey, bloom, bloom_bits - 1};
 	if (table_out) *table_out = tb;
 	const dim3 gs((ns + 255) / 256), bs(256);
 	{
 		vdjx_prof_scope ps(c, "k_surv_table");
-		hipLaunchKernelGGL(k_surv_table2, gs, bs, 0, st, sv.lo, sv.hi, ns, table, tmask, skey0, bloom, bloom_bits - 1);
-		hipLaunchKernelGGL(k_succ_links2, gs, bs, 0, st, tb0, ns, k, sv.gcnt, succ0, pred, bestsucc);
+		hipLaunchKernelGGL(k_surv_table2, gs, bs, 0, st, sv.lo, sv.hi, ns, table, tmask, skey0, bloom, bloom_bits - 1, slot_of);
+		hipLaunchKernelGGL(k_succ_links2, gs, bs, 0, st, tb0, ns, k, sv.gcnt, succ0, pred, bestsucc, partner0);
 	}
 	{
 		vdjx_prof_scope ps(c, "k_chain_order");
 		hipLaunchKernelGGL(k_chain_init, gs, bs, 0, st, pred, bestsucc, ns, pd);
 		for (u32 j = 0; j < n_jump; j++) hipLaunchKernelGGL(k_chain_jump, gs, bs, 0, st, pd, ns, j ? jump_open + j - 1 : (const u32*) nullptr, jump_open + j);
-		hipLaunchKernelGGL(k_chain_len, gs, bs, 0, st, pd, ns, clen);
+		hipLaunchKernelGGL(k_chain_len, gs, bs, 0, st, pd, pred, bestsucc, ns, clen);
 		hipLaunchKernelGGL(k_scan_sums, dim3(n_scan), dim3(256), 0, st, clen, ns, csum);
 		hipLaunchKernelGGL(k_bucket_scan, dim3(1), dim3(1024), 0, st, csum, n_scan, csum_start);
 		hipLaunchKernelGGL(k_scan_apply, dim3(n_scan), dim3(256), 0, st, clen, ns, csum_start, coff);
 		hipLaunchKernelGGL(k_chain_place, gs, bs, 0, st, pd, coff, ns, newidx);
-		hipLaunchKernelGGL(k_chain_permute, gs, bs, 0, st, newidx, ns, sv.lo, sv.hi, sv.gcnt, sv.gfirst, succ0, lo2, hi2, gcnt2, gfirst2, skey, succ);
-		hipLaunchKernelGGL(k_table_remap, dim3(tmask / 256 + 1), bs, 0, st, table, tmask + 1, newidx);
-		if (sym_walk) hipLaunchKernelGGL(k_partner, gs, bs, 0, st, tb, ns, k, partner);
-		hipLaunchKernelGGL(k_chain_words, gs, bs, 0, st, succ, skey, ns, k, linw, fbw, (const u32*) partner);
+		hipLaunchKernelGGL(k_chain_permute, gs, bs, 0, st, newidx, ns, k, sv.lo, sv.hi, sv.gcnt, sv.gfirst, succ0, slot_of, partner0, gcnt2, gfirst2, skey, succ,
+		                   in_from, table, partner);
+		hipLaunchKernelGGL(k_chain_words, gs, bs, 0, st, succ, skey, ns, k, linw, fbw, (const u32*) partner, g_err + 3);
 	}
 	dbg_sync(c, "k_chain_order");
 	if (sync_debug()) {
@@ -2526,38 +2609,8 @@
 			shown++;
 		}
 	}
-	sv.lo = lo2; sv.hi = hi2; sv.gcnt = gcnt2; sv.gfirst = gfirst2;
-	ItemFmt f;
-	{
-		const u32 sb = ceil_log2_u64(ns);
-		static const u32 force_lb = (u32) vdjx_env_num("VDJX_RC_LEN_BITS", 4, 0, 4);
-		const u32 lb = std::min(std::min(4u, 26u - sb), force_lb);
-		const u32 pb = 26u - lb;
-		f.pmask = (1u << pb) - 1u;
-		f.len_shift = IT_SURV_SHIFT + pb;
-		f.maxlen = 1u << lb;
-		const u32 t = ceil_log2_u64(nb16);
-		f.bmask = (1u << t) - 1u;
-		f.mul = t ? ((0x9E3779B9u >> (32 - t)) | 1u) : 1u;
-		u32 x = f.mul;
-		for (int i = 0; i < 5; i++) x *= 2u - f.mul * x;
-		f.inv = x & f.bmask;
-		f.ns = ns;
-	}
-	const u32 nsp = (f.bmask + 1u) << 4;
-	static const bool force_wide = vdjx_env_num("VDJX_RC_WIDE", 0, 0, 1) != 0;
-	static const u32 cap_shift = (u32) vdjx_env_num("VDJX_RC_MAX_SHIFT", 12, 8, 12);
-	const bool narrow = R < (1ull << (32 - pool->ob)) && !force_wide;
-	static const u32 max_ranges = (u32) vdjx_env_num("VDJX_RC_MAX_RANGES", PART_MAXB, 2, PART_MAXB);
-	const u32 max_shift = std::max(8u, std::min(narrow ? 11u : 10u, cap_shift));
-	u32 range_shift = 8;
-	while (range_shift < max_shift && (nsp >> range_shift) > max_ranges) range_shift++;
-	const u32 n_ranges = std::max(1u, nsp >> range_shift);
-	u32 l2bits = 0;
-	while (((n_ranges + (1u << l2bits) - 1) >> l2bits) > max_ranges) l2bits++;
-	if (l2bits) l2bits = std::min(10u, std::max(l2bits, (ceil_log2_u64(n_ranges) + 1u) / 2u));
-	const u32 n_coarse = (n_ranges + (1u << l2bits) - 1) >> l2bits;
-	const u32 n_ranges_p = n_coarse << l2bits;
+	sv.lo = sv.hi = nullptr; sv.skey = skey; sv.gcnt = gcnt2; sv.gfirst = gfirst2;
+	ro.succ = succ; ro.in_from = in_from;
 	constexpr size_t walk_blocks = 7168;
 	const size_t Rw = sym_walk ? R / 2 : R;
 	u32 nblk = (u32) std::min<size_t>(walk_blocks, (Rw + WALK_THREADS * 8 - 1) / (WALK_THREADS * 8));
@@ -2571,27 +2624,14 @@
 	while (blk_items > 256 && nwaves * blk_items > NI / 2 + 65536) blk_items >>= 1;
 	const u64 raw_cap = (u64) NI + (u64) NI / (blk_items / 64) + nwaves * (u64) blk_items + blk_items;
 	u64 *raw, *items;
-	unsigned long long *g_cursor, *n_inst;
-	u32 *range_cnt, *range_start, *g_err, *gcur;
+	u32 *range_start, *gcur;
 	const vdjx_arena::mark_t tmp_mark = db.mark();
 	HIP_TRY(db.alloc(&raw, (size_t) raw_cap));
-	HIP_TRY(db.alloc(&g_cursor, 4 + ((size_t) n_ranges_p + 1) / 2));
-	n_inst = g_cursor + 1;
-	g_err = (u32*) (g_cursor + 2);
-	range_cnt = (u32*) (g_cursor + 4);
 	HIP_TRY(db.alloc(&range_start, n_ranges_p + 1));
-	HIP_TRY(hipMemsetAsync(g_cursor, 0, 32 + (size_t) n_ranges_p * 4, st));
-	if (sym_walk) {
-		vdjx_prof_scope ps(c, "k_chain_order");
-		hipLaunchKernelGGL(k_partner_check, gs, bs, 0, st, partner, linw, ns, g_err + 3);
-	}
 	const bool lng = pool->W > 2;
 	if (lng && R >= (1ull << 27)) { vdjx_set_error("more than 2^27 records of long reads on one GPU: not supported by the recount items"); return VDJX_ELIMIT; }
 	const size_t lds_walk = (((size_t) n_ranges_p + 1) & ~(size_t) 1) * 4 + (lng ? (size_t) WALK_THREADS * GL_ROW_LONG * 8 : 0);
-	if ((size_t) n_ranges_p * 4 > 64 * 1024) { vdjx_set_error("too many survivor ranges for the walk histogram"); return VDJX_ELIMIT; }
-	HIP_TRY(hipFuncSetAttribute((const void*) k_walk_items<false>, hipFuncAttributeMaxDynamicSharedMemorySize, (int) lds_walk));
-	HIP_TRY(hipFuncSetAttribute((const void*) k_walk_items<true>, hipFuncAttributeMaxDynamicSharedMemorySize, (int) lds_walk));
-	HIP_TRY(hipFuncSetAttribute((const void*) k_walk_items<false, true>, hipFuncAttributeMaxDynamicSharedMemorySize, (int) lds_walk));
+	if (int rc = kernel_attrs_once(c)) return rc;
 #ifdef VDJX_ABLATE
 	static const u32 walk_dbg = (u32) vdjx_env_num("VDJX_WALK_DBG", 0, 0, 63);
 #else
@@ -2640,7 +2680,6 @@
 		items_cap = (size_t) hp[0] + 1;
 	}
 	HIP_TRY(db.alloc(&items, items_cap));
-	HIP_TRY(hipFuncSetAttribute((const void*) k_part_items, hipFuncAttributeMaxDynamicSharedMemorySize, PART_LDS_BYTES));
 	HIP_TRY(db.alloc(&gcur, n_ranges_p));
 	{
 		vdjx_prof_scope ps(c, "k_part_items");
@@ -2654,7 +2693,6 @@
 			u32* gcur1;
 			HIP_TRY(db.alloc(&l1, items_cap));
 			HIP_TRY(db.alloc(&gcur1, n_coarse));
-			HIP_TRY(hipFuncSetAttribute((const void*) k_part_items2, hipFuncAttributeMaxDynamicSharedMemorySize, PART_LDS_BYTES));
 			hipLaunchKernelGGL(k_init_cursors, dim3((n_coarse + 255) / 256), dim3(256), 0, st, range_start, n_coarse, l2bits, gcur1);
 			hipLaunchKernelGGL(k_part_items, dim3(npb), dim3(PART_THREADS), PART_LDS_BYTES, st, raw, g_cursor, f, range_shift + l2bits, n_coarse, gcur1, l1);
 			hipLaunchKernelGGL(k_init_cursors, dim3((n_ranges_p + 255) / 256), dim3(256), 0, st, range_start, n_ranges_p, 0u, gcur);
@@ -2683,11 +2721,6 @@
 #undef RC_LAUNCH
 	}
 	dbg_sync(c, "k_recount");
-	if (derive_edges) {
-		hipLaunchKernelGGL(k_count_unseen, dim3((ns + 255) / 256), dim3(256), 0, st, ro.ufirst, ns, g_err + 1);
-		HIP_TRY(hipMemsetAsync(ro.edge_first, 0xFF, (size_t) ns * 32, st));
-		hipLaunchKernelGGL(k_edges_from_in, dim3((ns * 4 + 255) / 256), dim3(256), 0, st, tb, ns, k, ro.in_first, ro.in_from, ro.edge_first, ro.edge_to);
-	}
 	if (defer && !sync_debug()) {
 		defer->g_err = g_err; defer->n_items = range_start + n_ranges_p; defer->n_inst = n_inst; defer->ns = ns;
 		return VDJX_OK;
@@ -2701,21 +2734,27 @@
 	HIP_TRY(hipStreamSynchronize(st));
 	HIP_TRY(hipGetLastError());
 	if (hp[6] || hp[7]) { vdjx_set_error("the mirrored walk found %u + %u places where the chains are not mirror images", hp[6], hp[7]); return VDJX_ESYMWALK; }
-	const u32 err[2] = {hp[0], hp[1]}, n_items = hp[2];
+	u32 err[2] = {hp[0], hp[1]};
+	const u32 n_items = hp[2];
 	const unsigned long long inst = *(const unsigned long long*) (hp + 4);
+	std::vector<u64> uf;
+	if (whole_pool && sync_debug()) {
+		uf.resize(ns);
+		(void) hipMemcpy(uf.data(), ro.ufirst, (size_t) ns * 8, hipMemcpyDeviceToHost);
+		for (u32 i = 0; i < ns; i++) err[1] += uf[i] == NONE64;
+	}
 	if (err[0]) { vdjx_set_error("k_walk_items: item buffer too small (%u waves stopped)", err[0]); return VDJX_EHIP; }
 	if (err[1]) {
 		if (sync_debug()) {
-			std::vector<u64> uf(ns), lo(ns), hi(ns), gf(ns);
+			std::vector<u64> gf(ns);
+			std::vector<ulonglong2> kk(ns);
 			std::vector<u32> gc(ns);
-			(void) hipMemcpy(uf.data(), ro.ufirst, (size_t) ns * 8, hipMemcpyDeviceToHost);
-			(void) hipMemcpy(lo.data(), sv.lo, (size_t) ns * 8, hipMemcpyDeviceToHost);
-			(void) hipMemcpy(hi.data(), sv.hi, (size_t) ns * 8, hipMemcpyDeviceToHost);
+			(void) hipMemcpy(kk.data(), skey, (size_t) ns * 16, hipMemcpyDeviceToHost);
 			(void) hipMemcpy(gf.data(), sv.gfirst, (size_t) ns * 8, hipMemcpyDeviceToHost);
 			(void) hipMemcpy(gc.data(), sv.gcnt, (size_t) ns * 4, hipMemcpyDeviceToHost);
 			for (u32 i = 0, shown = 0; i < ns && shown < 8; i++) if (uf[i] == NONE64) {
 				char txt[65];
-				for (int j = 0; j < k; j++) { const int sh = 2 * (k - 1 - j); const u32 c2 = (u32) (sh < 64 ? lo[i] >> sh : hi[i] >> (sh - 64)) & 3u; txt[j] = "ATCG"[c2]; }
+				for (int j = 0; j < k; j++) { const int sh = 2 * (k - 1 - j); const u32 c2 = (u32) (sh < 64 ? kk[i].x >> sh : kk[i].y >> (sh - 64)) & 3u; txt[j] = "ATCG"[c2]; }
 				txt[k] = 0;
 				fprintf(stderr, "[vdjx] unseen survivor %u: %s gated count %u first gated instance record %llu offset %llu\n", i, txt, gc[i],
 				        (unsigned long long) (gf[i] >> 6), (unsigned long long) (gf[i] & 63));
@@ -2732,7 +2771,8 @@
 }
 
 template <typename A>
-int stage_finish2(vdjx_ctx* c, A& db, const SurvivorsG& sv, const RecountOut& ro, u64 n_records_total, int k, int P, int ob, vdjx_graph* g) {
+int stage_finish2(vdjx_ctx* c, A& db, const SurvivorsG& sv, const RecountOut& ro, u64 n_records_total, int k, int P, int ob, vdjx_graph* g,
+                  const RecountStatus* rs = nullptr, u32* rs_host = nullptr) {
 	hipStream_t st = c->stream;
 	const u32 ns = sv.n;
 	const u32 nr = sv.n_real <= ns ? sv.n_real : ns;
@@ -2746,7 +2786,7 @@
 	HIP_TRY(db.alloc(&d_hj, ns));
 	{
 		vdjx_prof_scope ps(c, "k_node_flags");
-		hipLaunchKernelGGL(k_node_flags, dim3((ns + 255) / 256), dim3(256), 0, st, sv.lo, sv.hi, ns, k, c->d_vbits, c->d_jbits, d_hv, d_hj);
+		hipLaunchKernelGGL(k_node_flags, dim3((ns + 255) / 256), dim3(256), 0, st, sv.skey, ns, k, c->d_vbits, c->d_jbits, d_hv, d_hj);
 	}
 	u64 *rk_key, *rk_key2;
 	u32 *rk_idx, *rk_idx2, *rank;
@@ -2781,7 +2821,7 @@
 	g->d_roots = (u32*) carve((size_t) ns * 4);
 	{
 		vdjx_prof_scope ps(c, "k_node_order");
-		hipLaunchKernelGGL(k_rank_keys, dim3((ns + 255) / 256), dim3(256), 0, st, sv.ufirst, sv.gcnt, ns, rk_key, rk_idx);
+		hipLaunchKernelGGL(k_rank_keys, dim3((ns + 255) / 256), dim3(256), 0, st, sv.ufirst, sv.gcnt, ns, rk_key, rk_idx, rs && rs->g_err ? rs->g_err + 1 : (u32*) nullptr);
 		{
 			size_t tb = 0;
 			int rc_ = vdjx_sort_pairs_raw(nullptr, &tb, st, rk_key, rk_key2, rk_idx, rk_idx2, ns, rk_bits);
@@ -2791,9 +2831,10 @@
 			if ((rc_ = vdjx_sort_pairs_raw(tmp, &tb, st, rk_key, rk_key2, rk_idx, rk_idx2, ns, rk_bits))) return rc_;
 		}
 		hipLaunchKernelGGL(k_rank_scatter, dim3((ns + 255) / 256), dim3(256), 0, st, rk_key2, rk_idx2, ns, rank);
-		hipLaunchKernelGGL(k_node_emit2, dim3((ns + 255) / 256), dim3(256), 0, st, sv.lo, sv.hi, sv.gcnt, sv.ucnt, sv.ufirst, d_hv, d_hj, rank,
-		                   ro.edge_first, ro.edge_to, ro.in_first, ro.in_from, ns, k, no);
-	}
+		hipLaunchKernelGGL(k_node_emit2, dim3((ns + 255) / 256), dim3(256), 0, st, sv.skey, sv.gcnt, sv.ucnt, sv.ufirst, d_hv, d_hj, rank,
+		                   ro.succ, ro.in_first, ro.in_from, ns, k, no);
+	}
+	if (rs && rs->g_err) { if (int rc_ = recount_status_fetch(c, *rs, rs_host)) return rc_; }
 	u32 n_roots = 0;
 	{
 		const u32 nrb = (nr + 255) / 256;
@@ -2833,25 +2874,22 @@
 	RecountOut ro{};
 	if (sv.n) {
 		HIP_TRY(db.alloc(&sv.ucnt, sv.n)); HIP_TRY(db.alloc(&sv.ufirst, sv.n));
-		HIP_TRY(db.alloc(&ro.in_first, (size_t) sv.n * 4)); HIP_TRY(db.alloc(&ro.in_from, (size_t) sv.n * 4));
-		HIP_TRY(db.alloc(&ro.edge_first, (size_t) sv.n * 4)); HIP_TRY(db.alloc(&ro.edge_to, (size_t) sv.n * 4));
+		HIP_TRY(db.alloc(&ro.in_first, (size_t) sv.n * 4));
 		ro.ucnt = sv.ucnt; ro.ufirst = sv.ufirst;
+		const SurvivorsG sv_in = sv;
 		for (int attempt = 0; attempt < 2; attempt++) {
 			const bool sym_walk = sym && sym_walk_wanted() && attempt == 0;
 			c->stats["kmer_build_sym_walk"] = sym_walk ? 1 : 0;
 			RecountStatus rs;
+			sv = sv_in;
 			rc = stage_recount(c, db, pool, 0, k, sv, ro, true, nullptr, &rs, sym_walk);
 			if (rc == VDJX_ESYMWALK && sym_walk) { c->stats["kmer_build_sym_walk_retries"] += 1; continue; }
 			if (rc) return rc;
 			u32* hp = (u32*) c->h_pin + 1024;
 			hp[6] = hp[7] = 0;
-			if (rs.g_err) {
-				HIP_TRY(hipMemcpyAsync(hp + 8, rs.n_inst, 24, hipMemcpyDeviceToHost, c->stream));
-				HIP_TRY(hipMemcpyAsync(hp + 2, rs.n_items, 4, hipMemcpyDeviceToHost, c->stream));
-			}
-			rc = stage_finish2(c, db, sv, ro, pool->n_records, k, P, pool->ob, g);
+			rc = stage_finish2(c, db, sv, ro, pool->n_records, k, P, pool->ob, g, &rs, hp);
 			if (rc) return rc;
-			if (rs.g_err) { hp[4] = hp[8]; hp[5] = hp[9]; hp[0] = hp[10]; hp[1] = hp[11]; hp[6] = hp[12]; hp[7] = hp[13]; }
+			if (rs.g_err) recount_status_order(hp);
 			rc = rs.g_err ? recount_status_check(c, hp, rs.ns) : VDJX_OK;
 			if (rc != VDJX_ESYMWALK || !sym_walk) return rc == VDJX_ESYMWALK ? VDJX_EHIP : rc;
 			c->stats["kmer_build_sym_walk_retries"] += 1;
@@ -2905,7 +2943,7 @@
 	std::vector<u32> src_base, nq;
 	u32 *p_fl = nullptr, *p_S = nullptr, *p_r0 = nullptr;
 	u32 mqq = 0, tlow = 0;
-	SurvTable tb{};
+	const u32 *succ = nullptr, *in_from = nullptr;
 	int phase = 0;
 	bool have_hist = false;
 	GatedHist gh;
@@ -3332,16 +3370,17 @@
 	hipLaunchKernelGGL(k_surv_unpack, dim3((a.n + 255) / 256), dim3(256), 0, c->stream, (const SurvRec*) d_surv_all, a.n, a.lo, a.hi, a.gcnt, a.gfirst, d_nreal);
 	u32* h_nreal = (u32*) c->h_pin + 1536;
 	HIP_TRY(hipMemcpyAsync(h_nreal, d_nreal, 4, hipMemcpyDeviceToHost, c->stream));
-	RecountOut ro{(u32*) d_ucnt, (u64*) d_ufirst, (u64*) d_in_first, nullptr, nullptr, nullptr};
+	RecountOut ro{(u32*) d_ucnt, (u64*) d_ufirst, (u64*) d_in_first, nullptr, nullptr};
 	const bool sym_walk = s->sym && sym_walk_wanted();
 	c->stats["kmer_build_sym_walk"] = sym_walk ? 1 : 0;
 	const SurvivorsG a_in = a;
-	int rc = stage_recount(c, db, s->pool, s->rec_base(), s->k, a, ro, false, &s->tb, nullptr, sym_walk);
+	int rc = stage_recount(c, db, s->pool, s->rec_base(), s->k, a, ro, false, nullptr, nullptr, sym_walk);
 	if (rc == VDJX_ESYMWALK && sym_walk) {
 		c->stats["kmer_build_sym_walk_retries"] += 1;
 		a = a_in;
-		rc = stage_recount(c, db, s->pool, s->rec_base(), s->k, a, ro, false, &s->tb, nullptr, false);
-	}
+		rc = stage_recount(c, db, s->pool, s->rec_base(), s->k, a, ro, false, nullptr, nullptr, false);
+	}
+	s->succ = ro.succ; s->in_from = ro.in_from;
 	if (rc == VDJX_OK) a.n_real = *h_nreal;
 	if (rc || !s->scan) return rc == VDJX_ESYMWALK ? VDJX_EHIP : rc;
 	hipLaunchKernelGGL(k_first_to_scan, dim3((a.n * 5 + 255) / 256), dim3(256), 0, c->stream, (u64*) d_in_first, (size_t) a.n * 4, (u64*) d_ufirst, (size_t) a.n, s->scan, s->pool->ob);
@@ -3366,11 +3405,8 @@
 		a.ucnt = (u32*) d_ucnt;
 		a.ufirst = (u64*) d_ufirst;
 		ro.ucnt = a.ucnt; ro.ufirst = a.ufirst; ro.in_first = (u64*) d_in_first;
-		HIP_TRY(db.alloc(&ro.in_from, (size_t) a.n * 4));
-		HIP_TRY(db.alloc(&ro.edge_first, (size_t) a.n * 4));
-		HIP_TRY(db.alloc(&ro.edge_to, (size_t) a.n * 4));
-		HIP_TRY(hipMemsetAsync(ro.edge_first, 0xFF, (size_t) a.n * 32, c->stream));
-		hipLaunchKernelGGL(k_edges_from_in, dim3((a.n * 4 + 255) / 256), dim3(256), 0, c->stream, s->tb, a.n, s->k, ro.in_first, ro.in_from, ro.edge_first, ro.edge_to);
+		if (!s->succ || !s->in_from) { vdjx_set_error("vdjx_shard_finish: vdjx_shard_edges did not complete"); return VDJX_ESTATE; }
+		ro.succ = s->succ; ro.in_from = s->in_from;
 	}
 	vdjx_graph* g = new vdjx_graph();
 	g->pre_nodes = (size_t) pre_nodes_total;
```
